# Kaixhin/imitation-learning

Measured on NVIDIA H100. Metric: env_steps_per_s, higher is better.
Workload: dtype f32

## Files before the change

### imitation-learning_b200/_lib.py

```python
from __future__ import annotations

import ctypes as C
import os
import threading
from typing import Dict, Optional

import torch

_HERE = os.path.dirname(os.path.abspath(__file__))
LIB_PATH = os.path.join(_HERE, 'csrc', 'libil_b200.so')
MAX_LAYERS = 6
MAX_WIDTH_CLASSES = 8
ACT = {'relu': 0, 'tanh': 1, 'sigmoid': 2}
REWARD = {'AIRL': 0, 'GAIL': 1, 'FAIRL': 2}
LOSS = {'BCE': 0, 'Mixup': 1, 'PUGAIL': 2}
GEMM_MODE = {'fp32': 0, 'tf32x3': 1, 'tf32': 2}

c_f32p, c_i32p, c_i64p, c_u64p, vp = C.c_void_p, C.c_void_p, C.c_void_p, C.c_void_p, C.c_void_p


class Mlp(C.Structure):
  _fields_ = [('params', vp), ('stride', C.c_int64), ('n_layers', C.c_int32), ('activation', C.c_int32), ('dims', C.c_int32 * (MAX_LAYERS + 1)), ('_pad', C.c_int32)]


class Adam(C.Structure):
  _fields_ = [('m', vp), ('v', vp), ('step', vp), ('lr', C.c_double), ('beta1', C.c_double), ('beta2', C.c_double), ('eps', C.c_double), ('weight_decay', C.c_double), ('lr_r', vp),
              ('weight_decay_r', vp), ('replica_floats', C.c_int64)]


class Batch(C.Structure):
  _fields_ = [('rows', vp), ('replica_stride', C.c_int64), ('B', C.c_int32), ('S', C.c_int32), ('A', C.c_int32), ('row', C.c_int32)]


class Replay(C.Structure):
  _fields_ = [('rows', vp), ('replica_stride', C.c_int64), ('idx', vp), ('full', vp), ('num_trajectories', vp), ('size', C.c_int32), ('S', C.c_int32), ('A', C.c_int32),
              ('row', C.c_int32), ('absorbing', C.c_int32), ('shared', C.c_int32)]


class SacArgs(C.Structure):
  _fields_ = [('actor', Mlp), ('critic', Mlp), ('target', Mlp), ('actor_opt', Adam), ('critic_opt', Adam), ('alpha_opt', Adam), ('log_alpha', vp), ('batch', Batch),
              ('absorbing', vp), ('absorbing_from_state', C.c_int32), ('R', C.c_int32), ('eps_next', vp), ('eps_new', vp), ('discount', C.c_float),
              ('entropy_target', C.c_float), ('polyak_factor', C.c_float), ('_pad0', C.c_float), ('out_log_probs', vp), ('out_q_values', vp), ('out_losses', vp),
              ('workspace', vp), ('workspace_bytes', C.c_int64), ('discount_r', vp), ('entropy_target_r', vp), ('polyak_r', vp)]


class BcArgs(C.Structure):
  _fields_ = [('actor', Mlp), ('opt', Adam), ('batch', Batch), ('R', C.c_int32), ('_pad', C.c_int32), ('out_loss', vp), ('workspace', vp), ('workspace_bytes', C.c_int64)]


class Gail(C.Structure):
  _fields_ = [('g', Mlp), ('u', vp), ('v', vp), ('u_stride', C.c_int32), ('v_stride', C.c_int32), ('state_only', C.c_int32), ('reward_function', C.c_int32),
              ('reward_function_r', vp), ('spectral_norm_r', vp), ('n_width_classes', C.c_int32), ('width_class_H', C.c_int32 * MAX_WIDTH_CLASSES),
              ('width_class_begin', C.c_int32 * MAX_WIDTH_CLASSES), ('_pad', C.c_int32), ('replica_order', vp)]


class GailUpdateArgs(C.Structure):
  _fields_ = [('disc', Gail), ('opt', Adam), ('policy', Batch), ('expert', Batch), ('eps_gp', vp), ('eps_mix', vp), ('R', C.c_int32), ('loss_function', C.c_int32),
              ('training', C.c_int32), ('_pad', C.c_int32), ('grad_penalty', C.c_float), ('entropy_bonus', C.c_float), ('pos_class_prior', C.c_float),
              ('nonnegative_margin', C.c_float), ('out_losses', vp), ('workspace', vp), ('workspace_bytes', C.c_int64), ('grad_penalty_r', vp), ('entropy_bonus_r', vp),
              ('loss_function_r', vp), ('pos_class_prior_r', vp), ('nonnegative_margin_r', vp)]


class Gailx(C.Structure):
  _fields_ = [('g', Mlp), ('h', Mlp), ('g_u', vp), ('g_v', vp), ('h_u', vp), ('h_v', vp), ('g_u_stride', C.c_int32), ('g_v_stride', C.c_int32), ('h_u_stride', C.c_int32),
              ('h_v_stride', C.c_int32), ('state_only', C.c_int32), ('reward_function', C.c_int32), ('subtract_log_policy', C.c_int32), ('discount', C.c_float), ('discount_r', vp)]


class GailxUpdateArgs(C.Structure):
  _fields_ = [('disc', Gailx), ('opt', Adam), ('params_floats', C.c_int64), ('policy', Batch), ('expert', Batch), ('eps_gp', vp), ('eps_mix', vp), ('logp_policy', vp),
              ('logp_expert', vp), ('logp_mix', vp), ('R', C.c_int32), ('loss_function', C.c_int32), ('training', C.c_int32), ('_pad', C.c_int32), ('grad_penalty', C.c_float),
              ('entropy_bonus', C.c_float), ('pos_class_prior', C.c_float), ('nonnegative_margin', C.c_float), ('out_losses', vp), ('workspace', vp), ('workspace_bytes', C.c_int64), ('grad_penalty_r', vp),
              ('entropy_bonus_r', vp)]


class Red(C.Structure):
  _fields_ = [('predictor', Mlp), ('target', Mlp), ('sigma', vp), ('state_only', C.c_int32), ('_pad', C.c_int32)]


class RedUpdateArgs(C.Structure):
  _fields_ = [('disc', Red), ('opt', Adam), ('batch', Batch), ('R', C.c_int32), ('_pad', C.c_int32), ('mask_in', vp), ('mask_hid', vp * MAX_LAYERS), ('out_loss', vp), ('workspace', vp),
              ('workspace_bytes', C.c_int64)]


class Pwil(C.Structure):
  _fields_ = [('atoms', vp), ('scale', vp), ('offset', vp), ('weights', vp), ('N', C.c_int32), ('d', C.c_int32), ('S', C.c_int32), ('A', C.c_int32), ('state_only', C.c_int32),
              ('time_horizon', C.c_int32), ('reward_scale', C.c_float), ('reward_bandwidth', C.c_float)]


class Env(C.Structure):
  _fields_ = [('M', vp), ('N', vp), ('c', vp), ('w_r', vp), ('x', vp), ('t', vp), ('obs', C.c_int32), ('act', C.c_int32), ('absorbing', C.c_int32),
              ('max_episode_steps', C.c_int32), ('early_termination', C.c_int32), ('term_threshold', C.c_float)]


class EvalArgs(C.Structure):
  _fields_ = [('actor', Mlp), ('env', Env), ('R', C.c_int32), ('episodes', C.c_int32), ('max_steps', C.c_int32), ('traj_T', C.c_int32), ('state', vp), ('returns', vp),
              ('traj_states', vp), ('traj_actions', vp), ('traj_rewards', vp), ('traj_len', vp), ('out_counters', vp), ('workspace', vp), ('workspace_bytes', C.c_int64)]


i32, i64, u64, f32 = C.c_int32, C.c_int64, C.c_uint64, C.c_float
P = C.POINTER

SIGNATURES = {
  'il_create': (C.c_int, [C.c_int, P(vp)]),
  'il_destroy': (C.c_int, [vp]),
  'il_last_error': (C.c_char_p, []),
  'il_version': (C.c_int, []),
  'il_set_gemm_mode': (C.c_int, [vp, C.c_int]),
  'il_launch_count': (i64, [vp]),
  'il_set_option': (C.c_int, [vp, C.c_char_p, C.c_int]),
  'il_struct_sizes': (C.c_int, [P(i32)]),
  'il_mlp_param_offsets': (C.c_int, [P(i32), C.c_int, P(i64), P(i64), P(i64)]),
  'il_row_layout': (C.c_int, [C.c_int, C.c_int, P(i32), P(i32)]),
  'il_profile_begin': (C.c_int, [vp]),
  'il_profile_end': (C.c_int, [vp, P(C.c_double), P(C.c_double), P(i64)]),
  'il_profile_bytes': (C.c_int, [vp, P(C.c_double)]),
  'il_debug_gemm': (C.c_int, [vp, C.c_int, C.c_int, C.c_int, C.c_int, vp, i64, C.c_int, C.c_int, vp, i64, C.c_int, C.c_int, vp, i64, C.c_int, vp, i64, C.c_int, vp, i64, C.c_int,
                              C.c_int, vp, i64, vp]),
  'il_fill_normal': (C.c_int, [vp, vp, i64, u64, u64, vp, vp]),
  'il_fill_uniform': (C.c_int, [vp, vp, i64, u64, u64, vp, vp]),
  'il_counter_add': (C.c_int, [vp, vp, u64, vp]),
  'il_fill_beta': (C.c_int, [vp, vp, C.c_int, i64, vp, u64, u64, vp, vp]),
  'il_actor_workspace_bytes': (i64, [P(Mlp), C.c_int, C.c_int]),
  'il_actor_forward': (C.c_int, [vp, P(Mlp), C.c_int, C.c_int, vp, i64, C.c_int, vp, vp, vp, vp, vp, vp, vp, i64, vp]),
  'il_critic_workspace_bytes': (i64, [P(Mlp), C.c_int, C.c_int]),
  'il_critic_forward': (C.c_int, [vp, P(Mlp), C.c_int, C.c_int, C.c_int, vp, i64, C.c_int, vp, i64, C.c_int, vp, vp, vp, i64, vp]),
  'il_polyak': (C.c_int, [vp, vp, vp, i64, f32, vp]),
  'il_sac_workspace_bytes': (i64, [P(SacArgs)]),
  'il_sac_update': (C.c_int, [vp, P(SacArgs), vp]),
  'il_bc_workspace_bytes': (i64, [P(BcArgs)]),
  'il_bc_update': (C.c_int, [vp, P(BcArgs), vp]),
  'il_adam_step': (C.c_int, [vp, vp, vp, P(Adam), i64, vp]),
  'il_adam_step_polyak': (C.c_int, [vp, vp, vp, P(Adam), i64, vp, C.c_float, vp]),
  'il_adam_step_polyak_r': (C.c_int, [vp, vp, vp, P(Adam), i64, vp, vp, vp]),
  'il_fill_dropout_mask': (C.c_int, [vp, vp, i64, f32, u64, u64, vp, vp]),
  'il_actor_dropout_workspace_bytes': (i64, [P(Mlp), C.c_int, C.c_int]),
  'il_actor_log_prob_dropout': (C.c_int, [vp, P(Mlp), C.c_int, C.c_int, C.c_int, vp, i64, C.c_int, vp, vp, P(vp), vp, vp, i64, vp]),
  'il_bc_update_dropout': (C.c_int, [vp, P(BcArgs), vp, P(vp), vp]),
  'il_dril_reward': (C.c_int, [vp, vp, C.c_int, C.c_int, C.c_int, vp, C.c_int, vp, i64, C.c_int, vp, vp]),
  'il_red_workspace_bytes': (i64, [P(Red), C.c_int, C.c_int]),
  'il_red_update': (C.c_int, [vp, P(RedUpdateArgs), vp]),
  'il_red_sigma': (C.c_int, [vp, P(Red), C.c_int, P(Batch), vp, P(vp), vp, i64, vp]),
  'il_red_reward': (C.c_int, [vp, P(Red), C.c_int, P(Batch), vp, i64, C.c_int, vp, i64, vp]),
  'il_replay_append': (C.c_int, [vp, P(Replay), C.c_int, vp, vp, vp, vp, vp, vp, vp, vp, C.c_int, vp]),
  'il_replay_wrap_absorbing': (C.c_int, [vp, P(Replay), C.c_int, vp, vp]),
  'il_replay_transfer': (C.c_int, [vp, P(Replay), C.c_int, P(Replay), vp]),
  'il_replay_sample_indices': (C.c_int, [vp, P(Replay), C.c_int, C.c_int, vp, vp, u64, u64, vp, vp]),
  'il_replay_gather': (C.c_int, [vp, P(Replay), C.c_int, vp, P(Batch), vp]),
  'il_mix_expert_rows': (C.c_int, [vp, P(Batch), P(Batch), C.c_int, vp]),
  'il_adril_relabel': (C.c_int, [vp, P(Batch), P(Batch), C.c_int, C.c_int, C.c_int, vp, vp, f32, vp, C.c_int, C.c_int, vp]),
  'il_gail_workspace_bytes': (i64, [P(GailUpdateArgs)]),
  'il_gail_update': (C.c_int, [vp, P(GailUpdateArgs), vp]),
  'il_gail_reward': (C.c_int, [vp, P(Gail), C.c_int, P(Batch), vp, i64, C.c_int, vp, vp]),
  'il_gailx_workspace_bytes': (i64, [P(GailxUpdateArgs)]),
  'il_gailx_update': (C.c_int, [vp, P(GailxUpdateArgs), vp]),
  'il_gailx_reward_workspace_bytes': (i64, [P(Gailx), C.c_int, C.c_int]),
  'il_gailx_reward': (C.c_int, [vp, P(Gailx), C.c_int, P(Batch), vp, vp, i64, C.c_int, vp, vp, i64, vp]),
  'il_gail_mix_batch': (C.c_int, [vp, P(Batch), P(Batch), vp, C.c_int, P(Batch), vp]),
  'il_gmmil_workspace_bytes': (i64, [C.c_int, C.c_int]),
  'il_gmmil_bandwidth': (C.c_int, [vp, C.c_int, P(Batch), P(Batch), C.c_int, vp, vp, i64, vp]),
  'il_gmmil_reward': (C.c_int, [vp, C.c_int, P(Batch), P(Batch), C.c_int, vp, vp, i64, C.c_int, vp]),
  'il_pwil_reset': (C.c_int, [vp, P(Pwil), C.c_int, vp, vp]),
  'il_pwil_reward': (C.c_int, [vp, P(Pwil), C.c_int, vp, vp, vp, vp, vp]),
  'il_env_reset': (C.c_int, [vp, P(Env), C.c_int, vp, vp, vp, vp, vp]),
  'il_env_step': (C.c_int, [vp, P(Env), C.c_int, vp, vp, vp, vp, vp, vp, vp, vp, vp]),
  'il_rollout_bookkeep': (C.c_int, [vp, C.c_int, vp, vp, vp, vp, vp, vp, vp, vp]),
  'il_eval_accumulate': (C.c_int, [vp, C.c_int, vp, vp, vp, vp, vp, vp]),
  'il_return_stats': (C.c_int, [vp, vp, i64, vp, vp]),
  'il_eval_workspace_bytes': (i64, [P(EvalArgs)]),
  'il_eval_rollout': (C.c_int, [vp, P(EvalArgs), vp]),
  'il_nccl_unique_id': (C.c_int, [vp]),
  'il_nccl_comm_create': (C.c_int, [vp, C.c_int, C.c_int, P(vp)]),
  'il_nccl_comm_destroy': (C.c_int, [vp]),
  'il_return_allreduce': (C.c_int, [vp, vp, vp, i64, vp, vp]),
}

_lock = threading.Lock()
_lib: Optional[C.CDLL] = None
_handles: Dict[int, int] = {}


def build(force: bool = False, verbose: bool = False) -> str:
  import importlib.util
  spec = importlib.util.spec_from_file_location('il_b200_csrc_build', os.path.join(_HERE, 'csrc', 'build.py'))
  mod = importlib.util.module_from_spec(spec)
  spec.loader.exec_module(mod)
  return mod.build(force=force, verbose=verbose)


def lib() -> C.CDLL:
  global _lib
  with _lock:
    if _lib is None:
      if not os.path.exists(LIB_PATH): build()
      l = C.CDLL(LIB_PATH)
      for name, (res, args) in SIGNATURES.items():
        fn = getattr(l, name)
        fn.restype, fn.argtypes = res, args
      _lib = l
  return _lib


def last_error() -> str:
  return lib().il_last_error().decode()


def check(rc: int):
  if rc != 0: raise RuntimeError(f'il_b200: {last_error()}')


def handle(device: Optional[int] = None) -> int:
  if not torch.cuda.is_available():
    raise RuntimeError('il_b200: no CUDA device available; the hot path only exists as sm_90a kernels (no CPU fallback)')
  device = torch.cuda.current_device() if device is None else device
  with _lock:
    h = _handles.get(device)
  if h is None:
    out = vp()
    check(lib().il_create(device, C.byref(out)))
    h = out.value
    with _lock: _handles[device] = h
    mode = os.environ.get('IL_GEMM_MODE')
    if mode: check(lib().il_set_gemm_mode(h, GEMM_MODE[mode]))
  return h


def set_option(name: str, value: int):
  check(lib().il_set_option(handle(), name.encode(), int(value)))


def stream() -> int:
  return torch.cuda.current_stream().cuda_stream


def launch_count() -> int:
  return int(lib().il_launch_count(handle()))


def mask_array(masks):
  arr = (vp * MAX_LAYERS)()
  for i, t in enumerate(masks or []): arr[i] = None if t is None else t.data_ptr()
  return arr


def ptr(t: Optional[torch.Tensor]) -> Optional[int]:
  if t is None: return None
  assert t.is_cuda, 'il_b200 expects CUDA tensors'
  return t.data_ptr()


def mlp_offsets(dims):
  n = len(dims) - 1
  d = (i32 * len(dims))(*dims)
  w, b, tot = (i64 * n)(), (i64 * n)(), i64()
  check(lib().il_mlp_param_offsets(d, n, w, b, C.byref(tot)))
  return list(w), list(b), tot.value


def row_layout(S: int, A: int):
  off, n = (i32 * 8)(), i32()
  check(lib().il_row_layout(S, A, off, C.byref(n)))
  names = ('states', 'actions', 'rewards', 'next_states', 'terminals', 'timeouts', 'weights', 'step')
  return dict(zip(names, list(off))), n.value


def py_mlp_offsets(dims):
  al = lambda x, a: (x + a - 1) // a * a
  off, w, b = 0, [], []
  for l in range(len(dims) - 1):
    w.append(off)
    off = al(off + dims[l + 1] * dims[l], 4)
    b.append(off)
    off = al(off + dims[l + 1], 4)
  return w, b, al(off, 32)


def py_row_layout(S: int, A: int):
  off = dict(states=0, actions=S, rewards=S + A, next_states=S + A + 1, terminals=2 * S + A + 1, timeouts=2 * S + A + 2, weights=2 * S + A + 3, step=2 * S + A + 4)
  return off, (2 * S + A + 5 + 3) // 4 * 4
```

### imitation-learning_b200/csrc/common.cuh

```cuda
#pragma once
#include <cuda_runtime.h>
#include <stdint.h>
#include <stdio.h>
#include <string.h>

#include <vector>

#include "../../include/il_b200.h"

struct ProfiledLaunch {
  cudaEvent_t start, stop;
  double flops;
  double bytes;
};
struct il_handle {
  int device;
  int sm_count;
  int gemm_mode;
  int thin_hoist;
  int wide_tn;
  int first_layer_fast;
  int mask_bits;
  int head_fused;
  int debug_sync;
  int adam_tma;
  int gail_tiled;
  int tc_fuse_l1;
  long long launches;
  int profiling;
  std::vector<ProfiledLaunch> profiled;
  double profiled_bytes;
  void* eval_graph;
  cudaStream_t build_stream;
};
void il_eval_release(il_handle* h);

extern thread_local char g_il_error[512];

#define IL_FAIL(...)                                     \
  do {                                                   \
    snprintf(g_il_error, sizeof(g_il_error), __VA_ARGS__); \
    return 1;                                            \
  } while (0)

#define IL_CHECK(cond, ...)        \
  do {                             \
    if (!(cond)) IL_FAIL(__VA_ARGS__); \
  } while (0)

#define IL_CUDA(expr)                                                                             \
  do {                                                                                            \
    cudaError_t _e = (expr);                                                                      \
    if (_e != cudaSuccess) IL_FAIL("%s failed: %s (%s:%d)", #expr, cudaGetErrorString(_e), __FILE__, __LINE__); \
  } while (0)

#define IL_LAUNCH(h, kernel, grid, block, smem, stream, ...)                                      \
  do {                                                                                            \
    kernel<<<(grid), (block), (smem), (cudaStream_t)(stream)>>>(__VA_ARGS__);                     \
    (h)->launches++;                                                                              \
    cudaError_t _e = cudaPeekAtLastError();                                                       \
    if (_e != cudaSuccess) IL_FAIL("launch of %s failed: %s (%s:%d)", #kernel, cudaGetErrorString(_e), __FILE__, __LINE__); \
  } while (0)

#define IL_TRY(expr)          \
  do {                        \
    int _r = (expr);          \
    if (_r != 0) return _r;   \
  } while (0)

__host__ __device__ static inline int64_t il_align_up(int64_t x, int64_t a) { return (x + a - 1) / a * a; }

struct RowLayout {
  int state, action, reward, next_state, terminal, timeout, weight, step, len;
};
__host__ __device__ inline RowLayout row_layout(int S, int A) {
  RowLayout L;
  L.state = 0;
  L.action = S;
  L.reward = S + A;
  L.next_state = S + A + 1;
  L.terminal = 2 * S + A + 1;
  L.timeout = L.terminal + 1;
  L.weight = L.terminal + 2;
  L.step = L.terminal + 3;
  L.len = (2 * S + A + 5 + 3) / 4 * 4;
  return L;
}

struct MlpOffsets {
  int64_t w[IL_MAX_LAYERS], b[IL_MAX_LAYERS], total;
};
__host__ __device__ static inline MlpOffsets mlp_offsets(const int32_t* dims, int n_layers) {
  MlpOffsets o;
  int64_t off = 0;
  for (int l = 0; l < n_layers; ++l) {
    o.w[l] = off;
    off = il_align_up(off + (int64_t)dims[l + 1] * dims[l], 4);
    o.b[l] = off;
    off = il_align_up(off + dims[l + 1], 4);
  }
  o.total = il_align_up(off, 32);
  return o;
}

__device__ __forceinline__ float act_apply(float x, int act) {
  if (act == IL_ACT_RELU) return fmaxf(x, 0.f);
  if (act == IL_ACT_TANH) return tanhf(x);
  return 1.f / (1.f + expf(-x));
}
__device__ __forceinline__ float act_grad_from_output(float y, int act) {
  if (act == IL_ACT_RELU) return y > 0.f ? 1.f : 0.f;
  if (act == IL_ACT_TANH) return 1.f - y * y;
  return y * (1.f - y);
}
__device__ __forceinline__ float softplusf(float x) {
  return x > 20.f ? x : log1pf(expf(x));
}
__device__ __forceinline__ float sigmoidf(float x) { return 1.f / (1.f + expf(-x)); }

__device__ __forceinline__ float warp_sum(float v) {
#pragma unroll
  for (int o = 16; o > 0; o >>= 1) v += __shfl_xor_sync(0xffffffffu, v, o);
  return v;
}
__device__ __forceinline__ float warp_max(float v) {
#pragma unroll
  for (int o = 16; o > 0; o >>= 1) v = fmaxf(v, __shfl_xor_sync(0xffffffffu, v, o));
  return v;
}
__device__ __forceinline__ float block_sum(float v, float* red) {
  const int lane = threadIdx.x & 31, warp = threadIdx.x >> 5, nw = (blockDim.x + 31) >> 5;
  v = warp_sum(v);
  __syncthreads();
  if (lane == 0) red[warp] = v;
  __syncthreads();
  float r = 0.f;
  if (warp == 0) {
    r = lane < nw ? red[lane] : 0.f;
    r = warp_sum(r);
    if (lane == 0) red[0] = r;
  }
  __syncthreads();
  return red[0];
}

__device__ __forceinline__ uint4 philox4x32_10(uint4 ctr, uint2 key) {
  const uint32_t M0 = 0xD2511F53u, M1 = 0xCD9E8D57u, W0 = 0x9E3779B9u, W1 = 0xBB67AE85u;
#pragma unroll
  for (int i = 0; i < 10; ++i) {
    const uint32_t hi0 = __umulhi(M0, ctr.x), lo0 = M0 * ctr.x;
    const uint32_t hi1 = __umulhi(M1, ctr.z), lo1 = M1 * ctr.z;
    ctr = make_uint4(hi1 ^ ctr.y ^ key.x, lo1, hi0 ^ ctr.w ^ key.y, lo0);
    key.x += W0;
    key.y += W1;
  }
  return ctr;
}
__device__ __forceinline__ float u32_to_unit(uint32_t x) { return (float)(x >> 8) * (1.0f / 16777216.0f); }

struct GemmArgs {
  const float* A;
  int64_t a_gs;
  int a_gdiv, lda, a_kmajor;
  const float* B;
  int64_t b_gs;
  int b_gdiv, ldb, b_kmajor;
  float* C;
  int64_t c_gs;
  int ldc;
  const float* bias;
  int64_t bias_gs;
  int act;
  const float* mask;
  int64_t mask_gs;
  int ldmask, mask_act;
  float* colsum;
  int64_t colsum_gs;
  int accumulate;
  int M, N, K, G;
  const uint32_t* mask_bits;
  int64_t mask_bits_gs;
  uint32_t* bits_out;
  int64_t bits_out_gs;
};
int launch_gemm(il_handle* h, const GemmArgs& a, cudaStream_t stream);
bool gemm_uses_tc(const il_handle* h, const GemmArgs& a);
bool gemm_first_layer_emits_bits(const il_handle* h, const GemmArgs& a);
double gemm_algorithmic_bytes(const GemmArgs& a, bool stores_c);
int profile_open(il_handle* h, ProfiledLaunch* pl, double flops, double bytes, cudaStream_t stream);
int profile_close(il_handle* h, ProfiledLaunch* pl, cudaStream_t stream);

bool tc_gemm_eligible(const GemmArgs& a);
int launch_tc_gemm(il_handle* h, const GemmArgs& a, cudaStream_t stream);
int tc_gemm_init();
struct TcFuseL1 {
  const float* x;
  int64_t x_gs;
  int x_gdiv, x_ld, x_k;
  const float* w1;
  const float* b1;
  int64_t gs;
  float* store;
  int64_t store_gs;
};
bool tc_head_fusable(const il_handle* h, const GemmArgs& a, int head_n);
bool tc_l1_fusable(const il_handle* h, const GemmArgs& a, int x_k);
bool tc_dx_head_fusable(const il_handle* h, const GemmArgs& a, int head_n);
int launch_tc_gemm_dx_head(il_handle* h, const GemmArgs& a, const float* w, int64_t w_gs, int w_ns, int head_n, float* out, int64_t out_gs, cudaStream_t stream);
int launch_tc_gemm_head(il_handle* h, const GemmArgs& a, const float* head_w, const float* head_b, int64_t head_gs, int head_n, float* head_out, int64_t head_out_gs, int store_c,
                        cudaStream_t stream, const TcFuseL1* l1 = nullptr);
```

### imitation-learning_b200/csrc/mlp.cu

```cuda
#include "mlp.cuh"

#include <math.h>

constexpr int HB_MAXN = 8;
struct HeadBwdArgs {
  const float* dout; int64_t dout_gs; int dout_gdiv, ld_dout;
  const float* w; int64_t w_gs;
  const float* y; int64_t y_gs;
  float* dz; int64_t dz_gs;
  float* dw; float* db; float* db_prev; int64_t g_gs;
  int n, H, Nh;
};
int launch_head_backward(il_handle* h, const HeadBwdArgs& a, int G, cudaStream_t stream);
int launch_head_dx_bits(il_handle* h, const HeadBwdArgs& a, const uint32_t* bits, int64_t bits_gs, int G, cudaStream_t stream);

int mlp_validate(const il_mlp* m, const char* what) {
  IL_CHECK(m != nullptr && m->params != nullptr, "%s: null mlp", what);
  IL_CHECK(m->n_layers >= 1 && m->n_layers <= IL_MAX_LAYERS, "%s: n_layers %d out of range", what, m->n_layers);
  IL_CHECK(m->activation >= 0 && m->activation <= 2, "%s: bad activation %d", what, m->activation);
  for (int l = 0; l <= m->n_layers; ++l) IL_CHECK(m->dims[l] > 0, "%s: dims[%d] = %d", what, l, m->dims[l]);
  const MlpOffsets o = mlp_offsets(m->dims, m->n_layers);
  IL_CHECK(m->stride >= o.total - 31 && m->stride % 4 == 0, "%s: stride %lld too small / unaligned for %lld parameters", what, (long long)m->stride, (long long)o.total);
  IL_CHECK((reinterpret_cast<uintptr_t>(m->params) & 15) == 0, "%s: params not 16-byte aligned", what);
  return 0;
}

int mlp_max_hidden(const il_mlp* m) {
  int mx = 1;
  for (int l = 1; l <= m->n_layers; ++l) mx = m->dims[l] > mx ? m->dims[l] : mx;
  return mx;
}

static int64_t mlp_bits_bytes(const il_mlp* m, int G, int n, int l) {
  return m->dims[l + 1] % 32 == 0 ? il_align_up((int64_t)G * n * (m->dims[l + 1] / 32) * 4, 256) : 0;
}

int64_t mlp_acts_bytes(const il_mlp* m, int G, int n) {
  int64_t b = 0;
  for (int l = 0; l + 1 < m->n_layers; ++l) b += il_align_up((int64_t)G * n * m->dims[l + 1] * 4, 256) + mlp_bits_bytes(m, G, n, l);
  return b;
}

char* mlp_acts_carve(const il_mlp* m, int G, int n, char* ws, MlpActs* acts) {
  for (int l = 0; l < IL_MAX_LAYERS; ++l) { acts->hid[l] = nullptr; acts->bits[l] = nullptr; acts->bits_valid[l] = false; }
  for (int l = 0; l + 1 < m->n_layers; ++l) {
    acts->hid[l] = reinterpret_cast<float*>(ws);
    ws += il_align_up((int64_t)G * n * m->dims[l + 1] * 4, 256);
    if (mlp_bits_bytes(m, G, n, l)) {
      acts->bits[l] = reinterpret_cast<uint32_t*>(ws);
      ws += mlp_bits_bytes(m, G, n, l);
    }
  }
  return ws;
}

int mlp_forward(il_handle* h, const il_mlp* m, int G, int n, MatView X, MlpActs& acts, float* out, int64_t out_gs, int ld_out, cudaStream_t stream, int keep) {
  const MlpOffsets o = mlp_offsets(m->dims, m->n_layers);
  const int L = m->n_layers;
  const bool keep_hidden = keep != MLP_KEEP_NONE;
  const bool want_bits = h->mask_bits && keep_hidden && m->activation == IL_ACT_RELU;
  for (int l = 0; l < IL_MAX_LAYERS; ++l) acts.bits_valid[l] = false;
  auto layer_args = [&](int l) {
    GemmArgs a{};
    if (l == 0) { a.A = X.ptr; a.a_gs = X.gs; a.a_gdiv = X.gdiv; a.lda = X.ld; }
    else { a.A = acts.hid[l - 1]; a.a_gs = (int64_t)n * m->dims[l]; a.a_gdiv = 1; a.lda = m->dims[l]; }
    a.a_kmajor = 1;
    a.B = m->params + o.w[l]; a.b_gs = m->stride; a.b_gdiv = 1; a.ldb = m->dims[l]; a.b_kmajor = 1;
    a.bias = m->params + o.b[l]; a.bias_gs = m->stride;
    if (l == L - 1) { a.C = out; a.c_gs = out_gs; a.ldc = ld_out; a.act = -1; }
    else { a.C = acts.hid[l]; a.c_gs = (int64_t)n * m->dims[l + 1]; a.ldc = m->dims[l + 1]; a.act = m->activation; }
    a.M = n; a.N = m->dims[l + 1]; a.K = m->dims[l]; a.G = G;
    return a;
  };
  const bool head_shape = L >= 2 && m->activation == IL_ACT_RELU && ld_out == m->dims[L] && out_gs == (int64_t)n * m->dims[L];
  for (int l = 0; l < L; ++l) {
    if (head_shape && l == L - 2) {
      GemmArgs a = layer_args(l);
      if (tc_head_fusable(h, a, m->dims[L])) {
        const bool bits = want_bits && keep == MLP_KEEP_MASKS && acts.bits[l] && m->dims[L] <= HB_MAXN;
        if (bits) { a.bits_out = acts.bits[l]; a.bits_out_gs = (int64_t)n * (m->dims[l + 1] / 32); acts.bits_valid[l] = true; }
        IL_TRY(launch_tc_gemm_head(h, a, m->params + o.w[L - 1], m->params + o.b[L - 1], m->stride, m->dims[L], out, out_gs, keep_hidden && !bits ? 1 : 0, stream));
        return 0;
      }
    }
    if (head_shape && l == 0 && L == 3) {
      GemmArgs a1 = layer_args(1);
      a1.A = nullptr; a1.a_gs = 0; a1.a_gdiv = 1; a1.lda = m->dims[1];
      if (tc_head_fusable(h, a1, m->dims[L]) && tc_l1_fusable(h, a1, m->dims[0])) {
        TcFuseL1 f{};
        f.x = X.ptr; f.x_gs = X.gs; f.x_gdiv = X.gdiv; f.x_ld = X.ld; f.x_k = m->dims[0];
        f.w1 = m->params + o.w[0]; f.b1 = m->params + o.b[0]; f.gs = m->stride;
        f.store = keep_hidden ? acts.hid[0] : nullptr; f.store_gs = (int64_t)n * m->dims[1];
        IL_TRY(launch_tc_gemm_head(h, a1, m->params + o.w[L - 1], m->params + o.b[L - 1], m->stride, m->dims[L], out, out_gs, keep_hidden ? 1 : 0, stream, &f));
        return 0;
      }
    }
    GemmArgs a = layer_args(l);
    if (want_bits && l + 1 < L && acts.bits[l] && gemm_first_layer_emits_bits(h, a)) {
      a.bits_out = acts.bits[l]; a.bits_out_gs = (int64_t)n * (m->dims[l + 1] / 32);
      acts.bits_valid[l] = true;
    }
    IL_TRY(launch_gemm(h, a, stream));
  }
  return 0;
}

static bool head_backward_eligible(const il_mlp* m, int n, int64_t grad_stride) {
  const int L = m->n_layers, H = m->dims[L - 1], Nh = m->dims[L];
  return m->activation == IL_ACT_RELU && Nh <= HB_MAXN && H % 4 == 0 && n <= 1024 && grad_stride % 4 == 0 && m->stride % 4 == 0;
}

int mlp_backward(il_handle* h, const il_mlp* m, int G, int n, MatView X, const MlpActs& acts, MatView dOut, float* grads, int64_t grad_stride,
                 float* dX, int64_t dx_gs, int ld_dx, int dx_col0, int dx_cols, float* tmpA, float* tmpB, cudaStream_t stream) {
  const MlpOffsets o = mlp_offsets(m->dims, m->n_layers);
  const int L = m->n_layers;
  MatView dZ = dOut;
  float* next_tmp = tmpA;
  bool bias_done = false;
  for (int l = L - 1; l >= 0; --l) {
    MatView Xin = l == 0 ? X : MatView{acts.hid[l - 1], (int64_t)n * m->dims[l], 1, m->dims[l]};
    if (l == L - 1 && l > 0 && grads && h->head_fused && head_backward_eligible(m, n, grad_stride)) {
      HeadBwdArgs a{};
      a.dout = dZ.ptr; a.dout_gs = dZ.gs; a.dout_gdiv = dZ.gdiv; a.ld_dout = dZ.ld;
      a.w = m->params + o.w[l]; a.w_gs = m->stride;
      a.y = acts.hid[l - 1]; a.y_gs = (int64_t)n * m->dims[l];
      a.dz = next_tmp; a.dz_gs = (int64_t)n * m->dims[l];
      a.dw = grads + o.w[l]; a.db = grads + o.b[l]; a.db_prev = grads + o.b[l - 1]; a.g_gs = grad_stride;
      a.n = n; a.H = m->dims[l]; a.Nh = m->dims[l + 1];
      IL_TRY(launch_head_backward(h, a, G, stream));
      dZ = MatView{next_tmp, (int64_t)n * m->dims[l], 1, m->dims[l]};
      next_tmp = next_tmp == tmpA ? tmpB : tmpA;
      bias_done = true;
      continue;
    }
    if (l == L - 1 && l > 0 && !grads && acts.bits_valid[l - 1] && m->dims[l + 1] <= HB_MAXN) {
      HeadBwdArgs a{};
      a.dout = dZ.ptr; a.dout_gs = dZ.gs; a.dout_gdiv = dZ.gdiv; a.ld_dout = dZ.ld;
      a.w = m->params + o.w[l]; a.w_gs = m->stride;
      a.dz = next_tmp; a.dz_gs = (int64_t)n * m->dims[l];
      a.n = n; a.H = m->dims[l]; a.Nh = m->dims[l + 1];
      IL_TRY(launch_head_dx_bits(h, a, acts.bits[l - 1], (int64_t)n * (m->dims[l] / 32), G, stream));
      dZ = MatView{next_tmp, (int64_t)n * m->dims[l], 1, m->dims[l]};
      next_tmp = next_tmp == tmpA ? tmpB : tmpA;
      continue;
    }
    if (grads) {
      GemmArgs a{};
      a.A = dZ.ptr; a.a_gs = dZ.gs; a.a_gdiv = dZ.gdiv; a.lda = dZ.ld; a.a_kmajor = 0;
      a.B = Xin.ptr; a.b_gs = Xin.gs; a.b_gdiv = Xin.gdiv; a.ldb = Xin.ld; a.b_kmajor = 0;
      a.C = grads + o.w[l]; a.c_gs = grad_stride; a.ldc = m->dims[l]; a.act = -1;
      if (!bias_done) { a.colsum = grads + o.b[l]; a.colsum_gs = grad_stride; }
      bias_done = false;
      a.M = m->dims[l + 1]; a.N = m->dims[l]; a.K = n; a.G = G;
      IL_TRY(launch_gemm(h, a, stream));
    }
    if (l > 0) {
      GemmArgs a{};
      a.A = dZ.ptr; a.a_gs = dZ.gs; a.a_gdiv = dZ.gdiv; a.lda = dZ.ld; a.a_kmajor = 1;
      a.B = m->params + o.w[l]; a.b_gs = m->stride; a.b_gdiv = 1; a.ldb = m->dims[l]; a.b_kmajor = 0;
      a.C = next_tmp; a.c_gs = (int64_t)n * m->dims[l]; a.ldc = m->dims[l]; a.act = -1;
      a.mask_act = m->activation;
      a.M = n; a.N = m->dims[l]; a.K = m->dims[l + 1]; a.G = G;
      if (acts.bits_valid[l - 1] && m->activation == IL_ACT_RELU && gemm_uses_tc(h, a)) {
        a.mask_bits = acts.bits[l - 1]; a.mask_bits_gs = (int64_t)n * (m->dims[l] / 32);
        if (h->mask_bits >= 2 && l == 1 && !grads && dX && ld_dx == dx_cols && dx_gs == (int64_t)n * dx_cols && tc_dx_head_fusable(h, a, dx_cols)) {
          a.C = nullptr;
          IL_TRY(launch_tc_gemm_dx_head(h, a, m->params + o.w[0] + dx_col0, m->stride, m->dims[0], dx_cols, dX, dx_gs, stream));
          return 0;
        }
      } else {
        a.mask = acts.hid[l - 1]; a.mask_gs = (int64_t)n * m->dims[l]; a.ldmask = m->dims[l];
      }
      IL_TRY(launch_gemm(h, a, stream));
      dZ = MatView{next_tmp, (int64_t)n * m->dims[l], 1, m->dims[l]};
      next_tmp = next_tmp == tmpA ? tmpB : tmpA;
    } else if (dX) {
      GemmArgs a{};
      a.A = dZ.ptr; a.a_gs = dZ.gs; a.a_gdiv = dZ.gdiv; a.lda = dZ.ld; a.a_kmajor = 1;
      a.B = m->params + o.w[0] + dx_col0; a.b_gs = m->stride; a.b_gdiv = 1; a.ldb = m->dims[0]; a.b_kmajor = 0;
      a.C = dX; a.c_gs = dx_gs; a.ldc = ld_dx; a.act = -1;
      a.M = n; a.N = dx_cols; a.K = m->dims[1]; a.G = G;
      IL_TRY(launch_gemm(h, a, stream));
    }
  }
  return 0;
}

namespace {

__global__ void actor_head_kernel(const HeadFwdArgs p) {
  const int64_t row = (int64_t)blockIdx.x * blockDim.x + threadIdx.x;
  if (row >= (int64_t)p.R * p.n) return;
  const int r = (int)(row / p.n), i = (int)(row % p.n);
  const int A = p.A;
  const float* hd = p.head + row * 2 * A;
  float* act_row = p.action ? p.action + (int64_t)r * p.action_rs + (int64_t)i * p.ld_action : nullptr;
  if (p.copy_src && act_row) {
    const float* src = p.copy_src + (int64_t)r * p.copy_rs + (int64_t)i * p.copy_ld;
    for (int j = 0; j < p.copy_cols; ++j) act_row[j - p.copy_cols] = __ldg(src + j);
  }
  const float keep = p.zero_mask ? 1.f - __ldg(p.zero_mask + (int64_t)r * p.zero_mask_rs + (int64_t)i * p.zero_mask_ld) : 1.f;
  const float LOG_SQRT_2PI = 0.91893853320467274178f, LOG2 = 0.69314718055994530942f;
  const float A_LO = (float)(-1.0 + 1e-6), A_HI = (float)(1.0 - 1e-6);
  float sum_ladj = 0.f, sum_nlp = 0.f;
  const bool want_lp = p.log_prob != nullptr && (p.eps != nullptr || p.given != nullptr);
  for (int j = 0; j < A; ++j) {
    const float mu = hd[j];
    const float ls = fminf(fmaxf(hd[A + j], -20.f), 2.f);
    if (p.mean) p.mean[row * A + j] = mu;
    if (p.log_std) p.log_std[row * A + j] = ls;
    float x, a;
    const float sd = expf(ls);
    if (p.given) {
      a = fminf(fmaxf(p.given[row * A + j], A_LO), A_HI);
      x = atanhf(a);
    } else if (p.eps) {
      x = __fadd_rn(mu, __fmul_rn(sd, p.eps[row * A + j]));
      a = tanhf(x);
    } else {
      x = mu;
      a = tanhf(mu);
    }
    if (act_row && !p.given) act_row[j] = keep * a;
    if (want_lp) {
      const float var = __fmul_rn(sd, sd);
      const float diff = __fsub_rn(x, mu);
      float nlp = __fdiv_rn(-__fmul_rn(diff, diff), __fmul_rn(2.f, var));
      nlp = __fsub_rn(__fsub_rn(nlp, logf(sd)), LOG_SQRT_2PI);
      const float ladj = __fmul_rn(2.f, __fsub_rn(__fsub_rn(LOG2, x), softplusf(__fmul_rn(-2.f, x))));
      sum_nlp += nlp;
      sum_ladj += ladj;
    }
  }
  if (want_lp) p.log_prob[row] = __fadd_rn(__fsub_rn(0.f, sum_ladj), sum_nlp);
}

struct SmallFwdArgs {
  il_mlp m;
  MlpOffsets o;
  const float* X;
  int64_t x_gs;
  int x_gdiv, ldx, n, maxd;
  float* out;
  int tanh_first;
};
template <int NR>
__global__ void __launch_bounds__(256) mlp_small_forward_kernel(const SmallFwdArgs p) {
  extern __shared__ __align__(16) float sm[];
  const int g = blockIdx.x, r0 = blockIdx.y * NR, tid = threadIdx.x, warp = tid >> 5, lane = tid & 31;
  const int nr = min(NR, p.n - r0), L = p.m.n_layers, maxd = p.maxd;
  float* bufs[2] = {sm, sm + NR * maxd};
  const float* X = p.X + (int64_t)(g / p.x_gdiv) * p.x_gs;
  for (int idx = tid; idx < NR * p.m.dims[0]; idx += 256) {
    const int r = idx / p.m.dims[0], k = idx % p.m.dims[0];
    bufs[0][r * maxd + k] = r < nr ? __ldg(X + (int64_t)(r0 + r) * p.ldx + k) : 0.f;
  }
  const float* prm = p.m.params + (int64_t)g * p.m.stride;
  __syncthreads();
  for (int l = 0; l < L; ++l) {
    const int in = p.m.dims[l], od = p.m.dims[l + 1];
    const float* W = prm + p.o.w[l];
    const float* bias = prm + p.o.b[l];
    const float* xin = bufs[l & 1];
    float* xout = bufs[(l + 1) & 1];
    const bool vec = (in % 4 == 0) && (p.m.stride % 4 == 0);
    if (NR == 1 && vec && in <= 16) {
      for (int o = tid; o < od; o += 256) {
        const float4* wr = reinterpret_cast<const float4*>(W + (int64_t)o * in);
        float4 w4[4];
#pragma unroll
        for (int q = 0; q < 4; ++q) w4[q] = 4 * q < in ? __ldg(wr + q) : make_float4(0.f, 0.f, 0.f, 0.f);
        float v = __ldg(bias + o);
#pragma unroll
        for (int q = 0; q < 4; ++q)
          if (4 * q < in) {
            const float4 x4 = *reinterpret_cast<const float4*>(xin + 4 * q);
            v = fmaf(w4[q].x, x4.x, fmaf(w4[q].y, x4.y, fmaf(w4[q].z, x4.z, fmaf(w4[q].w, x4.w, v))));
          }
        if (l < L - 1) v = act_apply(v, p.m.activation);
        xout[o] = v;
      }
      __syncthreads();
      continue;
    }
    if (NR == 1 && vec && in % 128 == 0 && in <= 256) {
      const int kv = in >> 7;
      float4 x4[2];
#pragma unroll
      for (int v = 0; v < 2; ++v) x4[v] = v < kv ? *reinterpret_cast<const float4*>(xin + v * 128 + lane * 4) : make_float4(0.f, 0.f, 0.f, 0.f);
      for (int o0 = warp * 8; o0 < od; o0 += 64) {
        float4 w4[8][2];
#pragma unroll
        for (int u = 0; u < 8; ++u)
#pragma unroll
          for (int v = 0; v < 2; ++v)
            w4[u][v] = (o0 + u < od && v < kv) ? __ldg(reinterpret_cast<const float4*>(W + (int64_t)(o0 + u) * in + v * 128 + lane * 4)) : make_float4(0.f, 0.f, 0.f, 0.f);
        float a8[8];
#pragma unroll
        for (int u = 0; u < 8; ++u) {
          float t = 0.f;
#pragma unroll
          for (int v = 0; v < 2; ++v) t = fmaf(w4[u][v].x, x4[v].x, fmaf(w4[u][v].y, x4[v].y, fmaf(w4[u][v].z, x4[v].z, fmaf(w4[u][v].w, x4[v].w, t))));
          a8[u] = warp_sum(t);
        }
        if (lane < 8 && o0 + lane < od) {
          float v = a8[0];
#pragma unroll
          for (int u = 1; u < 8; ++u) v = lane == u ? a8[u] : v;
          v += __ldg(bias + o0 + lane);
          if (l < L - 1) v = act_apply(v, p.m.activation);
          xout[o0 + lane] = v;
        }
      }
      __syncthreads();
      continue;
    }
    if (NR == 1 && vec) {
      for (int o0 = warp * 4; o0 < od; o0 += 32) {
        float a4[4] = {0.f, 0.f, 0.f, 0.f};
        for (int k = lane * 4; k < in; k += 128) {
          const float4 x4 = *reinterpret_cast<const float4*>(xin + k);
          float4 w4[4];
#pragma unroll
          for (int u = 0; u < 4; ++u) w4[u] = o0 + u < od ? __ldg(reinterpret_cast<const float4*>(W + (int64_t)(o0 + u) * in + k)) : make_float4(0.f, 0.f, 0.f, 0.f);
#pragma unroll
          for (int u = 0; u < 4; ++u) a4[u] = fmaf(w4[u].x, x4.x, fmaf(w4[u].y, x4.y, fmaf(w4[u].z, x4.z, fmaf(w4[u].w, x4.w, a4[u]))));
        }
#pragma unroll
        for (int u = 0; u < 4; ++u) a4[u] = warp_sum(a4[u]);
        if (lane < 4 && o0 + lane < od) {
          float v = (lane == 0 ? a4[0] : lane == 1 ? a4[1] : lane == 2 ? a4[2] : a4[3]) + __ldg(bias + o0 + lane);
          if (l < L - 1) v = act_apply(v, p.m.activation);
          xout[o0 + lane] = v;
        }
      }
      __syncthreads();
      continue;
    }
    for (int o = warp; o < od; o += 8) {
      float acc[NR];
#pragma unroll
      for (int r = 0; r < NR; ++r) acc[r] = 0.f;
      const float* wr = W + (int64_t)o * in;
      if (vec) {
        for (int k = lane * 4; k < in; k += 128) {
          const float4 w4 = __ldg(reinterpret_cast<const float4*>(wr + k));
#pragma unroll
          for (int r = 0; r < NR; ++r) {
            const float4 x4 = *reinterpret_cast<const float4*>(xin + r * maxd + k);
            acc[r] = fmaf(w4.x, x4.x, fmaf(w4.y, x4.y, fmaf(w4.z, x4.z, fmaf(w4.w, x4.w, acc[r]))));
          }
        }
      } else {
        for (int k = lane; k < in; k += 32) {
          const float w = __ldg(wr + k);
#pragma unroll
          for (int r = 0; r < NR; ++r) acc[r] = fmaf(w, xin[r * maxd + k], acc[r]);
        }
      }
#pragma unroll
      for (int r = 0; r < NR; ++r) acc[r] = warp_sum(acc[r]);
      if (lane == 0) {
        const float b = __ldg(bias + o);
#pragma unroll
        for (int r = 0; r < NR; ++r) {
          float v = acc[r] + b;
          if (l < L - 1) v = act_apply(v, p.m.activation);
          xout[r * maxd + o] = v;
        }
      }
    }
    __syncthreads();
  }
  const int od = p.m.dims[L];
  const float* fin = bufs[L & 1];
  if (p.tanh_first > 0) {
    const int A = p.tanh_first;
    for (int idx = tid; idx < nr * A; idx += 256) {
      const int r = idx / A, o = idx % A;
      p.out[((int64_t)g * p.n + r0 + r) * A + o] = tanhf(fin[r * maxd + o]);
    }
    return;
  }
  for (int idx = tid; idx < nr * od; idx += 256) {
    const int r = idx / od, o = idx % od;
    p.out[((int64_t)g * p.n + r0 + r) * od + o] = fin[r * maxd + o];
  }
}

struct AdamReplicas {
  const double* lr_r;
  const double* wd_r;
  const float* tau_r;
  int64_t rf;
  float inv_rf;
  int R;
};
struct AdamCoef { float step_size, decay, tau, one_minus_tau; };
constexpr int ADAM_MAX_REPLICAS = 2048;
__device__ __forceinline__ void adam_fill_table(AdamCoef* tab, const AdamReplicas& rp, double lr, double wd, double beta1_d, const int64_t* step, float tau) {
  if (!rp.R) return;
  const double bc1 = 1.0 - pow(beta1_d, (double)*step);
  for (int r = threadIdx.x; r < rp.R; r += blockDim.x) {
    const double l = rp.lr_r ? rp.lr_r[r] : lr, w = rp.wd_r ? rp.wd_r[r] : wd;
    const float t = rp.tau_r ? rp.tau_r[r] : tau;
    tab[r] = AdamCoef{(float)(l / bc1), w != 0.0 ? (float)(1.0 - l * w) : 1.f, t, (float)(1.0 - (double)t)};
  }
}
__device__ __forceinline__ int adam_replica(int64_t f, const AdamReplicas& rp) {
  int r = (int)((float)f * rp.inv_rf);
  if ((int64_t)r * rp.rf > f) --r;
  else if ((int64_t)(r + 1) * rp.rf <= f) ++r;
  return r;
}

__global__ void adam_kernel(float* __restrict__ p, const float* __restrict__ g, float* __restrict__ m, float* __restrict__ v, const int64_t* __restrict__ step,
                            double lr, double beta1_d, double beta2_d, double eps_d, double wd, int64_t n, float* __restrict__ target, float tau, float one_minus_tau,
                            const AdamReplicas rp) {
  extern __shared__ AdamCoef adam_tab[];
  __shared__ float s_step_size, s_bc2_sqrt;
  if (threadIdx.x == 0) {
    const double t = (double)*step;
    const double bc1 = 1.0 - pow(beta1_d, t), bc2 = 1.0 - pow(beta2_d, t);
    s_step_size = (float)(lr / bc1);
    s_bc2_sqrt = (float)sqrt(bc2);
  }
  adam_fill_table(adam_tab, rp, lr, wd, beta1_d, step, tau);
  __syncthreads();
  const float step_size = s_step_size, bc2_sqrt = s_bc2_sqrt;
  const float decay = (float)(1.0 - lr * wd), w1 = (float)(1.0 - beta1_d), w2 = (float)(1.0 - beta2_d);
  const float beta2 = (float)beta2_d, eps = (float)eps_d;
  const bool has_wd = wd != 0.0;
  auto upd = [&](float& pi, float& mi, float& vi, float gi, float ss, float dc, bool wdf) {
    if (wdf) pi = __fmul_rn(pi, dc);
    mi = __fadd_rn(mi, __fmul_rn(w1, __fsub_rn(gi, mi)));
    vi = __fadd_rn(__fmul_rn(vi, beta2), __fmul_rn(__fmul_rn(w2, gi), gi));
    const float denom = __fadd_rn(__fdiv_rn(sqrtf(vi), bc2_sqrt), eps);
    pi = __fadd_rn(pi, __fmul_rn(-ss, __fdiv_rn(mi, denom)));
  };
  const int64_t n4 = n >> 2;
  for (int64_t i = (int64_t)blockIdx.x * blockDim.x + threadIdx.x; i < n4; i += (int64_t)gridDim.x * blockDim.x) {
    float ss = step_size, dc = decay, ta = tau, omt = one_minus_tau;
    bool wdf = has_wd;
    if (rp.R) {
      const AdamCoef c = adam_tab[adam_replica(i << 2, rp)];
      ss = c.step_size; dc = c.decay; wdf = c.decay != 1.f; ta = c.tau; omt = c.one_minus_tau;
    }
    float4 pv = reinterpret_cast<float4*>(p)[i], mv = reinterpret_cast<float4*>(m)[i], vv = reinterpret_cast<float4*>(v)[i];
    const float4 gv = reinterpret_cast<const float4*>(g)[i];
    upd(pv.x, mv.x, vv.x, gv.x, ss, dc, wdf); upd(pv.y, mv.y, vv.y, gv.y, ss, dc, wdf); upd(pv.z, mv.z, vv.z, gv.z, ss, dc, wdf); upd(pv.w, mv.w, vv.w, gv.w, ss, dc, wdf);
    reinterpret_cast<float4*>(p)[i] = pv; reinterpret_cast<float4*>(m)[i] = mv; reinterpret_cast<float4*>(v)[i] = vv;
    if (target) {
      const float tau = ta, one_minus_tau = omt;
      float4 tv = reinterpret_cast<float4*>(target)[i];
      tv.x = __fadd_rn(__fmul_rn(tv.x, tau), __fmul_rn(one_minus_tau, pv.x)); tv.y = __fadd_rn(__fmul_rn(tv.y, tau), __fmul_rn(one_minus_tau, pv.y));
      tv.z = __fadd_rn(__fmul_rn(tv.z, tau), __fmul_rn(one_minus_tau, pv.z)); tv.w = __fadd_rn(__fmul_rn(tv.w, tau), __fmul_rn(one_minus_tau, pv.w));
      reinterpret_cast<float4*>(target)[i] = tv;
    }
  }
  for (int64_t i = (n4 << 2) + (int64_t)blockIdx.x * blockDim.x + threadIdx.x; i < n; i += (int64_t)gridDim.x * blockDim.x) {
    float pi = p[i], mi = m[i], vi = v[i];
    upd(pi, mi, vi, g[i], step_size, decay, has_wd);
    p[i] = pi; m[i] = mi; v[i] = vi;
    if (target) target[i] = __fadd_rn(__fmul_rn(target[i], tau), __fmul_rn(one_minus_tau, pi));
  }
}

constexpr int ADAM_STREAMS = 5;
constexpr int ADAM_CONSUMERS = 256;
template <int TILE, int STAGES> constexpr int adam_tma_smem() { return STAGES * ADAM_STREAMS * TILE * 4 + 2 * STAGES * 8 + 64; }
__device__ __forceinline__ void adam_mbar_wait(uint32_t bar, uint32_t parity) {
  asm volatile(
      "{\n\t.reg .pred q;\n\t"
      "ADAM_WAIT:\n\t"
      "mbarrier.try_wait.parity.shared::cta.b64 q, [%0], %1;\n\t"
      "@q bra ADAM_DONE;\n\t"
      "bra ADAM_WAIT;\n\t"
      "ADAM_DONE:\n\t}" ::"r"(bar), "r"(parity) : "memory");
}
template <int TILE, int STAGES>
__global__ void __launch_bounds__(ADAM_CONSUMERS + 32) adam_tma_kernel(float* __restrict__ p, const float* __restrict__ g, float* __restrict__ m, float* __restrict__ v,
                                                                      const int64_t* __restrict__ step, double lr, double beta1_d, double beta2_d, double eps_d, double wd, int64_t n,
                                                                      float* __restrict__ target, float tau, float one_minus_tau, const AdamReplicas rp) {
  extern __shared__ __align__(128) uint8_t adam_smem[];
  float* buf = reinterpret_cast<float*>(adam_smem);
  AdamCoef* tab = reinterpret_cast<AdamCoef*>(adam_smem + adam_tma_smem<TILE, STAGES>());
  const uint32_t smem0 = (uint32_t)__cvta_generic_to_shared(buf);
  const uint32_t full0 = smem0 + (uint32_t)(STAGES * ADAM_STREAMS * TILE * 4), done0 = full0 + 8u * STAGES;
  __shared__ float s_step_size, s_bc2_sqrt;
  const int tid = threadIdx.x;
  adam_fill_table(tab, rp, lr, wd, beta1_d, step, tau);
  if (tid == 0) {
    const double t = (double)*step;
    s_step_size = (float)(lr / (1.0 - pow(beta1_d, t)));
    s_bc2_sqrt = (float)sqrt(1.0 - pow(beta2_d, t));
    for (int s_ = 0; s_ < STAGES; ++s_) {
      asm volatile("mbarrier.init.shared::cta.b64 [%0], 1;" ::"r"(full0 + 8u * s_));
      asm volatile("mbarrier.init.shared::cta.b64 [%0], %1;" ::"r"(done0 + 8u * s_), "r"(ADAM_CONSUMERS));
    }
    asm volatile("fence.mbarrier_init.release.cluster;" ::: "memory");
  }
  __syncthreads();
  const int64_t n_tiles = (n + TILE - 1) / TILE;
  const int n_streams = target ? 5 : 4;
  auto tile_floats = [&](int64_t tile) { const int64_t left = n - tile * TILE; return (int)(left < TILE ? left : TILE); };
  const int64_t my_tiles = blockIdx.x < n_tiles ? (n_tiles - blockIdx.x + gridDim.x - 1) / gridDim.x : 0;
  if (tid >= ADAM_CONSUMERS) {
    if (tid != ADAM_CONSUMERS) return;
    auto issue_loads = [&](int64_t k) {
      const int64_t tile = blockIdx.x + k * gridDim.x;
      const int stage = (int)(k % STAGES);
      const uint32_t bytes = (uint32_t)tile_floats(tile) * 4u, bar = full0 + 8u * stage;
      asm volatile("mbarrier.arrive.expect_tx.shared::cta.b64 _, [%0], %1;" ::"r"(bar), "r"(bytes * (uint32_t)n_streams) : "memory");
      const float* src[5] = {p, g, m, v, target};
      for (int q = 0; q < n_streams; ++q)
        asm volatile("cp.async.bulk.shared::cluster.global.mbarrier::complete_tx::bytes [%0], [%1], %2, [%3];" ::"r"(smem0 + (uint32_t)((stage * ADAM_STREAMS + q) * TILE * 4)),
                     "l"(src[q] + tile * TILE), "r"(bytes), "r"(bar) : "memory");
    };
    for (int64_t k = 0; k < STAGES - 1 && k < my_tiles; ++k) issue_loads(k);
    for (int64_t k = 0; k < my_tiles; ++k) {
      const int stage = (int)(k % STAGES);
      const int64_t tile = blockIdx.x + k * gridDim.x;
      if (k + STAGES - 1 < my_tiles) {
        if (k > 0) asm volatile("cp.async.bulk.wait_group.read 0;" ::: "memory");
        issue_loads(k + STAGES - 1);
      }
      adam_mbar_wait(done0 + 8u * stage, (uint32_t)((k / STAGES) & 1));
      const uint32_t bytes = (uint32_t)tile_floats(tile) * 4u;
      float* dst[5] = {p, nullptr, m, v, target};
      for (int q = 0; q < n_streams; ++q) {
        if (!dst[q]) continue;
        asm volatile("cp.async.bulk.global.shared::cta.bulk_group [%0], [%1], %2;" ::"l"(dst[q] + tile * TILE), "r"(smem0 + (uint32_t)((stage * ADAM_STREAMS + q) * TILE * 4)), "r"(bytes)
                     : "memory");
      }
      asm volatile("cp.async.bulk.commit_group;" ::: "memory");
    }
    asm volatile("cp.async.bulk.wait_group 0;" ::: "memory");
    return;
  }
  const float step_size = s_step_size, bc2_sqrt = s_bc2_sqrt;
  const float decay = (float)(1.0 - lr * wd), w1 = (float)(1.0 - beta1_d), w2 = (float)(1.0 - beta2_d), beta2 = (float)beta2_d, eps = (float)eps_d;
  const bool has_wd = wd != 0.0;
  auto upd = [&](float& pi, float& mi, float& vi, float gi, float ss, float dc, bool wdf) {
    if (wdf) pi = __fmul_rn(pi, dc);
    mi = __fadd_rn(mi, __fmul_rn(w1, __fsub_rn(gi, mi)));
    vi = __fadd_rn(__fmul_rn(vi, beta2), __fmul_rn(__fmul_rn(w2, gi), gi));
    const float denom = __fadd_rn(__fdiv_rn(sqrtf(vi), bc2_sqrt), eps);
    pi = __fadd_rn(pi, __fmul_rn(-ss, __fdiv_rn(mi, denom)));
  };
  for (int64_t k = 0; k < my_tiles; ++k) {
    const int stage = (int)(k % STAGES);
    const int64_t tile = blockIdx.x + k * gridDim.x;
    adam_mbar_wait(full0 + 8u * stage, (uint32_t)((k / STAGES) & 1));
    const int nf4 = tile_floats(tile) >> 2;
    float4* sp = reinterpret_cast<float4*>(buf + (stage * ADAM_STREAMS + 0) * TILE);
    const float4* sg = reinterpret_cast<const float4*>(buf + (stage * ADAM_STREAMS + 1) * TILE);
    float4* smm = reinterpret_cast<float4*>(buf + (stage * ADAM_STREAMS + 2) * TILE);
    float4* sv = reinterpret_cast<float4*>(buf + (stage * ADAM_STREAMS + 3) * TILE);
    float4* stg = reinterpret_cast<float4*>(buf + (stage * ADAM_STREAMS + 4) * TILE);
    for (int i = tid; i < nf4; i += ADAM_CONSUMERS) {
      float ss = step_size, dc = decay, ta = tau, omt = one_minus_tau;
      bool wdf = has_wd;
      if (rp.R) {
        const AdamCoef c = tab[adam_replica(tile * TILE + 4 * i, rp)];
        ss = c.step_size; dc = c.decay; wdf = c.decay != 1.f; ta = c.tau; omt = c.one_minus_tau;
      }
      float4 pv = sp[i], mv = smm[i], vv = sv[i];
      const float4 gv = sg[i];
      upd(pv.x, mv.x, vv.x, gv.x, ss, dc, wdf); upd(pv.y, mv.y, vv.y, gv.y, ss, dc, wdf); upd(pv.z, mv.z, vv.z, gv.z, ss, dc, wdf); upd(pv.w, mv.w, vv.w, gv.w, ss, dc, wdf);
      sp[i] = pv; smm[i] = mv; sv[i] = vv;
      if (target) {
        const float tau = ta, one_minus_tau = omt;
        float4 tv = stg[i];
        tv.x = __fadd_rn(__fmul_rn(tv.x, tau), __fmul_rn(one_minus_tau, pv.x)); tv.y = __fadd_rn(__fmul_rn(tv.y, tau), __fmul_rn(one_minus_tau, pv.y));
        tv.z = __fadd_rn(__fmul_rn(tv.z, tau), __fmul_rn(one_minus_tau, pv.z)); tv.w = __fadd_rn(__fmul_rn(tv.w, tau), __fmul_rn(one_minus_tau, pv.w));
        stg[i] = tv;
      }
    }
    asm volatile("fence.proxy.async.shared::cta;" ::: "memory");
    asm volatile("mbarrier.arrive.shared::cta.b64 _, [%0];" ::"r"(done0 + 8u * stage) : "memory");
  }
}

template <int TILE, int STAGES>
static int launch_adam_tma(il_handle* h, int ctas_per_sm, float* params, const float* grads, const il_adam* opt, int64_t n, cudaStream_t stream, float* polyak_target, float polyak_factor,
                           const AdamReplicas& rp) {
  static bool attr_set = false;
  if (!attr_set) {
    IL_CUDA(cudaFuncSetAttribute(adam_tma_kernel<TILE, STAGES>, cudaFuncAttributeMaxDynamicSharedMemorySize, adam_tma_smem<TILE, STAGES>() + ADAM_MAX_REPLICAS * (int)sizeof(AdamCoef)));
    attr_set = true;
  }
  const size_t smem = (size_t)adam_tma_smem<TILE, STAGES>() + (size_t)rp.R * sizeof(AdamCoef);
  IL_LAUNCH(h, (adam_tma_kernel<TILE, STAGES>), h->sm_count * ctas_per_sm, ADAM_CONSUMERS + 32, smem, stream, params, grads, opt->m, opt->v, opt->step, opt->lr, opt->beta1,
            opt->beta2, opt->eps, opt->weight_decay, n, polyak_target, polyak_factor, (float)(1.0 - (double)polyak_factor), rp);
  return 0;
}
constexpr int ADAM_TMA_MIN_TILES = 4096;


template <int NH>
__global__ void __launch_bounds__(256, 2) head_backward_kernel(const HeadBwdArgs p) {
  extern __shared__ __align__(16) float hb_sm[];
  const int g = blockIdx.y, n0 = blockIdx.x * 256, tid = threadIdx.x, tc = tid & 63, tr = tid >> 6, col = n0 + tc * 4;
  float* dos = hb_sm;
  float* red = hb_sm + p.n * HB_MAXN;
  const float* dout = p.dout + (int64_t)(g / p.dout_gdiv) * p.dout_gs;
  const bool active = col < p.H;
  const float* Y = p.y + (int64_t)g * p.y_gs + col;
  float4 yv[4], yn[4];
  auto fetch = [&](float4 (&dst)[4], int b0) {
#pragma unroll
    for (int u = 0; u < 4; ++u) {
      const int b = b0 + 4 * u;
      dst[u] = (active && b < p.n) ? __ldg(reinterpret_cast<const float4*>(Y + (int64_t)b * p.H)) : make_float4(0.f, 0.f, 0.f, 0.f);
    }
  };
  fetch(yv, tr);
  for (int i = tid; i < p.n * HB_MAXN; i += 256) {
    const int b = i / HB_MAXN, j = i % HB_MAXN;
    dos[i] = j < p.Nh ? __ldg(dout + (int64_t)b * p.ld_dout + j) : 0.f;
  }
  float4 w[NH];
#pragma unroll
  for (int j = 0; j < NH; ++j) w[j] = (active && j < p.Nh) ? __ldg(reinterpret_cast<const float4*>(p.w + (int64_t)g * p.w_gs + (int64_t)j * p.H + col)) : make_float4(0.f, 0.f, 0.f, 0.f);
  __syncthreads();
  float4 dw[NH], cs = make_float4(0.f, 0.f, 0.f, 0.f);
#pragma unroll
  for (int j = 0; j < NH; ++j) dw[j] = make_float4(0.f, 0.f, 0.f, 0.f);
  if (active) {
    float* DZ = p.dz + (int64_t)g * p.dz_gs + col;
    for (int b0 = tr; b0 < p.n; b0 += 16) {
      fetch(yn, b0 + 16);
#pragma unroll
      for (int u = 0; u < 4; ++u) {
        const int b = b0 + 4 * u;
        if (b >= p.n) continue;
        float dj[NH];
        if (NH == 1) dj[0] = dos[b * HB_MAXN];
        else {
          const float4 d0 = *reinterpret_cast<const float4*>(dos + b * HB_MAXN), d1 = *reinterpret_cast<const float4*>(dos + b * HB_MAXN + 4);
          const float t[8] = {d0.x, d0.y, d0.z, d0.w, d1.x, d1.y, d1.z, d1.w};
#pragma unroll
          for (int j = 0; j < NH; ++j) dj[j] = t[j];
        }
        float4 z = make_float4(0.f, 0.f, 0.f, 0.f);
#pragma unroll
        for (int j = 0; j < NH; ++j) {
          z.x = fmaf(dj[j], w[j].x, z.x); z.y = fmaf(dj[j], w[j].y, z.y); z.z = fmaf(dj[j], w[j].z, z.z); z.w = fmaf(dj[j], w[j].w, z.w);
          dw[j].x = fmaf(dj[j], yv[u].x, dw[j].x); dw[j].y = fmaf(dj[j], yv[u].y, dw[j].y); dw[j].z = fmaf(dj[j], yv[u].z, dw[j].z); dw[j].w = fmaf(dj[j], yv[u].w, dw[j].w);
        }
        z.x = yv[u].x > 0.f ? z.x : 0.f; z.y = yv[u].y > 0.f ? z.y : 0.f; z.z = yv[u].z > 0.f ? z.z : 0.f; z.w = yv[u].w > 0.f ? z.w : 0.f;
        cs.x += z.x; cs.y += z.y; cs.z += z.z; cs.w += z.w;
        *reinterpret_cast<float4*>(DZ + (int64_t)b * p.H) = z;
      }
#pragma unroll
      for (int u = 0; u < 4; ++u) yv[u] = yn[u];
    }
  }
  float4* r4 = reinterpret_cast<float4*>(red);
#pragma unroll
  for (int j = 0; j < NH; ++j) r4[(tr * (HB_MAXN + 1) + j) * 64 + tc] = dw[j];
  r4[(tr * (HB_MAXN + 1) + HB_MAXN) * 64 + tc] = cs;
  __syncthreads();
  if (tr == 0 && active) {
#pragma unroll
    for (int j = 0; j <= HB_MAXN; ++j) {
      if ((j < NH && j < p.Nh) || j == HB_MAXN) {
        float4 a = r4[(0 * (HB_MAXN + 1) + j) * 64 + tc];
#pragma unroll
        for (int q = 1; q < 4; ++q) {
          const float4 t = r4[(q * (HB_MAXN + 1) + j) * 64 + tc];
          a.x += t.x; a.y += t.y; a.z += t.z; a.w += t.w;
        }
        float* dst = j == HB_MAXN ? p.db_prev + (int64_t)g * p.g_gs + col : p.dw + (int64_t)g * p.g_gs + (int64_t)j * p.H + col;
        *reinterpret_cast<float4*>(dst) = a;
      }
    }
  }
  if (blockIdx.x == 0 && tid < p.Nh) {
    float sacc = 0.f;
    for (int b = 0; b < p.n; ++b) sacc += dos[b * HB_MAXN + tid];
    p.db[(int64_t)g * p.g_gs + tid] = sacc;
  }
}

__global__ void tick_kernel(int64_t* s0, int64_t* s1, int64_t* s2) {
  if (s0) *s0 += 1;
  if (s1) *s1 += 1;
  if (s2) *s2 += 1;
}

__global__ void polyak_kernel(float* __restrict__ t, const float* __restrict__ o, int64_t n, float tau, float one_minus_tau) {
  for (int64_t i = (int64_t)blockIdx.x * blockDim.x + threadIdx.x; i < n; i += (int64_t)gridDim.x * blockDim.x)
    t[i] = __fadd_rn(__fmul_rn(t[i], tau), __fmul_rn(one_minus_tau, o[i]));
}

__global__ void split_twin_kernel(const float* __restrict__ q, float* __restrict__ q1, float* __restrict__ q2, int R, int n) {
  const int64_t i = (int64_t)blockIdx.x * blockDim.x + threadIdx.x;
  if (i >= (int64_t)R * n) return;
  const int r = (int)(i / n), b = (int)(i % n);
  if (q1) q1[i] = q[((int64_t)2 * r) * n + b];
  if (q2) q2[i] = q[((int64_t)2 * r + 1) * n + b];
}

__global__ void concat_kernel(const float* __restrict__ s, int64_t s_rs, int ld_s, int S, const float* __restrict__ a, int64_t a_rs, int ld_a, int A,
                              float* __restrict__ x, int R, int n) {
  const int64_t idx = (int64_t)blockIdx.x * blockDim.x + threadIdx.x;
  const int d = S + A;
  if (idx >= (int64_t)R * n * d) return;
  const int j = (int)(idx % d);
  const int64_t row = idx / d;
  const int r = (int)(row / n), i = (int)(row % n);
  x[idx] = j < S ? s[(int64_t)r * s_rs + (int64_t)i * ld_s + j] : a[(int64_t)r * a_rs + (int64_t)i * ld_a + (j - S)];
}

inline int ew_blocks(int64_t n, int threads, int sm_count) {
  int64_t b = (n + threads - 1) / threads;
  const int64_t cap = (int64_t)sm_count * 16;
  return (int)(b < 1 ? 1 : (b > cap ? cap : b));
}

}

int launch_actor_head(il_handle* h, const HeadFwdArgs& a, cudaStream_t stream) {
  const int64_t rows = (int64_t)a.R * a.n;
  IL_LAUNCH(h, actor_head_kernel, (unsigned)((rows + 127) / 128), 128, 0, stream, a);
  return 0;
}

int launch_adam(il_handle* h, float* params, const float* grads, const il_adam* opt, int64_t n, cudaStream_t stream, float* polyak_target, float polyak_factor,
                const float* polyak_r) {
  IL_CHECK(opt->m && opt->v && opt->step, "adam: null state");
  IL_CHECK(((reinterpret_cast<uintptr_t>(params) | reinterpret_cast<uintptr_t>(grads) | reinterpret_cast<uintptr_t>(opt->m) | reinterpret_cast<uintptr_t>(opt->v) |
             reinterpret_cast<uintptr_t>(polyak_target)) & 15) == 0, "adam: buffers must be 16-byte aligned");
  AdamReplicas rp{opt->lr_r, opt->weight_decay_r, polyak_target ? polyak_r : nullptr, 0, 0.f, 0};
  if (rp.lr_r || rp.wd_r || rp.tau_r) {
    const int64_t rf = opt->replica_floats;
    IL_CHECK(rf > 0 && rf % 4 == 0 && n % rf == 0, "adam: per-replica hyper-parameters need replica_floats (%lld) > 0, a multiple of 4 dividing n = %lld", (long long)rf, (long long)n);
    IL_CHECK(n / rf <= ADAM_MAX_REPLICAS, "adam: %lld replicas with per-replica hyper-parameters exceed the limit of %d per buffer", (long long)(n / rf), ADAM_MAX_REPLICAS);
    rp.rf = rf; rp.inv_rf = 1.f / (float)rf; rp.R = (int)(n / rf);
  }
  if (h->adam_tma && n % 4 == 0 && n >= (int64_t)ADAM_TMA_MIN_TILES * h->sm_count * 2) {
    const int variant = h->adam_tma;
    switch (variant) {
      case 2: return launch_adam_tma<4096, 2>(h, 1, params, grads, opt, n, stream, polyak_target, polyak_factor, rp);
      case 3: return launch_adam_tma<2048, 3>(h, 1, params, grads, opt, n, stream, polyak_target, polyak_factor, rp);
      case 4: return launch_adam_tma<1024, 4>(h, 2, params, grads, opt, n, stream, polyak_target, polyak_factor, rp);
      case 5: return launch_adam_tma<1024, 3>(h, 3, params, grads, opt, n, stream, polyak_target, polyak_factor, rp);
      case 6: return launch_adam_tma<512, 4>(h, 4, params, grads, opt, n, stream, polyak_target, polyak_factor, rp);
      case 7: return launch_adam_tma<2048, 4>(h, 1, params, grads, opt, n, stream, polyak_target, polyak_factor, rp);
      default: return launch_adam_tma<2048, 2>(h, 2, params, grads, opt, n, stream, polyak_target, polyak_factor, rp);
    }
  }
  IL_LAUNCH(h, adam_kernel, ew_blocks(n / 4 + 1, 256, h->sm_count), 256, (size_t)rp.R * sizeof(AdamCoef), stream, params, grads, opt->m, opt->v, opt->step, opt->lr, opt->beta1, opt->beta2,
            opt->eps, opt->weight_decay, n, polyak_target, polyak_factor, (float)(1.0 - (double)polyak_factor), rp);
  return 0;
}

namespace {
template <int NH, int U>
__global__ void __launch_bounds__(256) head_dx_bits_kernel(const HeadBwdArgs p, const uint32_t* __restrict__ bits, int64_t bits_gs) {
  const int g = blockIdx.y, tid = threadIdx.x, tc = tid & 63, tr = tid >> 6, col = blockIdx.x * 256 + tc * 4;
  if (col >= p.H) return;
  const float* __restrict__ dout = p.dout + (int64_t)(g / p.dout_gdiv) * p.dout_gs;
  const uint32_t* __restrict__ bw = bits + (int64_t)g * bits_gs + (col >> 5);
  const int sh = col & 31, wpr = p.H >> 5;
  float4 w[NH];
#pragma unroll
  for (int j = 0; j < NH; ++j) w[j] = j < p.Nh ? __ldg(reinterpret_cast<const float4*>(p.w + (int64_t)g * p.w_gs + (int64_t)j * p.H + col)) : make_float4(0.f, 0.f, 0.f, 0.f);
  float* __restrict__ dz = p.dz + (int64_t)g * p.dz_gs + col;
  for (int b0 = tr; b0 < p.n; b0 += 4 * U) {
    uint32_t m[U];
    float d[U][NH];
#pragma unroll
    for (int u = 0; u < U; ++u) {
      const int b = b0 + 4 * u;
      m[u] = b < p.n ? __ldg(bw + (int64_t)b * wpr) >> sh : 0u;
#pragma unroll
      for (int j = 0; j < NH; ++j) d[u][j] = (j < p.Nh && b < p.n) ? __ldg(dout + (int64_t)b * p.ld_dout + j) : 0.f;
    }
#pragma unroll
    for (int u = 0; u < U; ++u) {
      const int b = b0 + 4 * u;
      if (b >= p.n) break;
      float4 v = make_float4(0.f, 0.f, 0.f, 0.f);
#pragma unroll
      for (int j = 0; j < NH; ++j)
        if (j < p.Nh) { v.x = fmaf(d[u][j], w[j].x, v.x); v.y = fmaf(d[u][j], w[j].y, v.y); v.z = fmaf(d[u][j], w[j].z, v.z); v.w = fmaf(d[u][j], w[j].w, v.w); }
      v.x = m[u] & 1u ? v.x : 0.f; v.y = m[u] & 2u ? v.y : 0.f; v.z = m[u] & 4u ? v.z : 0.f; v.w = m[u] & 8u ? v.w : 0.f;
      *reinterpret_cast<float4*>(dz + (int64_t)b * p.H) = v;
    }
  }
}
}

int launch_head_dx_bits(il_handle* h, const HeadBwdArgs& a, const uint32_t* bits, int64_t bits_gs, int G, cudaStream_t stream) {
  IL_CHECK(a.H % 32 == 0 && a.Nh <= HB_MAXN && (reinterpret_cast<uintptr_t>(a.w) & 15) == 0 && a.w_gs % 4 == 0 && (reinterpret_cast<uintptr_t>(a.dz) & 15) == 0 && a.dz_gs % 4 == 0,
           "head_dx_bits: H=%d Nh=%d or unaligned buffers", a.H, a.Nh);
  if (a.Nh == 1) IL_LAUNCH(h, (head_dx_bits_kernel<1, 8>), dim3((a.H + 255) / 256, G), 256, 0, stream, a, bits, bits_gs);
  else IL_LAUNCH(h, (head_dx_bits_kernel<HB_MAXN, 4>), dim3((a.H + 255) / 256, G), 256, 0, stream, a, bits, bits_gs);
  return 0;
}

int launch_head_backward(il_handle* h, const HeadBwdArgs& a, int G, cudaStream_t stream) {
  const size_t smem = ((size_t)a.n * HB_MAXN + 4 * (HB_MAXN + 1) * 64 * 4) * sizeof(float);
  if (a.Nh == 1) IL_LAUNCH(h, head_backward_kernel<1>, dim3((a.H + 255) / 256, G), 256, smem, stream, a);
  else IL_LAUNCH(h, head_backward_kernel<HB_MAXN>, dim3((a.H + 255) / 256, G), 256, smem, stream, a);
  return 0;
}

int mlp_init() {
  IL_CUDA(cudaFuncSetAttribute(head_backward_kernel<1>, cudaFuncAttributeMaxDynamicSharedMemorySize, (1024 * HB_MAXN + 4 * (HB_MAXN + 1) * 64 * 4) * 4));
  IL_CUDA(cudaFuncSetAttribute(head_backward_kernel<HB_MAXN>, cudaFuncAttributeMaxDynamicSharedMemorySize, (1024 * HB_MAXN + 4 * (HB_MAXN + 1) * 64 * 4) * 4));
  return 0;
}

int launch_tick(il_handle* h, int64_t* s0, int64_t* s1, int64_t* s2, cudaStream_t stream) {
  IL_LAUNCH(h, tick_kernel, 1, 1, 0, stream, s0, s1, s2);
  return 0;
}

int mlp_small_forward(il_handle* h, const il_mlp* m, int G, int n, MatView X, float* out, cudaStream_t stream, int tanh_first) {
  SmallFwdArgs a;
  a.m = *m; a.o = mlp_offsets(m->dims, m->n_layers);
  a.X = X.ptr; a.x_gs = X.gs; a.x_gdiv = X.gdiv; a.ldx = X.ld; a.n = n; a.out = out; a.tanh_first = tanh_first;
  int maxd = 4;
  for (int l = 0; l <= m->n_layers; ++l) maxd = m->dims[l] > maxd ? m->dims[l] : maxd;
  a.maxd = (maxd + 3) / 4 * 4;
  if (n == 1) {
    IL_LAUNCH(h, mlp_small_forward_kernel<1>, dim3(G, 1), 256, (size_t)2 * 1 * a.maxd * 4, stream, a);
  } else {
    IL_CHECK((size_t)2 * 8 * a.maxd * 4 <= 48 * 1024, "mlp_small_forward: layer width %d too large", maxd);
    IL_LAUNCH(h, mlp_small_forward_kernel<8>, dim3(G, (n + 7) / 8), 256, (size_t)2 * 8 * a.maxd * 4, stream, a);
  }
  return 0;
}

extern "C" int il_adam_step(il_handle* h, float* params, const float* grads, const il_adam* opt, int64_t n, void* stream) {
  IL_CHECK(h && params && grads && opt, "il_adam_step: null argument");
  IL_TRY(launch_tick(h, opt->step, nullptr, nullptr, (cudaStream_t)stream));
  return launch_adam(h, params, grads, opt, n, (cudaStream_t)stream);
}

extern "C" int il_adam_step_polyak(il_handle* h, float* params, const float* grads, const il_adam* opt, int64_t n, float* target, float polyak_factor, void* stream) {
  IL_CHECK(h && params && grads && opt && target, "il_adam_step_polyak: null argument");
  IL_TRY(launch_tick(h, opt->step, nullptr, nullptr, (cudaStream_t)stream));
  return launch_adam(h, params, grads, opt, n, (cudaStream_t)stream, target, polyak_factor);
}

extern "C" int il_adam_step_polyak_r(il_handle* h, float* params, const float* grads, const il_adam* opt, int64_t n, float* target, const float* polyak_r, void* stream) {
  IL_CHECK(h && params && grads && opt && target && polyak_r, "il_adam_step_polyak_r: null argument");
  IL_TRY(launch_tick(h, opt->step, nullptr, nullptr, (cudaStream_t)stream));
  return launch_adam(h, params, grads, opt, n, (cudaStream_t)stream, target, 0.f, polyak_r);
}

extern "C" int il_polyak(il_handle* h, float* target, const float* online, int64_t n, float polyak_factor, void* stream) {
  IL_CHECK(h && target && online && n >= 0, "il_polyak: bad argument");
  if (n == 0) return 0;
  IL_LAUNCH(h, polyak_kernel, ew_blocks(n, 256, h->sm_count), 256, 0, (cudaStream_t)stream, target, online, n, polyak_factor, (float)(1.0 - (double)polyak_factor));
  return 0;
}

extern "C" int64_t il_actor_workspace_bytes(const il_mlp* actor, int R, int n) {
  return mlp_acts_bytes(actor, R, n) + il_align_up((int64_t)R * n * actor->dims[actor->n_layers] * 4, 256);
}

extern "C" int il_actor_forward(il_handle* h, const il_mlp* actor, int R, int n, const float* states, int64_t states_rs, int ld_states, const float* eps,
                                const float* given_action, float* action, float* log_prob, float* mean, float* log_std, void* workspace, int64_t workspace_bytes,
                                void* stream) {
  IL_CHECK(h && states && workspace, "il_actor_forward: null argument");
  IL_TRY(mlp_validate(actor, "il_actor_forward"));
  IL_CHECK(R > 0 && n > 0, "il_actor_forward: R=%d n=%d", R, n);
  const int out = actor->dims[actor->n_layers];
  IL_CHECK(out % 2 == 0, "il_actor_forward: head size %d is not 2*A", out);
  IL_CHECK(workspace_bytes >= il_actor_workspace_bytes(actor, R, n), "il_actor_forward: workspace too small");
  MlpActs acts;
  char* ws = mlp_acts_carve(actor, R, n, static_cast<char*>(workspace), &acts);
  float* head = reinterpret_cast<float*>(ws);
  if (n <= 32) IL_TRY(mlp_small_forward(h, actor, R, n, MatView{states, states_rs, 1, ld_states}, head, (cudaStream_t)stream));
  else IL_TRY(mlp_forward(h, actor, R, n, MatView{states, states_rs, 1, ld_states}, acts, head, (int64_t)n * out, out, (cudaStream_t)stream, MLP_KEEP_NONE));
  HeadFwdArgs a{};
  a.head = head; a.eps = eps; a.given = given_action;
  a.action = action; a.action_rs = (int64_t)n * (out / 2); a.ld_action = out / 2;
  a.log_prob = log_prob; a.mean = mean; a.log_std = log_std;
  a.R = R; a.n = n; a.A = out / 2;
  return launch_actor_head(h, a, (cudaStream_t)stream);
}

extern "C" int64_t il_critic_workspace_bytes(const il_mlp* critic, int R, int n) {
  return mlp_acts_bytes(critic, 2 * R, n) + il_align_up((int64_t)R * n * critic->dims[0] * 4, 256) + il_align_up((int64_t)2 * R * n * 4, 256);
}

extern "C" int il_critic_forward(il_handle* h, const il_mlp* twin, int R, int n, int S, const float* states, int64_t states_rs, int ld_states, const float* actions,
                                 int64_t actions_rs, int ld_actions, float* q1, float* q2, void* workspace, int64_t workspace_bytes, void* stream) {
  IL_CHECK(h && states && actions && workspace, "il_critic_forward: null argument");
  IL_TRY(mlp_validate(twin, "il_critic_forward"));
  IL_CHECK(twin->dims[twin->n_layers] == 1, "il_critic_forward: critic head must have one output");
  IL_CHECK(workspace_bytes >= il_critic_workspace_bytes(twin, R, n), "il_critic_forward: workspace too small");
  cudaStream_t st = (cudaStream_t)stream;
  const int d = twin->dims[0];
  MlpActs acts;
  char* ws = mlp_acts_carve(twin, 2 * R, n, static_cast<char*>(workspace), &acts);
  float* X = reinterpret_cast<float*>(ws);
  ws += il_align_up((int64_t)R * n * d * 4, 256);
  float* q = reinterpret_cast<float*>(ws);
  const int A = d - S;
  IL_CHECK(S > 0 && A > 0, "il_critic_forward: S=%d with input width %d", S, d);
  const int64_t total = (int64_t)R * n * d;
  IL_LAUNCH(h, concat_kernel, (unsigned)((total + 255) / 256), 256, 0, st, states, states_rs, ld_states, S, actions, actions_rs, ld_actions, A, X, R, n);
  IL_TRY(mlp_forward(h, twin, 2 * R, n, MatView{X, (int64_t)n * d, 2, d}, acts, q, (int64_t)n, 1, st, MLP_KEEP_NONE));
  IL_LAUNCH(h, split_twin_kernel, (unsigned)(((int64_t)R * n + 255) / 256), 256, 0, st, q, q1, q2, R, n);
  return 0;
}
```

### imitation-learning_b200/csrc/mlp.cuh

```cuda
#pragma once
#include "common.cuh"

struct MatView {
  const float* ptr;
  int64_t gs;
  int gdiv;
  int ld;
};

struct MlpActs {
  float* hid[IL_MAX_LAYERS];
  uint32_t* bits[IL_MAX_LAYERS];
  bool bits_valid[IL_MAX_LAYERS];
};
enum { MLP_KEEP_NONE = 0, MLP_KEEP_ALL = 1, MLP_KEEP_MASKS = 2 };

int64_t mlp_acts_bytes(const il_mlp* m, int G, int n);
char* mlp_acts_carve(const il_mlp* m, int G, int n, char* ws, MlpActs* acts);

int mlp_forward(il_handle* h, const il_mlp* m, int G, int n, MatView X, MlpActs& acts, float* out, int64_t out_gs, int ld_out,
                cudaStream_t stream, int keep = MLP_KEEP_ALL);

int mlp_backward(il_handle* h, const il_mlp* m, int G, int n, MatView X, const MlpActs& acts, MatView dOut, float* grads, int64_t grad_stride,
                 float* dX, int64_t dx_gs, int ld_dx, int dx_col0, int dx_cols, float* tmpA, float* tmpB, cudaStream_t stream);

int mlp_small_forward(il_handle* h, const il_mlp* m, int G, int n, MatView X, float* out, cudaStream_t stream, int tanh_first = 0);
int mlp_max_hidden(const il_mlp* m);
int mlp_validate(const il_mlp* m, const char* what);

struct HeadFwdArgs {
  const float* head;
  const float* eps;
  const float* given;
  float* action;
  int64_t action_rs;
  int ld_action;
  const float* zero_mask;
  int64_t zero_mask_rs;
  int zero_mask_ld;
  float* log_prob;
  float* mean;
  float* log_std;
  const float* copy_src;
  int64_t copy_rs;
  int copy_ld, copy_cols;
  int R, n, A;
};
int launch_actor_head(il_handle* h, const HeadFwdArgs& a, cudaStream_t stream);

int launch_adam(il_handle* h, float* params, const float* grads, const il_adam* opt, int64_t n, cudaStream_t stream, float* polyak_target = nullptr, float polyak_factor = 0.f,
                const float* polyak_r = nullptr);
int launch_tick(il_handle* h, int64_t* s0, int64_t* s1, int64_t* s2, cudaStream_t stream);
```

### imitation-learning_b200/csrc/sac.cu

```cuda
#include "mlp.cuh"

namespace {

struct AbsView {
  const float* ptr;
  int64_t rs;
  int ld;
};
__device__ __forceinline__ float abs_at(const AbsView& v, int r, int b) { return v.ptr ? __ldg(v.ptr + (int64_t)r * v.rs + (int64_t)b * v.ld) : 0.f; }

__global__ void sac_target_kernel(const float* __restrict__ qt, const float* __restrict__ lp_next, const float* __restrict__ log_alpha, const float* __restrict__ rows,
                                  int64_t rs, int row, int off_reward, int off_terminal, AbsView av, float discount, const float* __restrict__ discount_r, float* __restrict__ y,
                                  int R, int B) {
  const int64_t i = (int64_t)blockIdx.x * blockDim.x + threadIdx.x;
  if (i >= (int64_t)R * B) return;
  const int r = (int)(i / B), b = (int)(i % B);
  if (discount_r) discount = discount_r[r];
  const float alpha = expf(__ldg(log_alpha + r));
  const float* tr = rows + (int64_t)r * rs + (int64_t)b * row;
  const float q = fminf(qt[((int64_t)2 * r) * B + b], qt[((int64_t)2 * r + 1) * B + b]);
  const float ent = __fmul_rn(__fmul_rn(__fsub_rn(1.f, abs_at(av, r, b)), alpha), lp_next[i]);
  const float tv = __fsub_rn(q, ent);
  y[i] = __fadd_rn(tr[off_reward], __fmul_rn(__fmul_rn(__fsub_rn(1.f, tr[off_terminal]), discount), tv));
}

__global__ void sac_critic_lossgrad_kernel(const float* __restrict__ q, const float* __restrict__ y, const float* __restrict__ rows, int64_t rs, int row, int off_weight,
                                           float* __restrict__ dq, float* __restrict__ out_q, float* __restrict__ out_losses, int B) {
  __shared__ float red[32];
  const int r = blockIdx.x;
  const float invB = 1.f / (float)B;
  float l1 = 0.f, l2 = 0.f;
  for (int b = threadIdx.x; b < B; b += blockDim.x) {
    const float w = rows[(int64_t)r * rs + (int64_t)b * row + off_weight];
    const float yy = y[(int64_t)r * B + b];
    const float q1 = q[((int64_t)2 * r) * B + b], q2 = q[((int64_t)2 * r + 1) * B + b];
    const float d1 = __fsub_rn(q1, yy), d2 = __fsub_rn(q2, yy);
    l1 += w * d1 * d1;
    l2 += w * d2 * d2;
    const float c = __fmul_rn(invB, w);
    dq[((int64_t)2 * r) * B + b] = __fmul_rn(c, __fmul_rn(2.f, d1));
    dq[((int64_t)2 * r + 1) * B + b] = __fmul_rn(c, __fmul_rn(2.f, d2));
    if (out_q) out_q[(int64_t)r * B + b] = fminf(q1, q2);
  }
  l1 = block_sum(l1, red);
  l2 = block_sum(l2, red);
  if (threadIdx.x == 0 && out_losses) out_losses[r * 3 + 0] = l1 * invB + l2 * invB;
}

__global__ void sac_actor_loss_kernel(const float* __restrict__ q, const float* __restrict__ lp_new, const float* __restrict__ log_alpha, const float* __restrict__ rows,
                                      int64_t rs, int row, int off_weight, AbsView av, float* __restrict__ dq, float* __restrict__ out_losses, int B) {
  __shared__ float red[32];
  const int r = blockIdx.x;
  const float invB = 1.f / (float)B;
  const float alpha = expf(__ldg(log_alpha + r));
  float loss = 0.f;
  for (int b = threadIdx.x; b < B; b += blockDim.x) {
    const float w = rows[(int64_t)r * rs + (int64_t)b * row + off_weight];
    const float q1 = q[((int64_t)2 * r) * B + b], q2 = q[((int64_t)2 * r + 1) * B + b];
    const float g1 = q1 < q2 ? 1.f : (q1 == q2 ? 0.5f : 0.f);
    dq[((int64_t)2 * r) * B + b] = -invB * g1;
    dq[((int64_t)2 * r + 1) * B + b] = -invB * (1.f - g1);
    loss += w * (1.f - abs_at(av, r, b)) * alpha * lp_new[(int64_t)r * B + b] - fminf(q1, q2);
  }
  loss = block_sum(loss, red);
  if (threadIdx.x == 0 && out_losses) out_losses[r * 3 + 1] = loss * invB;
}

__global__ void sac_head_backward_kernel(const float* __restrict__ head, const float* __restrict__ eps, const float* __restrict__ xnew, int d, int S,
                                         const float* __restrict__ dxa, const float* __restrict__ log_alpha, const float* __restrict__ rows, int64_t rs, int row,
                                         int off_weight, AbsView av, float* __restrict__ dhead, int R, int B, int A) {
  const int64_t i = (int64_t)blockIdx.x * blockDim.x + threadIdx.x;
  if (i >= (int64_t)R * B) return;
  const int r = (int)(i / B), b = (int)(i % B);
  const float alpha = expf(__ldg(log_alpha + r));
  const float w = rows[(int64_t)r * rs + (int64_t)b * row + off_weight];
  const float c = w * (1.f - abs_at(av, r, b)) * alpha / (float)B;
  const float* hd = head + i * 2 * A;
  const float* a_row = xnew + i * d + S;
  const float* g1 = dxa + (((int64_t)2 * r) * B + b) * A;
  const float* g2 = dxa + (((int64_t)2 * r + 1) * B + b) * A;
  for (int j = 0; j < A; ++j) {
    const float raw = hd[A + j];
    const bool in_range = raw >= -20.f && raw <= 2.f;
    const float sd = expf(fminf(fmaxf(raw, -20.f), 2.f));
    const float a = a_row[j];
    const float dx = (g1[j] + g2[j]) * (1.f - a * a) + c * 2.f * a;
    dhead[i * 2 * A + j] = dx;
    dhead[i * 2 * A + A + j] = in_range ? dx * (sd * eps[i * A + j]) - c : 0.f;
  }
}

__global__ void sac_alpha_kernel(float* __restrict__ log_alpha, const float* __restrict__ lp_new, const float* __restrict__ rows, int64_t rs, int row, int off_weight,
                                 AbsView av, float entropy_target, const float* __restrict__ entropy_target_r, float* __restrict__ m, float* __restrict__ v,
                                 const int64_t* __restrict__ step, double lr, const double* __restrict__ lr_r, double beta1, double beta2, double eps, double wd,
                                 const double* __restrict__ wd_r, float* __restrict__ out_losses, int B) {
  __shared__ float red[32];
  const int r = blockIdx.x;
  if (entropy_target_r) entropy_target = entropy_target_r[r];
  if (lr_r) lr = lr_r[r];
  if (wd_r) wd = wd_r[r];
  float s = 0.f;
  for (int b = threadIdx.x; b < B; b += blockDim.x) {
    const float w = rows[(int64_t)r * rs + (int64_t)b * row + off_weight];
    s += w * (1.f - abs_at(av, r, b)) * (lp_new[(int64_t)r * B + b] + entropy_target);
  }
  s = block_sum(s, red);
  if (threadIdx.x == 0) {
    float p = log_alpha[r];
    const float alpha = expf(p);
    const float g = -alpha * s / (float)B;
    if (out_losses) out_losses[r * 3 + 2] = g;
    const double t = (double)*step;
    const float step_size = (float)(lr / (1.0 - pow(beta1, t))), bc2_sqrt = (float)sqrt(1.0 - pow(beta2, t));
    float mi = m[r], vi = v[r];
    if (wd != 0.0) p = __fmul_rn(p, (float)(1.0 - lr * wd));
    mi = __fadd_rn(mi, __fmul_rn((float)(1.0 - beta1), __fsub_rn(g, mi)));
    vi = __fadd_rn(__fmul_rn(vi, (float)beta2), __fmul_rn(__fmul_rn((float)(1.0 - beta2), g), g));
    const float denom = __fadd_rn(__fdiv_rn(sqrtf(vi), bc2_sqrt), (float)eps);
    p = __fadd_rn(p, __fmul_rn(-step_size, __fdiv_rn(mi, denom)));
    log_alpha[r] = p; m[r] = mi; v[r] = vi;
  }
}

__global__ void bc_head_backward_kernel(const float* __restrict__ head, const float* __restrict__ rows, int64_t rs, int row, int off_action, int off_weight,
                                        float* __restrict__ dhead, float* __restrict__ row_loss, int R, int B, int A) {
  const int64_t i = (int64_t)blockIdx.x * blockDim.x + threadIdx.x;
  if (i >= (int64_t)R * B) return;
  const int r = (int)(i / B), b = (int)(i % B);
  const float* tr = rows + (int64_t)r * rs + (int64_t)b * row;
  const float w = tr[off_weight], c = -w / (float)B;
  const float A_LO = (float)(-1.0 + 1e-6), A_HI = (float)(1.0 - 1e-6), LOG_SQRT_2PI = 0.91893853320467274178f, LOG2 = 0.69314718055994530942f;
  const float* hd = head + i * 2 * A;
  float lp = 0.f, ladj = 0.f;
  for (int j = 0; j < A; ++j) {
    const float raw = hd[A + j];
    const bool in_range = raw >= -20.f && raw <= 2.f;
    const float ls = fminf(fmaxf(raw, -20.f), 2.f), sd = expf(ls), var = sd * sd;
    const float x = atanhf(fminf(fmaxf(tr[off_action + j], A_LO), A_HI));
    const float diff = x - hd[j];
    lp += -(diff * diff) / (2.f * var) - logf(sd) - LOG_SQRT_2PI;
    ladj += 2.f * (LOG2 - x - softplusf(-2.f * x));
    dhead[i * 2 * A + j] = c * diff / var;
    dhead[i * 2 * A + A + j] = in_range ? c * (diff * diff / var - 1.f) : 0.f;
  }
  if (row_loss) row_loss[i] = -w * ((0.f - ladj) + lp);
}

__global__ void row_mean_kernel(const float* __restrict__ x, float* __restrict__ out, int B) {
  __shared__ float red[32];
  float s = 0.f;
  for (int b = threadIdx.x; b < B; b += blockDim.x) s += x[(int64_t)blockIdx.x * B + b];
  s = block_sum(s, red);
  if (threadIdx.x == 0) out[blockIdx.x] = s / (float)B;
}

struct SacWs {
  MlpActs actor_acts, critic_acts;
  float *head, *q, *xn, *y, *lp_next, *dq, *dxa, *dhead, *tmpA, *tmpB, *g_actor, *g_critic;
  int64_t bytes;
};

int64_t carve(char*& p, int64_t floats) {
  const int64_t b = il_align_up(floats * 4, 256);
  p += b;
  return b;
}

SacWs sac_layout(const il_sac_args* a, char* base) {
  SacWs w{};
  const int R = a->R, B = a->batch.B, A = a->batch.A, d = a->batch.S + a->batch.A;
  char* p = base;
  p = mlp_acts_carve(&a->actor, R, B, p, &w.actor_acts);
  p = mlp_acts_carve(&a->critic, 2 * R, B, p, &w.critic_acts);
  auto take = [&](int64_t floats) { float* r = reinterpret_cast<float*>(p); carve(p, floats); return r; };
  w.head = take((int64_t)R * B * 2 * A);
  w.q = take((int64_t)2 * R * B);
  w.xn = take((int64_t)R * B * d);
  w.y = take((int64_t)R * B);
  w.lp_next = take((int64_t)R * B);
  w.dq = take((int64_t)2 * R * B);
  w.dxa = take((int64_t)2 * R * B * A);
  w.dhead = take((int64_t)R * B * 2 * A);
  int hmax = mlp_max_hidden(&a->critic);
  if (mlp_max_hidden(&a->actor) > hmax) hmax = mlp_max_hidden(&a->actor);
  w.tmpA = take((int64_t)2 * R * B * hmax);
  w.tmpB = take((int64_t)2 * R * B * hmax);
  w.g_actor = take((int64_t)R * a->actor.stride);
  w.g_critic = take((int64_t)2 * R * a->critic.stride);
  w.bytes = p - base;
  return w;
}

}

extern "C" int64_t il_sac_workspace_bytes(const il_sac_args* a) {
  if (!a) return -1;
  return sac_layout(a, nullptr).bytes;
}

extern "C" int il_sac_update(il_handle* h, const il_sac_args* a, void* stream) {
  IL_CHECK(h && a, "il_sac_update: null argument");
  cudaStream_t st = (cudaStream_t)stream;
  const int R = a->R, B = a->batch.B, S = a->batch.S, A = a->batch.A, d = S + A;
  IL_CHECK(R > 0 && B > 0 && S > 0 && A > 0, "il_sac_update: R=%d B=%d S=%d A=%d", R, B, S, A);
  IL_TRY(mlp_validate(&a->actor, "il_sac_update(actor)"));
  IL_TRY(mlp_validate(&a->critic, "il_sac_update(critic)"));
  IL_TRY(mlp_validate(&a->target, "il_sac_update(target)"));
  IL_CHECK(a->actor.dims[0] == S && a->actor.dims[a->actor.n_layers] == 2 * A, "il_sac_update: actor dims do not match S=%d A=%d", S, A);
  IL_CHECK(a->critic.dims[0] == d && a->critic.dims[a->critic.n_layers] == 1, "il_sac_update: critic dims do not match S+A=%d", d);
  IL_CHECK(a->target.n_layers == a->critic.n_layers && a->target.stride == a->critic.stride, "il_sac_update: target/critic layout mismatch");
  const RowLayout L = row_layout(S, A);
  IL_CHECK(a->batch.row == L.len, "il_sac_update: batch row length %d != %d", a->batch.row, L.len);
  IL_CHECK(a->batch.rows && a->log_alpha && a->eps_next && a->eps_new && a->workspace, "il_sac_update: null buffer");
  IL_CHECK(a->workspace_bytes >= il_sac_workspace_bytes(a), "il_sac_update: workspace too small (%lld < %lld)", (long long)a->workspace_bytes,
           (long long)il_sac_workspace_bytes(a));
  IL_CHECK(!(a->actor_opt.lr_r || a->actor_opt.weight_decay_r) || a->actor_opt.replica_floats == a->actor.stride, "il_sac_update: actor_opt.replica_floats must be the actor stride");
  IL_CHECK(!(a->critic_opt.lr_r || a->critic_opt.weight_decay_r || a->polyak_r) || a->critic_opt.replica_floats == 2 * a->critic.stride,
           "il_sac_update: critic_opt.replica_floats must be 2 x the critic stride");
  SacWs w = sac_layout(a, static_cast<char*>(a->workspace));
  const float* rows = a->batch.rows;
  const int64_t rs = a->batch.replica_stride;
  const int row = L.len;
  AbsView av{nullptr, 0, 0};
  if (a->absorbing) av = AbsView{a->absorbing, (int64_t)B, 1};
  else if (a->absorbing_from_state) av = AbsView{rows + L.state + (S - 1), rs, row};
  const unsigned ew = (unsigned)(((int64_t)R * B + 127) / 128);

  IL_TRY(launch_tick(h, a->actor_opt.step, a->critic_opt.step, a->alpha_opt.step, st));

  IL_TRY(mlp_forward(h, &a->actor, R, B, MatView{rows + L.next_state, rs, 1, row}, w.actor_acts, w.head, (int64_t)B * 2 * A, 2 * A, st, false));
  {
    HeadFwdArgs ha{};
    ha.head = w.head; ha.eps = a->eps_next;
    ha.action = w.xn + S; ha.action_rs = (int64_t)B * d; ha.ld_action = d;
    ha.zero_mask = av.ptr; ha.zero_mask_rs = av.rs; ha.zero_mask_ld = av.ld;
    ha.log_prob = w.lp_next;
    ha.copy_src = rows + L.next_state; ha.copy_rs = rs; ha.copy_ld = row; ha.copy_cols = S;
    ha.R = R; ha.n = B; ha.A = A;
    IL_TRY(launch_actor_head(h, ha, st));
  }
  IL_TRY(mlp_forward(h, &a->target, 2 * R, B, MatView{w.xn, (int64_t)B * d, 2, d}, w.critic_acts, w.q, (int64_t)B, 1, st, false));
  IL_LAUNCH(h, sac_target_kernel, ew, 128, 0, st, w.q, w.lp_next, a->log_alpha, rows, rs, row, L.reward, L.terminal, av, a->discount, a->discount_r, w.y, R, B);
  IL_TRY(mlp_forward(h, &a->critic, 2 * R, B, MatView{rows + L.state, rs, 2, row}, w.critic_acts, w.q, (int64_t)B, 1, st));
  IL_LAUNCH(h, sac_critic_lossgrad_kernel, R, 256, 0, st, w.q, w.y, rows, rs, row, L.weight, w.dq, a->out_q_values, a->out_losses, B);
  IL_TRY(mlp_backward(h, &a->critic, 2 * R, B, MatView{rows + L.state, rs, 2, row}, w.critic_acts, MatView{w.dq, (int64_t)B, 1, 1}, w.g_critic, a->critic.stride, nullptr, 0,
                      0, 0, 0, w.tmpA, w.tmpB, st));
  IL_TRY(launch_adam(h, a->critic.params, w.g_critic, &a->critic_opt, (int64_t)2 * R * a->critic.stride, st, a->target.params, a->polyak_factor, a->polyak_r));
  IL_TRY(mlp_forward(h, &a->actor, R, B, MatView{rows + L.state, rs, 1, row}, w.actor_acts, w.head, (int64_t)B * 2 * A, 2 * A, st));
  {
    HeadFwdArgs ha{};
    ha.head = w.head; ha.eps = a->eps_new;
    ha.action = w.xn + S; ha.action_rs = (int64_t)B * d; ha.ld_action = d;
    ha.log_prob = a->out_log_probs ? a->out_log_probs : w.lp_next;
    ha.copy_src = rows + L.state; ha.copy_rs = rs; ha.copy_ld = row; ha.copy_cols = S;
    ha.R = R; ha.n = B; ha.A = A;
    IL_TRY(launch_actor_head(h, ha, st));
  }
  const float* lp_new = a->out_log_probs ? a->out_log_probs : w.lp_next;
  IL_TRY(mlp_forward(h, &a->critic, 2 * R, B, MatView{w.xn, (int64_t)B * d, 2, d}, w.critic_acts, w.q, (int64_t)B, 1, st, MLP_KEEP_MASKS));
  IL_LAUNCH(h, sac_actor_loss_kernel, R, 256, 0, st, w.q, lp_new, a->log_alpha, rows, rs, row, L.weight, av, w.dq, a->out_losses, B);
  IL_TRY(mlp_backward(h, &a->critic, 2 * R, B, MatView{w.xn, (int64_t)B * d, 2, d}, w.critic_acts, MatView{w.dq, (int64_t)B, 1, 1}, nullptr, 0, w.dxa, (int64_t)B * A, A, S,
                      A, w.tmpA, w.tmpB, st));
  IL_LAUNCH(h, sac_head_backward_kernel, ew, 128, 0, st, w.head, a->eps_new, w.xn, d, S, w.dxa, a->log_alpha, rows, rs, row, L.weight, av, w.dhead, R, B, A);
  IL_TRY(mlp_backward(h, &a->actor, R, B, MatView{rows + L.state, rs, 1, row}, w.actor_acts, MatView{w.dhead, (int64_t)B * 2 * A, 1, 2 * A}, w.g_actor, a->actor.stride,
                      nullptr, 0, 0, 0, 0, w.tmpA, w.tmpB, st));
  IL_TRY(launch_adam(h, a->actor.params, w.g_actor, &a->actor_opt, (int64_t)R * a->actor.stride, st));
  IL_LAUNCH(h, sac_alpha_kernel, R, 256, 0, st, a->log_alpha, lp_new, rows, rs, row, L.weight, av, a->entropy_target, a->entropy_target_r, a->alpha_opt.m, a->alpha_opt.v,
            a->alpha_opt.step, a->alpha_opt.lr, a->alpha_opt.lr_r, a->alpha_opt.beta1, a->alpha_opt.beta2, a->alpha_opt.eps, a->alpha_opt.weight_decay, a->alpha_opt.weight_decay_r,
            a->out_losses, B);
  return 0;
}

namespace {
struct BcWs {
  MlpActs acts;
  float *head, *dhead, *row_loss, *tmpA, *tmpB, *grads;
  int64_t bytes;
};
BcWs bc_layout(const il_bc_args* a, char* base) {
  BcWs w{};
  const int R = a->R, B = a->batch.B, A = a->batch.A;
  char* p = mlp_acts_carve(&a->actor, R, B, base, &w.acts);
  auto take = [&](int64_t floats) { float* r = reinterpret_cast<float*>(p); carve(p, floats); return r; };
  w.head = take((int64_t)R * B * 2 * A);
  w.dhead = take((int64_t)R * B * 2 * A);
  w.row_loss = take((int64_t)R * B);
  const int hmax = mlp_max_hidden(&a->actor);
  w.tmpA = take((int64_t)R * B * hmax);
  w.tmpB = take((int64_t)R * B * hmax);
  w.grads = take((int64_t)R * a->actor.stride);
  w.bytes = p - base;
  return w;
}
}

int bc_head_backward_launch(il_handle* h, const float* head, const il_batch* batch, float* dhead, float* row_loss, int R, cudaStream_t st) {
  const RowLayout L = row_layout(batch->S, batch->A);
  IL_LAUNCH(h, bc_head_backward_kernel, (unsigned)(((int64_t)R * batch->B + 127) / 128), 128, 0, st, head, batch->rows, batch->replica_stride, L.len, L.action, L.weight, dhead, row_loss, R,
            batch->B, batch->A);
  return 0;
}
int bc_row_mean_launch(il_handle* h, const float* row_loss, float* out_loss, int R, int B, cudaStream_t st) {
  IL_LAUNCH(h, row_mean_kernel, R, 256, 0, st, row_loss, out_loss, B);
  return 0;
}

extern "C" int64_t il_bc_workspace_bytes(const il_bc_args* a) { return a ? bc_layout(a, nullptr).bytes : -1; }

extern "C" int il_bc_update(il_handle* h, const il_bc_args* a, void* stream) {
  IL_CHECK(h && a, "il_bc_update: null argument");
  cudaStream_t st = (cudaStream_t)stream;
  const int R = a->R, B = a->batch.B, S = a->batch.S, A = a->batch.A;
  IL_TRY(mlp_validate(&a->actor, "il_bc_update(actor)"));
  IL_CHECK(R > 0 && B > 0 && a->actor.dims[0] == S && a->actor.dims[a->actor.n_layers] == 2 * A, "il_bc_update: actor dims do not match the batch");
  const RowLayout L = row_layout(S, A);
  IL_CHECK(a->batch.rows && a->batch.row == L.len && a->workspace && a->workspace_bytes >= il_bc_workspace_bytes(a), "il_bc_update: bad batch / workspace");
  BcWs w = bc_layout(a, static_cast<char*>(a->workspace));
  const MatView X{a->batch.rows + L.state, a->batch.replica_stride, 1, L.len};
  IL_TRY(launch_tick(h, a->opt.step, nullptr, nullptr, st));
  IL_TRY(mlp_forward(h, &a->actor, R, B, X, w.acts, w.head, (int64_t)B * 2 * A, 2 * A, st));
  IL_LAUNCH(h, bc_head_backward_kernel, (unsigned)(((int64_t)R * B + 127) / 128), 128, 0, st, w.head, a->batch.rows, a->batch.replica_stride, L.len, L.action, L.weight, w.dhead,
            a->out_loss ? w.row_loss : nullptr, R, B, A);
  if (a->out_loss) IL_LAUNCH(h, row_mean_kernel, R, 256, 0, st, w.row_loss, a->out_loss, B);
  IL_TRY(mlp_backward(h, &a->actor, R, B, X, w.acts, MatView{w.dhead, (int64_t)B * 2 * A, 1, 2 * A}, w.grads, a->actor.stride, nullptr, 0, 0, 0, 0, w.tmpA, w.tmpB, st));
  return launch_adam(h, a->actor.params, w.grads, &a->opt, (int64_t)R * a->actor.stride, st);
}
```

### imitation-learning_b200/csrc/tc_gemm.cu

```cuda
#include "common.cuh"
#include <cstdio>
#include <cstdlib>

namespace {

constexpr int BM = 128, BN = 256, BK = 16;
constexpr int THREADS = 256;
constexpr int A_BYTES = BM * BK * 4, B_BYTES = BN * BK * 4;
constexpr int A_HI = 0, A_LO = A_BYTES, B_HI = 2 * A_BYTES, B_LO = 2 * A_BYTES + B_BYTES;
constexpr int STAGE_BYTES = 2 * (A_BYTES + B_BYTES);
constexpr int N_STAGES = 3;
constexpr int RAW_STAGES = 3;
constexpr int HEAD_MAX = 8;
constexpr int HEAD_BYTES = (BN + HEAD_MAX * BN) * 4;
constexpr int L1_MAXK = 16, L1_ROWS = 256;
constexpr int L1_W_BYTES = L1_ROWS * L1_MAXK * 4, L1_B_BYTES = L1_ROWS * 4, L1_X_BYTES = BM * L1_MAXK * 4;
constexpr int raw_a_bytes(bool fuse) { return fuse ? 0 : A_BYTES; }
constexpr int raw_bytes(bool fuse) { return raw_a_bytes(fuse) + B_BYTES; }
constexpr int RAW_OFF = N_STAGES * STAGE_BYTES;
constexpr int head_off(bool fuse) { return RAW_OFF + RAW_STAGES * raw_bytes(fuse); }
constexpr int l1_off(bool fuse) { return head_off(fuse) + HEAD_BYTES; }
constexpr int smem_bytes(bool fuse) { return 1024 + l1_off(fuse) + (fuse ? L1_W_BYTES + L1_B_BYTES + L1_X_BYTES : 0); }
static_assert(smem_bytes(false) <= 227 * 1024 && smem_bytes(true) <= 227 * 1024, "tc_gemm: shared memory over the 227 KB per-CTA limit");

__device__ __forceinline__ uint32_t smem_u32(const void* p) { return (uint32_t)__cvta_generic_to_shared(p); }
__device__ __forceinline__ void fence_proxy_async() { asm volatile("fence.proxy.async.shared::cta;" ::: "memory"); }
__device__ __forceinline__ void wgmma_fence() { asm volatile("wgmma.fence.sync.aligned;" ::: "memory"); }
__device__ __forceinline__ void wgmma_commit() { asm volatile("wgmma.commit_group.sync.aligned;" ::: "memory"); }
template <int N>
__device__ __forceinline__ void wgmma_wait() { asm volatile("wgmma.wait_group.sync.aligned %0;" ::"n"(N) : "memory"); }
__device__ __forceinline__ void cp_async16(uint32_t dst, const float* src) { asm volatile("cp.async.cg.shared.global [%0], [%1], 16;" ::"r"(dst), "l"(src) : "memory"); }
__device__ __forceinline__ void cp_async_commit() { asm volatile("cp.async.commit_group;" ::: "memory"); }
template <int N>
__device__ __forceinline__ void cp_async_wait() { asm volatile("cp.async.wait_group %0;" ::"n"(N) : "memory"); }
__device__ __forceinline__ void wgmma_tf32(float (&d)[128], uint64_t a_desc, uint64_t b_desc) {
  asm volatile(
      "wgmma.mma_async.sync.aligned.m64n256k8.f32.tf32.tf32 {"
      "%0, %1, %2, %3, %4, %5, %6, %7, %8, %9, %10, %11, %12, %13, %14, %15, "
      "%16, %17, %18, %19, %20, %21, %22, %23, %24, %25, %26, %27, %28, %29, %30, %31, "
      "%32, %33, %34, %35, %36, %37, %38, %39, %40, %41, %42, %43, %44, %45, %46, %47, "
      "%48, %49, %50, %51, %52, %53, %54, %55, %56, %57, %58, %59, %60, %61, %62, %63, "
      "%64, %65, %66, %67, %68, %69, %70, %71, %72, %73, %74, %75, %76, %77, %78, %79, "
      "%80, %81, %82, %83, %84, %85, %86, %87, %88, %89, %90, %91, %92, %93, %94, %95, "
      "%96, %97, %98, %99, %100, %101, %102, %103, %104, %105, %106, %107, %108, %109, %110, %111, "
      "%112, %113, %114, %115, %116, %117, %118, %119, %120, %121, %122, %123, %124, %125, %126, %127 "
      "}, %128, %129, 1, 1, 1;"
      : "+f"(d[0]), "+f"(d[1]), "+f"(d[2]), "+f"(d[3]), "+f"(d[4]), "+f"(d[5]), "+f"(d[6]), "+f"(d[7]),
        "+f"(d[8]), "+f"(d[9]), "+f"(d[10]), "+f"(d[11]), "+f"(d[12]), "+f"(d[13]), "+f"(d[14]), "+f"(d[15]),
        "+f"(d[16]), "+f"(d[17]), "+f"(d[18]), "+f"(d[19]), "+f"(d[20]), "+f"(d[21]), "+f"(d[22]), "+f"(d[23]),
        "+f"(d[24]), "+f"(d[25]), "+f"(d[26]), "+f"(d[27]), "+f"(d[28]), "+f"(d[29]), "+f"(d[30]), "+f"(d[31]),
        "+f"(d[32]), "+f"(d[33]), "+f"(d[34]), "+f"(d[35]), "+f"(d[36]), "+f"(d[37]), "+f"(d[38]), "+f"(d[39]),
        "+f"(d[40]), "+f"(d[41]), "+f"(d[42]), "+f"(d[43]), "+f"(d[44]), "+f"(d[45]), "+f"(d[46]), "+f"(d[47]),
        "+f"(d[48]), "+f"(d[49]), "+f"(d[50]), "+f"(d[51]), "+f"(d[52]), "+f"(d[53]), "+f"(d[54]), "+f"(d[55]),
        "+f"(d[56]), "+f"(d[57]), "+f"(d[58]), "+f"(d[59]), "+f"(d[60]), "+f"(d[61]), "+f"(d[62]), "+f"(d[63]),
        "+f"(d[64]), "+f"(d[65]), "+f"(d[66]), "+f"(d[67]), "+f"(d[68]), "+f"(d[69]), "+f"(d[70]), "+f"(d[71]),
        "+f"(d[72]), "+f"(d[73]), "+f"(d[74]), "+f"(d[75]), "+f"(d[76]), "+f"(d[77]), "+f"(d[78]), "+f"(d[79]),
        "+f"(d[80]), "+f"(d[81]), "+f"(d[82]), "+f"(d[83]), "+f"(d[84]), "+f"(d[85]), "+f"(d[86]), "+f"(d[87]),
        "+f"(d[88]), "+f"(d[89]), "+f"(d[90]), "+f"(d[91]), "+f"(d[92]), "+f"(d[93]), "+f"(d[94]), "+f"(d[95]),
        "+f"(d[96]), "+f"(d[97]), "+f"(d[98]), "+f"(d[99]), "+f"(d[100]), "+f"(d[101]), "+f"(d[102]), "+f"(d[103]),
        "+f"(d[104]), "+f"(d[105]), "+f"(d[106]), "+f"(d[107]), "+f"(d[108]), "+f"(d[109]), "+f"(d[110]), "+f"(d[111]),
        "+f"(d[112]), "+f"(d[113]), "+f"(d[114]), "+f"(d[115]), "+f"(d[116]), "+f"(d[117]), "+f"(d[118]), "+f"(d[119]),
        "+f"(d[120]), "+f"(d[121]), "+f"(d[122]), "+f"(d[123]), "+f"(d[124]), "+f"(d[125]), "+f"(d[126]), "+f"(d[127])
      : "l"(a_desc), "l"(b_desc));
}
__device__ __forceinline__ uint64_t make_desc(uint32_t smem_addr) {
  return (uint64_t)((smem_addr >> 4) & 0x3FFF) | ((uint64_t)1 << 16) | ((uint64_t)(512 >> 4) << 32) | ((uint64_t)2 << 62);
}
__device__ __forceinline__ uint32_t sw64(int r, int c) { return (uint32_t)((r >> 3) * 512 + (r & 7) * 64 + ((c ^ ((r >> 1) & 3)) << 4)); }
__device__ __forceinline__ void sts128(uint32_t addr, uint32_t x, uint32_t y, uint32_t z, uint32_t w) {
  asm volatile("st.shared.v4.b32 [%0], {%1, %2, %3, %4};" ::"r"(addr), "r"(x), "r"(y), "r"(z), "r"(w) : "memory");
}
__device__ __forceinline__ uint4 lds128(uint32_t addr) {
  uint4 v;
  asm volatile("ld.shared.v4.b32 {%0, %1, %2, %3}, [%4];" : "=r"(v.x), "=r"(v.y), "=r"(v.z), "=r"(v.w) : "r"(addr));
  return v;
}
__device__ __forceinline__ uint32_t hi_of(uint32_t x) { return x & 0xFFFFE000u; }
__device__ __forceinline__ uint32_t lo_of(uint32_t x) { return __float_as_uint(__uint_as_float(x) - __uint_as_float(x & 0xFFFFE000u)); }
__device__ __forceinline__ void store_chunk(uint32_t hi_tile, uint32_t lo_tile, uint32_t off, uint4 v, bool split) {
  sts128(hi_tile + off, hi_of(v.x), hi_of(v.y), hi_of(v.z), hi_of(v.w));
  if (split) sts128(lo_tile + off, lo_of(v.x), lo_of(v.y), lo_of(v.z), lo_of(v.w));
}
__device__ __forceinline__ void store_block_t(uint32_t hi_tile, uint32_t lo_tile, int c4, int kg, const uint4 (&v)[4], bool split) {
  uint4 q0 = make_uint4(v[0].x, v[1].x, v[2].x, v[3].x), q1 = make_uint4(v[0].y, v[1].y, v[2].y, v[3].y);
  uint4 q2 = make_uint4(v[0].z, v[1].z, v[2].z, v[3].z), q3 = make_uint4(v[0].w, v[1].w, v[2].w, v[3].w);
  const int s = (c4 >> 1) & 3;
  if (s & 1) { const uint4 t = q0; q0 = q1; q1 = q2; q2 = q3; q3 = t; }
  if (s & 2) { uint4 t = q0; q0 = q2; q2 = t; t = q1; q1 = q3; q3 = t; }
  store_chunk(hi_tile, lo_tile, sw64(4 * c4 + (s & 3), kg), q0, split);
  store_chunk(hi_tile, lo_tile, sw64(4 * c4 + ((s + 1) & 3), kg), q1, split);
  store_chunk(hi_tile, lo_tile, sw64(4 * c4 + ((s + 2) & 3), kg), q2, split);
  store_chunk(hi_tile, lo_tile, sw64(4 * c4 + ((s + 3) & 3), kg), q3, split);
}

struct TcParams {
  GemmArgs g;
  int tiles_m;
  int split;
  const float* head_w;
  const float* head_b;
  float* head_out;
  int64_t head_gs, head_out_gs;
  int head_n, store_c;
  int head_js, head_ns;
  TcFuseL1 l1;
};

template <int EPI, bool FUSE = false>
__global__ void __launch_bounds__(THREADS, 1) tc_gemm_kernel(const TcParams p) {
  extern __shared__ uint8_t smem_raw[];
  uint8_t* smem = reinterpret_cast<uint8_t*>((reinterpret_cast<uintptr_t>(smem_raw) + 1023) & ~(uintptr_t)1023);
  float* head_s = reinterpret_cast<float*>(smem + head_off(FUSE));
  const uint32_t stage0 = smem_u32(smem), raw0 = stage0 + RAW_OFF;
  const uint32_t w1s = stage0 + l1_off(FUSE), b1s = w1s + L1_W_BYTES, xs = b1s + L1_B_BYTES;
  constexpr uint32_t RAW_A = 0, RAW_B = raw_a_bytes(FUSE), RAW_BYTES = raw_bytes(FUSE);

  const int tid = threadIdx.x, warp = tid >> 5, lane = tid & 31, wg = tid >> 7;
  const GemmArgs& g = p.g;
  const int nkb = g.K / BK, tiles_m = p.tiles_m;
  const int my_tiles = (g.G * tiles_m - (int)blockIdx.x + (int)gridDim.x - 1) / (int)gridDim.x;
  const int nq = my_tiles * nkb;
  const bool a_km = FUSE || g.a_kmajor != 0, b_km = g.b_kmajor != 0, split = p.split != 0;

  const int fr = tid >> 2, fc = tid & 3;
  const int a_c4 = tid & 31, a_kg = (tid >> 5) & 3, b_c4 = tid & 63, b_kg = tid >> 6;
  const uint32_t km_off = sw64(fr, fc);
  auto tile_of = [&](int i) { return (int)blockIdx.x + i * (int)gridDim.x; };

  auto copy_kb = [&](int q) {
    if (q < nq) {
      const int t = tile_of(q / nkb), kb = q % nkb, grp = t / tiles_m, m0 = (t % tiles_m) * BM;
      const uint32_t raw = raw0 + (uint32_t)(q % RAW_STAGES) * RAW_BYTES + (uint32_t)tid * 16u;
      if (!FUSE) {
        const float* A = g.A + (int64_t)(grp / g.a_gdiv) * g.a_gs;
        if (a_km) {
          const float* src = A + (int64_t)(m0 + fr) * g.lda + kb * BK + fc * 4;
          cp_async16(raw + RAW_A, src);
          cp_async16(raw + RAW_A + THREADS * 16, src + (int64_t)64 * g.lda);
        } else if (wg == 0) {
          const float* src = A + (int64_t)(kb * BK + a_kg * 4) * g.lda + m0 + a_c4 * 4;
#pragma unroll
          for (int k = 0; k < 4; ++k) cp_async16(raw + RAW_A + k * (THREADS / 2) * 16, src + (int64_t)k * g.lda);
        }
      }
      const float* Bg = g.B + (int64_t)(grp / g.b_gdiv) * g.b_gs;
      const float* src = b_km ? Bg + (int64_t)fr * g.ldb + kb * BK + fc * 4 : Bg + (int64_t)(kb * BK + b_kg * 4) * g.ldb + b_c4 * 4;
      const int64_t step = b_km ? (int64_t)64 * g.ldb : (int64_t)g.ldb;
#pragma unroll
      for (int j = 0; j < 4; ++j) cp_async16(raw + RAW_B + j * THREADS * 16, src + j * step);
    }
    cp_async_commit();
  };

  auto split_kb = [&](int q) {
    const uint32_t st = stage0 + (uint32_t)(q % N_STAGES) * STAGE_BYTES;
    const uint32_t raw = raw0 + (uint32_t)(q % RAW_STAGES) * RAW_BYTES + (uint32_t)tid * 16u;
    if (FUSE) {
      const int kb = q % nkb, k0 = kb * BK + fc * 4;
      const uint4 bq = lds128(b1s + (uint32_t)k0 * 4u);
      float c0[4] = {__uint_as_float(bq.x), __uint_as_float(bq.y), __uint_as_float(bq.z), __uint_as_float(bq.w)};
      float c1[4] = {c0[0], c0[1], c0[2], c0[3]};
      const int np = (p.l1.x_k + 3) >> 2;
#pragma unroll
      for (int c4 = 0; c4 < L1_MAXK / 4; ++c4) {
        if (c4 < np) {
          const uint4 x0 = lds128(xs + sw64(fr, c4)), x1 = lds128(xs + sw64(fr + 64, c4));
#pragma unroll
          for (int qq = 0; qq < 4; ++qq) {
            const uint4 w = lds128(w1s + (uint32_t)((k0 + qq) * 64 + ((c4 ^ fc) << 4)));
            c0[qq] = fmaf(__uint_as_float(x0.x), __uint_as_float(w.x), c0[qq]); c1[qq] = fmaf(__uint_as_float(x1.x), __uint_as_float(w.x), c1[qq]);
            c0[qq] = fmaf(__uint_as_float(x0.y), __uint_as_float(w.y), c0[qq]); c1[qq] = fmaf(__uint_as_float(x1.y), __uint_as_float(w.y), c1[qq]);
            c0[qq] = fmaf(__uint_as_float(x0.z), __uint_as_float(w.z), c0[qq]); c1[qq] = fmaf(__uint_as_float(x1.z), __uint_as_float(w.z), c1[qq]);
            c0[qq] = fmaf(__uint_as_float(x0.w), __uint_as_float(w.w), c0[qq]); c1[qq] = fmaf(__uint_as_float(x1.w), __uint_as_float(w.w), c1[qq]);
          }
        }
      }
      const uint4 a0 = make_uint4(__float_as_uint(fmaxf(c0[0], 0.f)), __float_as_uint(fmaxf(c0[1], 0.f)), __float_as_uint(fmaxf(c0[2], 0.f)), __float_as_uint(fmaxf(c0[3], 0.f)));
      const uint4 a1 = make_uint4(__float_as_uint(fmaxf(c1[0], 0.f)), __float_as_uint(fmaxf(c1[1], 0.f)), __float_as_uint(fmaxf(c1[2], 0.f)), __float_as_uint(fmaxf(c1[3], 0.f)));
      store_chunk(st + A_HI, st + A_LO, km_off, a0, split);
      store_chunk(st + A_HI, st + A_LO, km_off + 4096u, a1, split);
      if (p.l1.store) {
        const int t = tile_of(q / nkb);
        float* hs = p.l1.store + (int64_t)(t / tiles_m) * p.l1.store_gs + (int64_t)((t % tiles_m) * BM + fr) * g.K + k0;
        *reinterpret_cast<uint4*>(hs) = a0;
        *reinterpret_cast<uint4*>(hs + (int64_t)64 * g.K) = a1;
      }
    } else if (a_km) {
      store_chunk(st + A_HI, st + A_LO, km_off, lds128(raw + RAW_A), split);
      store_chunk(st + A_HI, st + A_LO, km_off + 4096u, lds128(raw + RAW_A + THREADS * 16), split);
    } else if (wg == 0) {
      uint4 v[4];
#pragma unroll
      for (int k = 0; k < 4; ++k) v[k] = lds128(raw + RAW_A + k * (THREADS / 2) * 16);
      store_block_t(st + A_HI, st + A_LO, a_c4, a_kg, v, split);
    }
    if (b_km) {
#pragma unroll
      for (int j = 0; j < 4; ++j) store_chunk(st + B_HI, st + B_LO, km_off + (uint32_t)j * 4096u, lds128(raw + RAW_B + j * THREADS * 16), split);
    } else {
      uint4 v[4];
#pragma unroll
      for (int k = 0; k < 4; ++k) v[k] = lds128(raw + RAW_B + k * THREADS * 16);
      store_block_t(st + B_HI, st + B_LO, b_c4, b_kg, v, split);
    }
  };

  auto stage_l1 = [&](int t) {
    const int grp = t / tiles_m, m0 = (t % tiles_m) * BM, xk = p.l1.x_k;
    const float* w1 = p.l1.w1 + (int64_t)grp * p.l1.gs;
    const float* b1 = p.l1.b1 + (int64_t)grp * p.l1.gs;
    const float* x = p.l1.x + (int64_t)(grp / p.l1.x_gdiv) * p.l1.x_gs + (int64_t)m0 * p.l1.x_ld;
    float* w1f = reinterpret_cast<float*>(smem + l1_off(FUSE));
    float* b1f = reinterpret_cast<float*>(smem + l1_off(FUSE) + L1_W_BYTES);
    float* xf = reinterpret_cast<float*>(smem + l1_off(FUSE) + L1_W_BYTES + L1_B_BYTES);
    for (int i = tid; i < L1_ROWS * L1_MAXK; i += THREADS) {
      const int k = i / L1_MAXK, j = i % L1_MAXK;
      w1f[k * L1_MAXK + ((((j >> 2) ^ ((k >> 2) & 3)) << 2) | (j & 3))] = (k < g.K && j < xk) ? __ldg(w1 + (int64_t)k * xk + j) : 0.f;
    }
    for (int i = tid; i < L1_ROWS; i += THREADS) b1f[i] = i < g.K ? __ldg(b1 + i) : 0.f;
    for (int i = tid; i < BM * L1_MAXK; i += THREADS) {
      const int r = i / L1_MAXK, j = i % L1_MAXK;
      xf[(sw64(r, j >> 2) >> 2) + (j & 3)] = j < xk ? __ldg(x + (int64_t)r * p.l1.x_ld + j) : 0.f;
    }
  };

#pragma unroll 1
  for (int q = 0; q < RAW_STAGES; ++q) copy_kb(q);
  if (FUSE) {
    stage_l1(tile_of(0));
    __syncthreads();
  }
  cp_async_wait<RAW_STAGES - 1>();
  split_kb(0);
  copy_kb(RAW_STAGES);
  fence_proxy_async();
  __syncthreads();
  const uint64_t a_desc0 = make_desc(stage0 + (uint32_t)wg * 4096u), b_desc0 = make_desc(stage0);

  float acc[128];
#pragma unroll 1
  for (int i = 0, q = 0; i < my_tiles; ++i) {
#pragma unroll
    for (int j = 0; j < 128; ++j) acc[j] = 0.f;
#pragma unroll 1
    for (int kb = 0; kb < nkb; ++kb, ++q) {
      const uint32_t cur = (uint32_t)(q % N_STAGES) * STAGE_BYTES;
      wgmma_fence();
#pragma unroll
      for (int kk = 0; kk < BK / 8; ++kk) {
        const uint32_t o = cur + kk * 32;
        const uint64_t ah = a_desc0 + ((o + A_HI) >> 4), al = a_desc0 + ((o + A_LO) >> 4), bh = b_desc0 + ((o + B_HI) >> 4), bl = b_desc0 + ((o + B_LO) >> 4);
        if (split) {
          wgmma_tf32(acc, al, bh);
          wgmma_tf32(acc, ah, bl);
        }
        wgmma_tf32(acc, ah, bh);
      }
      wgmma_commit();
      if (q + 1 < nq) {
        if (FUSE && kb == nkb - 1) {
          stage_l1(tile_of(i + 1));
          __syncthreads();
        }
        cp_async_wait<RAW_STAGES - 1>();
        split_kb(q + 1);
      }
      copy_kb(q + 1 + RAW_STAGES);
      wgmma_wait<1>();
      fence_proxy_async();
      __syncthreads();
    }

    const int t = tile_of(i), grp = t / tiles_m, m0 = (t % tiles_m) * BM;
    if (EPI == 4 || EPI == 6) {
      const float* wsrc = p.head_w + (int64_t)grp * p.head_gs;
      if (EPI == 4) head_s[tid] = __ldg(g.bias + (int64_t)grp * g.bias_gs + tid);
#pragma unroll
      for (int j = 0; j < HEAD_MAX; ++j)
        if (j < p.head_n) head_s[BN + j * BN + tid] = __ldg(wsrc + (int64_t)j * p.head_js + (int64_t)tid * p.head_ns);
    }
    wgmma_wait<0>();
    if (EPI == 4 || EPI == 6) __syncthreads();
    const int r0 = m0 + wg * 64 + (warp & 3) * 16 + (lane >> 2), cl = (lane & 3) * 2;
    float* C = g.C + (int64_t)grp * g.c_gs + (int64_t)r0 * g.ldc + cl;
    const int64_t c8 = (int64_t)8 * g.ldc;
    const float* bias = (EPI == 1 || (EPI == 3 && g.bias)) ? g.bias + (int64_t)grp * g.bias_gs + cl : nullptr;
    const float* mask = (EPI == 2 || (EPI == 3 && g.mask)) ? g.mask + (int64_t)grp * g.mask_gs + (int64_t)r0 * g.ldmask + cl : nullptr;
    const int64_t m8 = (int64_t)8 * g.ldmask;
    const uint32_t* mbits = (EPI == 5 || EPI == 6) ? g.mask_bits + (int64_t)grp * g.mask_bits_gs + (int64_t)r0 * (BN / 32) : nullptr;
    uint32_t word0 = 0, word1 = 0;
#pragma unroll
    for (int c = 0; c < BN / 8; ++c) {
      float v00 = acc[4 * c], v01 = acc[4 * c + 1], v10 = acc[4 * c + 2], v11 = acc[4 * c + 3];
      const int col = 8 * c, bit = (c & 3) * 8 + cl;
      if (EPI == 5 || EPI == 6) {
        if ((c & 3) == 0) { word0 = __ldg(mbits + (c >> 2)); word1 = __ldg(mbits + 8 * (BN / 32) + (c >> 2)); }
        v00 = (word0 >> bit) & 1u ? v00 : 0.f; v01 = (word0 >> (bit + 1)) & 1u ? v01 : 0.f;
        v10 = (word1 >> bit) & 1u ? v10 : 0.f; v11 = (word1 >> (bit + 1)) & 1u ? v11 : 0.f;
      }
      if (EPI == 4) {
        const float2 b = *reinterpret_cast<const float2*>(head_s + col + cl);
        v00 = fmaxf(v00 + b.x, 0.f); v01 = fmaxf(v01 + b.y, 0.f); v10 = fmaxf(v10 + b.x, 0.f); v11 = fmaxf(v11 + b.y, 0.f);
        if (g.bits_out) {
          if ((c & 3) == 0) word0 = word1 = 0;
          word0 |= (v00 > 0.f ? 1u : 0u) << bit | (v01 > 0.f ? 1u : 0u) << (bit + 1);
          word1 |= (v10 > 0.f ? 1u : 0u) << bit | (v11 > 0.f ? 1u : 0u) << (bit + 1);
          if ((c & 3) == 3) {
            word0 |= __shfl_xor_sync(0xffffffffu, word0, 1); word0 |= __shfl_xor_sync(0xffffffffu, word0, 2);
            word1 |= __shfl_xor_sync(0xffffffffu, word1, 1); word1 |= __shfl_xor_sync(0xffffffffu, word1, 2);
            if ((lane & 3) == 0) {
              uint32_t* bo = g.bits_out + (int64_t)grp * g.bits_out_gs + (int64_t)r0 * (BN / 32) + (c >> 2);
              bo[0] = word0;
              bo[8 * (BN / 32)] = word1;
            }
          }
        }
      }
      if (EPI == 4 || EPI == 6) {
        acc[4 * c] = v00; acc[4 * c + 1] = v01; acc[4 * c + 2] = v10; acc[4 * c + 3] = v11;
        if (!p.store_c) continue;
      }
      if (EPI == 1) {
        const float2 b = __ldg(reinterpret_cast<const float2*>(bias + col));
        v00 = fmaxf(v00 + b.x, 0.f); v01 = fmaxf(v01 + b.y, 0.f); v10 = fmaxf(v10 + b.x, 0.f); v11 = fmaxf(v11 + b.y, 0.f);
      } else if (EPI == 2) {
        const float2 ma = __ldg(reinterpret_cast<const float2*>(mask + col)), mb = __ldg(reinterpret_cast<const float2*>(mask + m8 + col));
        v00 = ma.x > 0.f ? v00 : 0.f; v01 = ma.y > 0.f ? v01 : 0.f; v10 = mb.x > 0.f ? v10 : 0.f; v11 = mb.y > 0.f ? v11 : 0.f;
      } else if (EPI == 3) {
        if (bias) {
          const float2 b = __ldg(reinterpret_cast<const float2*>(bias + col));
          v00 += b.x; v01 += b.y; v10 += b.x; v11 += b.y;
        }
        if (g.act >= 0) { v00 = act_apply(v00, g.act); v01 = act_apply(v01, g.act); v10 = act_apply(v10, g.act); v11 = act_apply(v11, g.act); }
        if (mask) {
          const float2 ma = __ldg(reinterpret_cast<const float2*>(mask + col)), mb = __ldg(reinterpret_cast<const float2*>(mask + m8 + col));
          v00 *= act_grad_from_output(ma.x, g.mask_act); v01 *= act_grad_from_output(ma.y, g.mask_act);
          v10 *= act_grad_from_output(mb.x, g.mask_act); v11 *= act_grad_from_output(mb.y, g.mask_act);
        }
      }
      *reinterpret_cast<float2*>(C + col) = make_float2(v00, v01);
      *reinterpret_cast<float2*>(C + c8 + col) = make_float2(v10, v11);
    }
    if (EPI == 4 || EPI == 6) {
      float* ho = p.head_out + (int64_t)grp * p.head_out_gs + (int64_t)r0 * p.head_n;
      const float* hb = p.head_b ? p.head_b + (int64_t)grp * p.head_gs : nullptr;
#pragma unroll 1
      for (int j = 0; j < HEAD_MAX; ++j) {
        if (j < p.head_n) {
          float s0 = 0.f, s1 = 0.f;
#pragma unroll
          for (int c = 0; c < BN / 8; ++c) {
            const float2 w = *reinterpret_cast<const float2*>(head_s + BN + j * BN + 8 * c + cl);
            s0 = fmaf(acc[4 * c], w.x, s0); s0 = fmaf(acc[4 * c + 1], w.y, s0);
            s1 = fmaf(acc[4 * c + 2], w.x, s1); s1 = fmaf(acc[4 * c + 3], w.y, s1);
          }
          s0 += __shfl_xor_sync(0xffffffffu, s0, 1); s0 += __shfl_xor_sync(0xffffffffu, s0, 2);
          s1 += __shfl_xor_sync(0xffffffffu, s1, 1); s1 += __shfl_xor_sync(0xffffffffu, s1, 2);
          if ((lane & 3) == 0) {
            const float b = hb ? __ldg(hb + j) : 0.f;
            ho[j] = s0 + b;
            ho[(int64_t)8 * p.head_n + j] = s1 + b;
          }
        }
      }
    }
  }
  cp_async_wait<0>();
}

__global__ void colsum_kernel(const float* __restrict__ A, int64_t a_gs, int a_gdiv, int lda, int K, int M, float* __restrict__ out, int64_t out_gs) {
  const int g = blockIdx.y, m = blockIdx.x * blockDim.x + threadIdx.x;
  if (m >= M) return;
  const float* a = A + (int64_t)(g / a_gdiv) * a_gs + m;
  float s = 0.f;
  for (int k = 0; k < K; ++k) s += a[(int64_t)k * lda];
  out[(int64_t)g * out_gs + m] = s;
}

}

bool tc_gemm_eligible(const GemmArgs& a) {
  auto al16 = [](const void* p) { return (reinterpret_cast<uintptr_t>(p) & 15) == 0; };
  if (a.M % BM != 0 || a.N != BN || a.K % BK != 0 || a.accumulate) return false;
  if (a.a_kmajor == 0 && a.b_kmajor != 0) return false;
  if (!al16(a.A) || !al16(a.B) || !al16(a.C) || a.lda % 4 || a.ldb % 4 || a.ldc % 4 || a.a_gs % 4 || a.b_gs % 4 || a.c_gs % 4) return false;
  if (a.bias && (!al16(a.bias) || a.bias_gs % 4)) return false;
  if (a.mask && (!al16(a.mask) || a.ldmask % 4 || a.mask_gs % 4)) return false;
  return true;
}

template <int EPI, bool FUSE = false>
int tc_set_attr() {
  IL_CUDA(cudaFuncSetAttribute(tc_gemm_kernel<EPI, FUSE>, cudaFuncAttributeMaxDynamicSharedMemorySize, smem_bytes(FUSE)));
  return 0;
}

int tc_gemm_init() {
  IL_TRY((tc_set_attr<0>())); IL_TRY((tc_set_attr<1>())); IL_TRY((tc_set_attr<2>())); IL_TRY((tc_set_attr<3>())); IL_TRY((tc_set_attr<4>()));
  IL_TRY((tc_set_attr<4, true>())); IL_TRY((tc_set_attr<5>())); IL_TRY((tc_set_attr<6>()));
  return 0;
}

template <int EPI, bool FUSE = false>
static int tc_launch(il_handle* h, TcParams& p, cudaStream_t stream) {
  const GemmArgs& a = p.g;
  p.tiles_m = a.M / BM;
  const int tiles = a.G * p.tiles_m, wave = h->sm_count >= p.tiles_m ? h->sm_count / p.tiles_m * p.tiles_m : h->sm_count;
  IL_LAUNCH(h, (tc_gemm_kernel<EPI, FUSE>), tiles < wave ? tiles : wave, THREADS, smem_bytes(FUSE), stream, p);
  return 0;
}

bool tc_head_fusable(const il_handle* h, const GemmArgs& a, int head_n) {
  return h->gemm_mode != IL_GEMM_FP32 && tc_gemm_eligible(a) && a.bias && a.act == IL_ACT_RELU && !a.mask && !a.colsum && head_n >= 1 && head_n <= HEAD_MAX;
}

bool tc_l1_fusable(const il_handle* h, const GemmArgs& a, int x_k) {
  return h->tc_fuse_l1 && tc_gemm_eligible(a) && x_k >= 1 && x_k <= L1_MAXK && a.K <= L1_ROWS && a.a_kmajor;
}

int launch_tc_gemm_head(il_handle* h, const GemmArgs& a, const float* head_w, const float* head_b, int64_t head_gs, int head_n, float* head_out, int64_t head_out_gs, int store_c,
                        cudaStream_t stream, const TcFuseL1* l1) {
  IL_CHECK(tc_head_fusable(h, a, head_n), "tc_gemm_head: not fusable");
  TcParams p{};
  p.g = a;
  p.split = h->gemm_mode == IL_GEMM_TF32X3 ? 1 : 0;
  p.head_w = head_w; p.head_b = head_b; p.head_out = head_out; p.head_gs = head_gs; p.head_out_gs = head_out_gs; p.head_n = head_n; p.store_c = store_c;
  p.head_js = BN; p.head_ns = 1;
  double bytes = gemm_algorithmic_bytes(a, store_c != 0) + 4.0 * a.G * (double)a.M * head_n, flops = 2.0 * a.M * a.N * a.K * a.G;
  if (l1) {
    IL_CHECK(tc_l1_fusable(h, a, l1->x_k), "tc_gemm_head: first layer not fusable (K0=%d)", l1->x_k);
    IL_CHECK(l1->x && l1->w1 && l1->b1 && (reinterpret_cast<uintptr_t>(l1->b1) & 15) == 0 && l1->gs % 4 == 0, "tc_gemm_head: bad first-layer buffers");
    IL_CHECK(!l1->store || ((reinterpret_cast<uintptr_t>(l1->store) & 15) == 0 && l1->store_gs % 4 == 0), "tc_gemm_head: unaligned hidden store");
    p.l1 = *l1;
    const double gx = (a.G + l1->x_gdiv - 1) / l1->x_gdiv;
    bytes += -4.0 * a.G * (double)a.M * a.K + 4.0 * (gx * a.M * l1->x_k + (double)a.G * a.K * (l1->x_k + 1)) + (l1->store ? 4.0 * a.G * (double)a.M * a.K : 0.0);
    flops += 2.0 * a.G * (double)a.M * a.K * l1->x_k;
  }
  auto run = [&]() { return l1 ? tc_launch<4, true>(h, p, stream) : tc_launch<4>(h, p, stream); };
  if (h->profiling) {
    ProfiledLaunch pl;
    IL_TRY(profile_open(h, &pl, flops, bytes, stream));
    const int rc = run();
    IL_TRY(profile_close(h, &pl, stream));
    return rc;
  }
  return run();
}

bool tc_dx_head_fusable(const il_handle* h, const GemmArgs& a, int head_n) {
  return h->gemm_mode != IL_GEMM_FP32 && a.M >= 128 && a.K >= 128 && tc_gemm_eligible(a) && a.mask_bits && !a.mask && !a.bias && a.act < 0 && !a.colsum && a.mask_act == IL_ACT_RELU &&
         head_n >= 1 && head_n <= HEAD_MAX;
}
int launch_tc_gemm_dx_head(il_handle* h, const GemmArgs& a, const float* w, int64_t w_gs, int w_ns, int head_n, float* out, int64_t out_gs, cudaStream_t stream) {
  IL_CHECK(tc_dx_head_fusable(h, a, head_n), "tc_gemm_dx_head: not fusable");
  TcParams p{};
  p.g = a;
  p.split = h->gemm_mode == IL_GEMM_TF32X3 ? 1 : 0;
  p.head_w = w; p.head_b = nullptr; p.head_out = out; p.head_gs = w_gs; p.head_out_gs = out_gs; p.head_n = head_n; p.store_c = 0;
  p.head_js = 1; p.head_ns = w_ns;
  const double bytes = gemm_algorithmic_bytes(a, false) + 4.0 * a.G * (double)a.M * head_n, flops = 2.0 * a.M * a.N * a.K * a.G;
  if (h->profiling) {
    ProfiledLaunch pl;
    IL_TRY(profile_open(h, &pl, flops, bytes, stream));
    const int rc = tc_launch<6>(h, p, stream);
    IL_TRY(profile_close(h, &pl, stream));
    return rc;
  }
  return tc_launch<6>(h, p, stream);
}

int launch_tc_gemm(il_handle* h, const GemmArgs& a, cudaStream_t stream) {
  IL_CHECK(tc_gemm_eligible(a), "tc_gemm: shape/layout not eligible (M=%d N=%d K=%d)", a.M, a.N, a.K);
  TcParams p{};
  p.g = a;
  p.split = h->gemm_mode == IL_GEMM_TF32X3 ? 1 : 0;
  const bool bits = a.mask_bits != nullptr;
  IL_CHECK(!bits || (!a.bias && a.act < 0 && a.mask_act == IL_ACT_RELU), "tc_gemm: sign-bit masks are the ReLU derivative of a plain product");
  if (bits) p.g.mask = nullptr;
  const bool plain = !a.bias && a.act < 0 && !a.mask && !bits;
  const bool bias_relu = a.bias && a.act == IL_ACT_RELU && !a.mask;
  const bool mask_relu = !a.bias && a.act < 0 && a.mask && a.mask_act == IL_ACT_RELU && !bits;
  if (bits) IL_TRY(tc_launch<5>(h, p, stream));
  else if (plain) IL_TRY(tc_launch<0>(h, p, stream));
  else if (bias_relu) IL_TRY(tc_launch<1>(h, p, stream));
  else if (mask_relu) IL_TRY(tc_launch<2>(h, p, stream));
  else IL_TRY(tc_launch<3>(h, p, stream));
  if (a.colsum) {
    dim3 cg((a.M + 127) / 128, a.G);
    IL_LAUNCH(h, colsum_kernel, cg, 128, 0, stream, a.A, a.a_gs, a.a_gdiv, a.lda, a.K, a.M, a.colsum, a.colsum_gs);
  }
  return 0;
}
```

### include/il_b200.h

```cpp
#ifndef IL_B200_H
#define IL_B200_H

#include <stdint.h>

#ifdef __cplusplus
extern "C" {
#endif

#define IL_MAX_LAYERS 6
#define IL_MAX_WIDTH_CLASSES 8

enum { IL_ACT_RELU = 0, IL_ACT_TANH = 1, IL_ACT_SIGMOID = 2 };
enum { IL_REWARD_AIRL = 0, IL_REWARD_GAIL = 1, IL_REWARD_FAIRL = 2 };
enum { IL_LOSS_BCE = 0, IL_LOSS_MIXUP = 1, IL_LOSS_PUGAIL = 2 };
enum { IL_GEMM_FP32 = 0, IL_GEMM_TF32X3 = 1, IL_GEMM_TF32 = 2 };

typedef struct il_handle il_handle;

typedef struct il_mlp {
  float*  params;
  int64_t stride;
  int32_t n_layers;
  int32_t activation;
  int32_t dims[IL_MAX_LAYERS + 1];
  int32_t _pad;
} il_mlp;

typedef struct il_adam {
  float*   m;
  float*   v;
  int64_t* step;
  double lr, beta1, beta2, eps, weight_decay;
  const double* lr_r;
  const double* weight_decay_r;
  int64_t replica_floats;
} il_adam;

typedef struct il_batch {
  float*  rows;
  int64_t replica_stride;
  int32_t B, S, A, row;
} il_batch;

typedef struct il_replay {
  float*   rows;
  int64_t  replica_stride;
  int32_t* idx;
  int32_t* full;
  int32_t* num_trajectories;
  int32_t  size, S, A, row;
  int32_t  absorbing;
  int32_t  shared;
} il_replay;

int         il_create(int device, il_handle** out);
int         il_destroy(il_handle* h);
const char* il_last_error(void);
int         il_version(void);
int         il_set_gemm_mode(il_handle* h, int mode);
int64_t     il_launch_count(il_handle* h);
int         il_set_option(il_handle* h, const char* name, int value);
int         il_struct_sizes(int32_t* out15);
int         il_mlp_param_offsets(const int32_t* dims, int n_layers, int64_t* w_off, int64_t* b_off, int64_t* total);
int         il_row_layout(int S, int A, int32_t* offsets8, int32_t* row_len);

int il_profile_begin(il_handle* h);
int il_profile_end(il_handle* h, double* total_ms, double* total_flops, int64_t* launches);
int il_profile_bytes(il_handle* h, double* total_bytes);

int il_debug_gemm(il_handle* h, int M, int N, int K, int G, const float* A, int64_t a_gs, int lda, int a_kmajor,
                  const float* B, int64_t b_gs, int ldb, int b_kmajor, float* C, int64_t c_gs, int ldc,
                  const float* bias, int64_t bias_gs, int act, const float* mask, int64_t mask_gs, int ldmask, int mask_act,
                  float* colsum, int64_t colsum_gs, void* stream);

int il_fill_normal(il_handle* h, float* out, int64_t n, uint64_t seed, uint64_t stream_id, const uint64_t* counter, void* stream);
int il_fill_uniform(il_handle* h, float* out, int64_t n, uint64_t seed, uint64_t stream_id, const uint64_t* counter, void* stream);
int il_counter_add(il_handle* h, uint64_t* counter, uint64_t inc, void* stream);
int il_fill_beta(il_handle* h, float* out, int R, int64_t n_per_replica, const float* alpha_r, uint64_t seed, uint64_t stream_id, const uint64_t* counter,
                 void* stream);

int64_t il_actor_workspace_bytes(const il_mlp* actor, int R, int n);
int il_actor_forward(il_handle* h, const il_mlp* actor, int R, int n,
                     const float* states, int64_t states_rs, int ld_states,
                     const float* eps, const float* given_action,
                     float* action, float* log_prob, float* mean, float* log_std,
                     void* workspace, int64_t workspace_bytes, void* stream);

int64_t il_critic_workspace_bytes(const il_mlp* critic, int R, int n);
int il_critic_forward(il_handle* h, const il_mlp* twin, int R, int n, int S,
                      const float* states, int64_t states_rs, int ld_states,
                      const float* actions, int64_t actions_rs, int ld_actions,
                      float* q1, float* q2, void* workspace, int64_t workspace_bytes, void* stream);

int il_polyak(il_handle* h, float* target, const float* online, int64_t n, float polyak_factor, void* stream);

typedef struct il_sac_args {
  il_mlp  actor, critic, target;
  il_adam actor_opt, critic_opt, alpha_opt;
  float*  log_alpha;
  il_batch batch;
  const float* absorbing;
  int32_t absorbing_from_state;
  int32_t R;
  const float* eps_next;
  const float* eps_new;
  float discount, entropy_target, polyak_factor;
  float _pad0;
  float* out_log_probs;
  float* out_q_values;
  float* out_losses;
  void*   workspace;
  int64_t workspace_bytes;
  const float* discount_r;
  const float* entropy_target_r;
  const float* polyak_r;
} il_sac_args;
int64_t il_sac_workspace_bytes(const il_sac_args* a);
int il_sac_update(il_handle* h, const il_sac_args* a, void* stream);

typedef struct il_bc_args {
  il_mlp   actor;
  il_adam  opt;
  il_batch batch;
  int32_t  R;
  int32_t  _pad;
  float*   out_loss;
  void*    workspace;
  int64_t  workspace_bytes;
} il_bc_args;
int64_t il_bc_workspace_bytes(const il_bc_args* a);
int il_bc_update(il_handle* h, const il_bc_args* a, void* stream);

int il_fill_dropout_mask(il_handle* h, float* out, int64_t n, float p, uint64_t seed, uint64_t stream_id, const uint64_t* counter, void* stream);
int64_t il_actor_dropout_workspace_bytes(const il_mlp* actor, int R, int n);
int il_actor_log_prob_dropout(il_handle* h, const il_mlp* actor, int R, int n, int repeat, const float* states, int64_t states_rs, int ld_states, const float* given_action,
                              const float* mask_in, const float* const* mask_hid, float* log_prob, void* workspace, int64_t workspace_bytes, void* stream);
int il_bc_update_dropout(il_handle* h, const il_bc_args* a, const float* mask_in, const float* const* mask_hid, void* stream);
int il_dril_reward(il_handle* h, const float* log_prob, int R, int B, int ensemble, const float* q, int q_shared, float* reward, int64_t reward_rs, int reward_ld, float* variance,
                   void* stream);

typedef struct il_red {
  il_mlp  predictor;
  il_mlp  target;
  float*  sigma;
  int32_t state_only, _pad;
} il_red;
typedef struct il_red_update_args {
  il_red   disc;
  il_adam  opt;
  il_batch batch;
  int32_t  R, _pad;
  const float* mask_in;
  const float* mask_hid[IL_MAX_LAYERS];
  float*   out_loss;
  void*    workspace;
  int64_t  workspace_bytes;
} il_red_update_args;
int64_t il_red_workspace_bytes(const il_red* disc, int R, int B);
int il_red_update(il_handle* h, const il_red_update_args* a, void* stream);
int il_red_sigma(il_handle* h, const il_red* disc, int R, const il_batch* batch, const float* mask_in, const float* const* mask_hid, void* workspace, int64_t workspace_bytes, void* stream);
int il_red_reward(il_handle* h, const il_red* disc, int R, const il_batch* batch, float* reward, int64_t reward_rs, int reward_ld, void* workspace, int64_t workspace_bytes, void* stream);

int il_adam_step(il_handle* h, float* params, const float* grads, const il_adam* opt, int64_t n, void* stream);
int il_adam_step_polyak(il_handle* h, float* params, const float* grads, const il_adam* opt, int64_t n, float* target, float polyak_factor, void* stream);
int il_adam_step_polyak_r(il_handle* h, float* params, const float* grads, const il_adam* opt, int64_t n, float* target, const float* polyak_r, void* stream);

int il_replay_append(il_handle* h, const il_replay* mem, int R, const float* step, const float* state, const float* action,
                     const float* reward, const float* next_state, const float* terminal, const float* timeout,
                     const int32_t* active, int wrap, void* stream);
int il_replay_transfer(il_handle* h, const il_replay* dst, int R, const il_replay* src, void* stream);
int il_replay_wrap_absorbing(il_handle* h, const il_replay* mem, int R, const int32_t* mask, void* stream);
int il_replay_sample_indices(il_handle* h, const il_replay* mem, int R, int n, int32_t* idx_out, const float* uniform,
                             uint64_t seed, uint64_t stream_id, const uint64_t* counter, void* stream);
int il_replay_gather(il_handle* h, const il_replay* mem, int R, const int32_t* idx, const il_batch* out, void* stream);
int il_mix_expert_rows(il_handle* h, const il_batch* batch, const il_batch* expert, int R, void* stream);

int il_adril_relabel(il_handle* h, const il_batch* batch, const il_batch* expert, int R, int balanced, int update_freq, int32_t* sample_expert_flag,
                     const float* step_f, float step_offset, const int32_t* num_trajectories, int trajectories_shared, int num_expert_trajectories, void* stream);

typedef struct il_gail {
  il_mlp  g;
  float*  u;
  float*  v;
  int32_t u_stride, v_stride;
  int32_t state_only;
  int32_t reward_function;
  const int32_t* reward_function_r;
  const int32_t* spectral_norm_r;
  int32_t n_width_classes;
  int32_t width_class_H[IL_MAX_WIDTH_CLASSES];
  int32_t width_class_begin[IL_MAX_WIDTH_CLASSES];
  int32_t _pad;
  const int32_t* replica_order;
} il_gail;
typedef struct il_gail_update_args {
  il_gail  disc;
  il_adam  opt;
  il_batch policy, expert;
  const float* eps_gp;
  const float* eps_mix;
  int32_t R;
  int32_t loss_function;
  int32_t training;
  int32_t _pad;
  float grad_penalty, entropy_bonus, pos_class_prior, nonnegative_margin;
  float* out_losses;
  void*   workspace;
  int64_t workspace_bytes;
  const float* grad_penalty_r;
  const float* entropy_bonus_r;
  const int32_t* loss_function_r;
  const float* pos_class_prior_r;
  const float* nonnegative_margin_r;
} il_gail_update_args;
int64_t il_gail_workspace_bytes(const il_gail_update_args* a);
int il_gail_update(il_handle* h, const il_gail_update_args* a, void* stream);
int il_gail_reward(il_handle* h, const il_gail* disc, int R, const il_batch* batch, float* reward, int64_t reward_rs, int reward_ld,
                   float* logits, void* stream);

typedef struct il_gailx {
  il_mlp  g;
  il_mlp  h;
  float*  g_u; float* g_v;
  float*  h_u; float* h_v;
  int32_t g_u_stride, g_v_stride, h_u_stride, h_v_stride;
  int32_t state_only;
  int32_t reward_function;
  int32_t subtract_log_policy;
  float   discount;
  const float* discount_r;
} il_gailx;
typedef struct il_gailx_update_args {
  il_gailx disc;
  il_adam  opt;
  int64_t  params_floats;
  il_batch policy, expert;
  const float* eps_gp;
  const float* eps_mix;
  const float* logp_policy;
  const float* logp_expert;
  const float* logp_mix;
  int32_t R, loss_function, training, _pad;
  float grad_penalty, entropy_bonus, pos_class_prior, nonnegative_margin;
  float* out_losses;
  void*   workspace;
  int64_t workspace_bytes;
  const float* grad_penalty_r;
  const float* entropy_bonus_r;
} il_gailx_update_args;
int64_t il_gailx_workspace_bytes(const il_gailx_update_args* a);
int il_gailx_update(il_handle* h, const il_gailx_update_args* a, void* stream);
int64_t il_gailx_reward_workspace_bytes(const il_gailx* disc, int R, int B);
int il_gailx_reward(il_handle* h, const il_gailx* disc, int R, const il_batch* batch, const float* log_policy, float* reward, int64_t reward_rs, int reward_ld,
                    float* logits, void* workspace, int64_t workspace_bytes, void* stream);
int il_gail_mix_batch(il_handle* h, const il_batch* expert, const il_batch* policy, const float* eps, int R, const il_batch* out, void* stream);

int64_t il_gmmil_workspace_bytes(int R, int B);
int il_gmmil_bandwidth(il_handle* h, int R, const il_batch* policy, const il_batch* expert, int state_only, float* gamma,
                       void* workspace, int64_t workspace_bytes, void* stream);
int il_gmmil_reward(il_handle* h, int R, const il_batch* policy, const il_batch* expert, int state_only, const float* gamma,
                    float* reward, int64_t reward_rs, int reward_ld, void* stream);

typedef struct il_pwil {
  const float* atoms;
  const float* scale;
  const float* offset;
  float*   weights;
  int32_t  N, d, S, A;
  int32_t  state_only, time_horizon;
  float    reward_scale, reward_bandwidth;
} il_pwil;
int il_pwil_reset(il_handle* h, const il_pwil* p, int R, const int32_t* mask, void* stream);
int il_pwil_reward(il_handle* h, const il_pwil* p, int R, const float* state, const float* action, float* reward,
                   const int32_t* active, void* stream);

typedef struct il_env {
  const float* M;
  const float* N;
  const float* c;
  const float* w_r;
  float*   x;
  int32_t* t;
  int32_t  obs, act, absorbing, max_episode_steps, early_termination;
  float    term_threshold;
} il_env;
int il_env_reset(il_handle* h, const il_env* env, int n_envs, const float* u, const int32_t* mask, float* state, const float* else_state, void* stream);
int il_env_step(il_handle* h, const il_env* env, int n_envs, const float* action, float* next_state, float* reward,
                int32_t* done, int32_t* timeout, float* terminal_f, float* timeout_f, const int32_t* frozen, void* stream);

int il_rollout_bookkeep(il_handle* h, int n_envs, const float* reward, const int32_t* done, float* running, float* last_return,
                        float* return_sum, int32_t* episodes, float* step_f, void* stream);

int il_eval_accumulate(il_handle* h, int n_envs, const float* reward, const int32_t* done, float* returns, int32_t* finished,
                       int32_t* n_unfinished, void* stream);
int il_return_stats(il_handle* h, const float* returns, int64_t n, float* out3, void* stream);

typedef struct il_eval_args {
  il_mlp   actor;
  il_env   env;
  int32_t  R, episodes;
  int32_t  max_steps;
  int32_t  traj_T;
  float*   state;
  float*   returns;
  float*   traj_states;
  float*   traj_actions;
  float*   traj_rewards;
  int32_t* traj_len;
  int64_t* out_counters;
  void*    workspace;
  int64_t  workspace_bytes;
} il_eval_args;
int64_t il_eval_workspace_bytes(const il_eval_args* a);
int il_eval_rollout(il_handle* h, const il_eval_args* a, void* stream);

int il_nccl_unique_id(uint8_t* out128);
int il_nccl_comm_create(const uint8_t* id128, int rank, int world, void** comm);
int il_nccl_comm_destroy(void* comm);
int il_return_allreduce(il_handle* h, void* nccl_comm, const float* returns, int64_t n, float* out3, void* stream);

#ifdef __cplusplus
}
#endif
#endif
```

Baseline: 79830.

## Fuse AdamW update into weight-gradient GEMM epilogue for hidden layers

For hidden layers whose weight-gradient GEMM runs on the wgmma tensor-core path, the gradient tile is staged in free shared-memory pipeline stages and the AdamW step (plus optional Polyak target update) is applied directly in the epilogue, so the gradient is never written out. The separate Adam kernel then updates only the remaining segments (first/last layers, biases) through a segment-index mapping. The aim is to remove the gradient store/reload and part of the standalone optimiser pass. In exchange the GEMM epilogue gets heavier, it loses the TMA Adam path for the remainder, and the bias colsum needs an extra kernel launch.

```diff
diff --git a/imitation-learning_b200/_lib.py b/imitation-learning_b200/_lib.py
--- a/imitation-learning_b200/_lib.py
+++ b/imitation-learning_b200/_lib.py
@@ -132,6 +132,7 @@
   'il_adam_step': (C.c_int, [vp, vp, vp, P(Adam), i64, vp]),
   'il_adam_step_polyak': (C.c_int, [vp, vp, vp, P(Adam), i64, vp, C.c_float, vp]),
   'il_adam_step_polyak_r': (C.c_int, [vp, vp, vp, P(Adam), i64, vp, vp, vp]),
+  'il_debug_gemm_adam': (C.c_int, [vp, C.c_int, C.c_int, C.c_int, C.c_int, vp, i64, C.c_int, C.c_int, vp, i64, C.c_int, C.c_int, vp, vp, i64, i64, P(Adam), vp, C.c_float, vp, vp]),
   'il_fill_dropout_mask': (C.c_int, [vp, vp, i64, f32, u64, u64, vp, vp]),
   'il_actor_dropout_workspace_bytes': (i64, [P(Mlp), C.c_int, C.c_int]),
   'il_actor_log_prob_dropout': (C.c_int, [vp, P(Mlp), C.c_int, C.c_int, C.c_int, vp, i64, C.c_int, vp, vp, P(vp), vp, vp, i64, vp]),
diff --git a/imitation-learning_b200/csrc/common.cuh b/imitation-learning_b200/csrc/common.cuh
--- a/imitation-learning_b200/csrc/common.cuh
+++ b/imitation-learning_b200/csrc/common.cuh
@@ -117,6 +117,22 @@
   return x > 20.f ? x : log1pf(expf(x));
 }
 __device__ __forceinline__ float sigmoidf(float x) { return 1.f / (1.f + expf(-x)); }
+
+struct AdamConst {
+  float w1, w2, beta2, eps;
+  float bc2_sqrt;
+};
+__device__ __forceinline__ AdamConst adam_const(double beta1_d, double beta2_d, double eps_d, double bc2_sqrt) {
+  return AdamConst{(float)(1.0 - beta1_d), (float)(1.0 - beta2_d), (float)beta2_d, (float)eps_d, (float)bc2_sqrt};
+}
+__device__ __forceinline__ void adamw_update(float& pi, float& mi, float& vi, float gi, float ss, float dc, bool wdf, const AdamConst& k) {
+  if (wdf) pi = __fmul_rn(pi, dc);
+  mi = __fadd_rn(mi, __fmul_rn(k.w1, __fsub_rn(gi, mi)));
+  vi = __fadd_rn(__fmul_rn(vi, k.beta2), __fmul_rn(__fmul_rn(k.w2, gi), gi));
+  const float denom = __fadd_rn(__fdiv_rn(sqrtf(vi), k.bc2_sqrt), k.eps);
+  pi = __fadd_rn(pi, __fmul_rn(-ss, __fdiv_rn(mi, denom)));
+}
+__device__ __forceinline__ float polyak_update(float ti, float pi, float tau, float one_minus_tau) { return __fadd_rn(__fmul_rn(ti, tau), __fmul_rn(one_minus_tau, pi)); }
 
 __device__ __forceinline__ float warp_sum(float v) {
 #pragma unroll
@@ -203,9 +219,24 @@
   float* store;
   int64_t store_gs;
 };
+struct TcAdam {
+  float* p;
+  float* m;
+  float* v;
+  float* target;
+  int64_t gs;
+  const int64_t* step;
+  double lr, beta1, beta2, eps, wd;
+  const double* lr_r;
+  const double* wd_r;
+  float tau;
+  const float* tau_r;
+  int nets_per_replica;
+};
 bool tc_head_fusable(const il_handle* h, const GemmArgs& a, int head_n);
 bool tc_l1_fusable(const il_handle* h, const GemmArgs& a, int x_k);
 bool tc_dx_head_fusable(const il_handle* h, const GemmArgs& a, int head_n);
 int launch_tc_gemm_dx_head(il_handle* h, const GemmArgs& a, const float* w, int64_t w_gs, int w_ns, int head_n, float* out, int64_t out_gs, cudaStream_t stream);
 int launch_tc_gemm_head(il_handle* h, const GemmArgs& a, const float* head_w, const float* head_b, int64_t head_gs, int head_n, float* head_out, int64_t head_out_gs, int store_c,
                         cudaStream_t stream, const TcFuseL1* l1 = nullptr);
+int launch_tc_gemm_adam(il_handle* h, const GemmArgs& a, const TcAdam& opt, cudaStream_t stream);
diff --git a/imitation-learning_b200/csrc/mlp.cu b/imitation-learning_b200/csrc/mlp.cu
--- a/imitation-learning_b200/csrc/mlp.cu
+++ b/imitation-learning_b200/csrc/mlp.cu
@@ -110,10 +110,24 @@
   return m->activation == IL_ACT_RELU && Nh <= HB_MAXN && H % 4 == 0 && n <= 1024 && grad_stride % 4 == 0 && m->stride % 4 == 0;
 }
 
+static TcAdam tc_adam_of(const il_adam* adam, float* params, int64_t gs, int64_t w_off, float* target, float tau, const float* tau_r) {
+  TcAdam t{};
+  t.p = params + w_off; t.m = adam->m + w_off; t.v = adam->v + w_off; t.target = target ? target + w_off : nullptr; t.gs = gs;
+  t.step = adam->step; t.lr = adam->lr; t.beta1 = adam->beta1; t.beta2 = adam->beta2; t.eps = adam->eps; t.wd = adam->weight_decay;
+  t.lr_r = adam->lr_r; t.wd_r = adam->weight_decay_r; t.tau = tau; t.tau_r = target ? tau_r : nullptr;
+  t.nets_per_replica = (t.lr_r || t.wd_r || t.tau_r) && adam->replica_floats >= gs ? (int)(adam->replica_floats / gs) : 1;
+  return t;
+}
+
 int mlp_backward(il_handle* h, const il_mlp* m, int G, int n, MatView X, const MlpActs& acts, MatView dOut, float* grads, int64_t grad_stride,
-                 float* dX, int64_t dx_gs, int ld_dx, int dx_col0, int dx_cols, float* tmpA, float* tmpB, cudaStream_t stream) {
+                 float* dX, int64_t dx_gs, int ld_dx, int dx_col0, int dx_cols, float* tmpA, float* tmpB, cudaStream_t stream, const MlpOptim* opt) {
   const MlpOffsets o = mlp_offsets(m->dims, m->n_layers);
   const int L = m->n_layers;
+  IL_CHECK(!opt || (grads && grad_stride == m->stride && opt->adam), "mlp_backward: the optimiser step needs the gradients in the parameter layout");
+  if (opt && (opt->adam->lr_r || opt->adam->weight_decay_r || (opt->target && opt->tau_r)))
+    IL_CHECK(opt->adam->replica_floats % m->stride == 0, "mlp_backward: replica_floats %lld is not a whole number of nets", (long long)opt->adam->replica_floats);
+  int64_t fused_off[IL_MAX_LAYERS], fused_len[IL_MAX_LAYERS];
+  int n_fused = 0;
   MatView dZ = dOut;
   float* next_tmp = tmpA;
   bool bias_done = false;
@@ -144,15 +158,17 @@
       next_tmp = next_tmp == tmpA ? tmpB : tmpA;
       continue;
     }
+    GemmArgs dw{};
+    bool fuse = false;
     if (grads) {
-      GemmArgs a{};
-      a.A = dZ.ptr; a.a_gs = dZ.gs; a.a_gdiv = dZ.gdiv; a.lda = dZ.ld; a.a_kmajor = 0;
-      a.B = Xin.ptr; a.b_gs = Xin.gs; a.b_gdiv = Xin.gdiv; a.ldb = Xin.ld; a.b_kmajor = 0;
-      a.C = grads + o.w[l]; a.c_gs = grad_stride; a.ldc = m->dims[l]; a.act = -1;
-      if (!bias_done) { a.colsum = grads + o.b[l]; a.colsum_gs = grad_stride; }
+      dw.A = dZ.ptr; dw.a_gs = dZ.gs; dw.a_gdiv = dZ.gdiv; dw.lda = dZ.ld; dw.a_kmajor = 0;
+      dw.B = Xin.ptr; dw.b_gs = Xin.gs; dw.b_gdiv = Xin.gdiv; dw.ldb = Xin.ld; dw.b_kmajor = 0;
+      dw.C = grads + o.w[l]; dw.c_gs = grad_stride; dw.ldc = m->dims[l]; dw.act = -1;
+      if (!bias_done) { dw.colsum = grads + o.b[l]; dw.colsum_gs = grad_stride; }
       bias_done = false;
-      a.M = m->dims[l + 1]; a.N = m->dims[l]; a.K = n; a.G = G;
-      IL_TRY(launch_gemm(h, a, stream));
+      dw.M = m->dims[l + 1]; dw.N = m->dims[l]; dw.K = n; dw.G = G;
+      fuse = opt && l > 0 && l < L - 1 && gemm_uses_tc(h, dw);
+      if (!fuse) IL_TRY(launch_gemm(h, dw, stream));
     }
     if (l > 0) {
       GemmArgs a{};
@@ -174,6 +190,10 @@
       IL_TRY(launch_gemm(h, a, stream));
       dZ = MatView{next_tmp, (int64_t)n * m->dims[l], 1, m->dims[l]};
       next_tmp = next_tmp == tmpA ? tmpB : tmpA;
+      if (fuse) {
+        IL_TRY(launch_tc_gemm_adam(h, dw, tc_adam_of(opt->adam, m->params, m->stride, o.w[l], opt->target, opt->tau, opt->tau_r), stream));
+        fused_off[n_fused] = o.w[l]; fused_len[n_fused++] = (int64_t)dw.M * dw.N;
+      }
     } else if (dX) {
       GemmArgs a{};
       a.A = dZ.ptr; a.a_gs = dZ.gs; a.a_gdiv = dZ.gdiv; a.lda = dZ.ld; a.a_kmajor = 1;
@@ -183,6 +203,8 @@
       IL_TRY(launch_gemm(h, a, stream));
     }
   }
+  if (opt)
+    IL_TRY(launch_adam_outside(h, m->params, grads, opt->adam, G, m->stride, fused_off, fused_len, n_fused, stream, opt->target, opt->tau, opt->target ? opt->tau_r : nullptr));
   return 0;
 }
 
@@ -414,9 +436,16 @@
   return r;
 }
 
+__device__ __forceinline__ int64_t adam_seg_index(int64_t f, const AdamSegs& s) {
+  const int64_t net = f / s.kept, local = f - net * s.kept;
+  int j = 0;
+  while (j + 1 < s.n_segs && local >= s.start[j + 1]) ++j;
+  return net * s.net_floats + s.off[j] + (local - s.start[j]);
+}
+
 __global__ void adam_kernel(float* __restrict__ p, const float* __restrict__ g, float* __restrict__ m, float* __restrict__ v, const int64_t* __restrict__ step,
                             double lr, double beta1_d, double beta2_d, double eps_d, double wd, int64_t n, float* __restrict__ target, float tau, float one_minus_tau,
-                            const AdamReplicas rp) {
+                            const AdamReplicas rp, const AdamSegs segs) {
   extern __shared__ AdamCoef adam_tab[];
   __shared__ float s_step_size, s_bc2_sqrt;
   if (threadIdx.x == 0) {
@@ -427,42 +456,36 @@
   }
   adam_fill_table(adam_tab, rp, lr, wd, beta1_d, step, tau);
   __syncthreads();
-  const float step_size = s_step_size, bc2_sqrt = s_bc2_sqrt;
-  const float decay = (float)(1.0 - lr * wd), w1 = (float)(1.0 - beta1_d), w2 = (float)(1.0 - beta2_d);
-  const float beta2 = (float)beta2_d, eps = (float)eps_d;
+  const float step_size = s_step_size;
+  const float decay = (float)(1.0 - lr * wd);
+  const AdamConst k = adam_const(beta1_d, beta2_d, eps_d, s_bc2_sqrt);
   const bool has_wd = wd != 0.0;
-  auto upd = [&](float& pi, float& mi, float& vi, float gi, float ss, float dc, bool wdf) {
-    if (wdf) pi = __fmul_rn(pi, dc);
-    mi = __fadd_rn(mi, __fmul_rn(w1, __fsub_rn(gi, mi)));
-    vi = __fadd_rn(__fmul_rn(vi, beta2), __fmul_rn(__fmul_rn(w2, gi), gi));
-    const float denom = __fadd_rn(__fdiv_rn(sqrtf(vi), bc2_sqrt), eps);
-    pi = __fadd_rn(pi, __fmul_rn(-ss, __fdiv_rn(mi, denom)));
-  };
-  const int64_t n4 = n >> 2;
-  for (int64_t i = (int64_t)blockIdx.x * blockDim.x + threadIdx.x; i < n4; i += (int64_t)gridDim.x * blockDim.x) {
+  const int64_t n4 = (segs.n_segs ? n / segs.net_floats * segs.kept : n) >> 2;
+  for (int64_t j = (int64_t)blockIdx.x * blockDim.x + threadIdx.x; j < n4; j += (int64_t)gridDim.x * blockDim.x) {
+    const int64_t f = segs.n_segs ? adam_seg_index(j << 2, segs) : j << 2, i = f >> 2;
     float ss = step_size, dc = decay, ta = tau, omt = one_minus_tau;
     bool wdf = has_wd;
     if (rp.R) {
-      const AdamCoef c = adam_tab[adam_replica(i << 2, rp)];
+      const AdamCoef c = adam_tab[adam_replica(f, rp)];
       ss = c.step_size; dc = c.decay; wdf = c.decay != 1.f; ta = c.tau; omt = c.one_minus_tau;
     }
     float4 pv = reinterpret_cast<float4*>(p)[i], mv = reinterpret_cast<float4*>(m)[i], vv = reinterpret_cast<float4*>(v)[i];
     const float4 gv = reinterpret_cast<const float4*>(g)[i];
-    upd(pv.x, mv.x, vv.x, gv.x, ss, dc, wdf); upd(pv.y, mv.y, vv.y, gv.y, ss, dc, wdf); upd(pv.z, mv.z, vv.z, gv.z, ss, dc, wdf); upd(pv.w, mv.w, vv.w, gv.w, ss, dc, wdf);
+    adamw_update(pv.x, mv.x, vv.x, gv.x, ss, dc, wdf, k); adamw_update(pv.y, mv.y, vv.y, gv.y, ss, dc, wdf, k);
+    adamw_update(pv.z, mv.z, vv.z, gv.z, ss, dc, wdf, k); adamw_update(pv.w, mv.w, vv.w, gv.w, ss, dc, wdf, k);
     reinterpret_cast<float4*>(p)[i] = pv; reinterpret_cast<float4*>(m)[i] = mv; reinterpret_cast<float4*>(v)[i] = vv;
     if (target) {
-      const float tau = ta, one_minus_tau = omt;
       float4 tv = reinterpret_cast<float4*>(target)[i];
-      tv.x = __fadd_rn(__fmul_rn(tv.x, tau), __fmul_rn(one_minus_tau, pv.x)); tv.y = __fadd_rn(__fmul_rn(tv.y, tau), __fmul_rn(one_minus_tau, pv.y));
-      tv.z = __fadd_rn(__fmul_rn(tv.z, tau), __fmul_rn(one_minus_tau, pv.z)); tv.w = __fadd_rn(__fmul_rn(tv.w, tau), __fmul_rn(one_minus_tau, pv.w));
+      tv.x = polyak_update(tv.x, pv.x, ta, omt); tv.y = polyak_update(tv.y, pv.y, ta, omt); tv.z = polyak_update(tv.z, pv.z, ta, omt); tv.w = polyak_update(tv.w, pv.w, ta, omt);
       reinterpret_cast<float4*>(target)[i] = tv;
     }
   }
+  if (segs.n_segs) return;
   for (int64_t i = (n4 << 2) + (int64_t)blockIdx.x * blockDim.x + threadIdx.x; i < n; i += (int64_t)gridDim.x * blockDim.x) {
     float pi = p[i], mi = m[i], vi = v[i];
-    upd(pi, mi, vi, g[i], step_size, decay, has_wd);
+    adamw_update(pi, mi, vi, g[i], step_size, decay, has_wd, k);
     p[i] = pi; m[i] = mi; v[i] = vi;
-    if (target) target[i] = __fadd_rn(__fmul_rn(target[i], tau), __fmul_rn(one_minus_tau, pi));
+    if (target) target[i] = polyak_update(target[i], pi, tau, one_minus_tau);
   }
 }
 
@@ -538,16 +561,10 @@
     asm volatile("cp.async.bulk.wait_group 0;" ::: "memory");
     return;
   }
-  const float step_size = s_step_size, bc2_sqrt = s_bc2_sqrt;
-  const float decay = (float)(1.0 - lr * wd), w1 = (float)(1.0 - beta1_d), w2 = (float)(1.0 - beta2_d), beta2 = (float)beta2_d, eps = (float)eps_d;
+  const float step_size = s_step_size;
+  const float decay = (float)(1.0 - lr * wd);
+  const AdamConst kc = adam_const(beta1_d, beta2_d, eps_d, s_bc2_sqrt);
   const bool has_wd = wd != 0.0;
-  auto upd = [&](float& pi, float& mi, float& vi, float gi, float ss, float dc, bool wdf) {
-    if (wdf) pi = __fmul_rn(pi, dc);
-    mi = __fadd_rn(mi, __fmul_rn(w1, __fsub_rn(gi, mi)));
-    vi = __fadd_rn(__fmul_rn(vi, beta2), __fmul_rn(__fmul_rn(w2, gi), gi));
-    const float denom = __fadd_rn(__fdiv_rn(sqrtf(vi), bc2_sqrt), eps);
-    pi = __fadd_rn(pi, __fmul_rn(-ss, __fdiv_rn(mi, denom)));
-  };
   for (int64_t k = 0; k < my_tiles; ++k) {
     const int stage = (int)(k % STAGES);
     const int64_t tile = blockIdx.x + k * gridDim.x;
@@ -567,13 +584,12 @@
       }
       float4 pv = sp[i], mv = smm[i], vv = sv[i];
       const float4 gv = sg[i];
-      upd(pv.x, mv.x, vv.x, gv.x, ss, dc, wdf); upd(pv.y, mv.y, vv.y, gv.y, ss, dc, wdf); upd(pv.z, mv.z, vv.z, gv.z, ss, dc, wdf); upd(pv.w, mv.w, vv.w, gv.w, ss, dc, wdf);
+      adamw_update(pv.x, mv.x, vv.x, gv.x, ss, dc, wdf, kc); adamw_update(pv.y, mv.y, vv.y, gv.y, ss, dc, wdf, kc);
+      adamw_update(pv.z, mv.z, vv.z, gv.z, ss, dc, wdf, kc); adamw_update(pv.w, mv.w, vv.w, gv.w, ss, dc, wdf, kc);
       sp[i] = pv; smm[i] = mv; sv[i] = vv;
       if (target) {
-        const float tau = ta, one_minus_tau = omt;
         float4 tv = stg[i];
-        tv.x = __fadd_rn(__fmul_rn(tv.x, tau), __fmul_rn(one_minus_tau, pv.x)); tv.y = __fadd_rn(__fmul_rn(tv.y, tau), __fmul_rn(one_minus_tau, pv.y));
-        tv.z = __fadd_rn(__fmul_rn(tv.z, tau), __fmul_rn(one_minus_tau, pv.z)); tv.w = __fadd_rn(__fmul_rn(tv.w, tau), __fmul_rn(one_minus_tau, pv.w));
+        tv.x = polyak_update(tv.x, pv.x, ta, omt); tv.y = polyak_update(tv.y, pv.y, ta, omt); tv.z = polyak_update(tv.z, pv.z, ta, omt); tv.w = polyak_update(tv.w, pv.w, ta, omt);
         stg[i] = tv;
       }
     }
@@ -729,7 +745,7 @@
 }
 
 int launch_adam(il_handle* h, float* params, const float* grads, const il_adam* opt, int64_t n, cudaStream_t stream, float* polyak_target, float polyak_factor,
-                const float* polyak_r) {
+                const float* polyak_r, const AdamSegs* segs) {
   IL_CHECK(opt->m && opt->v && opt->step, "adam: null state");
   IL_CHECK(((reinterpret_cast<uintptr_t>(params) | reinterpret_cast<uintptr_t>(grads) | reinterpret_cast<uintptr_t>(opt->m) | reinterpret_cast<uintptr_t>(opt->v) |
              reinterpret_cast<uintptr_t>(polyak_target)) & 15) == 0, "adam: buffers must be 16-byte aligned");
@@ -739,6 +755,16 @@
     IL_CHECK(rf > 0 && rf % 4 == 0 && n % rf == 0, "adam: per-replica hyper-parameters need replica_floats (%lld) > 0, a multiple of 4 dividing n = %lld", (long long)rf, (long long)n);
     IL_CHECK(n / rf <= ADAM_MAX_REPLICAS, "adam: %lld replicas with per-replica hyper-parameters exceed the limit of %d per buffer", (long long)(n / rf), ADAM_MAX_REPLICAS);
     rp.rf = rf; rp.inv_rf = 1.f / (float)rf; rp.R = (int)(n / rf);
+  }
+  AdamSegs sg{};
+  if (segs && segs->n_segs) {
+    sg = *segs;
+    IL_CHECK(sg.n_segs <= IL_MAX_LAYERS + 1 && sg.net_floats > 0 && sg.net_floats % 4 == 0 && n % sg.net_floats == 0 && sg.kept > 0 && sg.kept % 4 == 0,
+             "adam: bad segment list");
+    const int64_t n_up = n / sg.net_floats * sg.kept;
+    IL_LAUNCH(h, adam_kernel, ew_blocks(n_up / 4 + 1, 256, h->sm_count), 256, (size_t)rp.R * sizeof(AdamCoef), stream, params, grads, opt->m, opt->v, opt->step, opt->lr, opt->beta1,
+              opt->beta2, opt->eps, opt->weight_decay, n, polyak_target, polyak_factor, (float)(1.0 - (double)polyak_factor), rp, sg);
+    return 0;
   }
   if (h->adam_tma && n % 4 == 0 && n >= (int64_t)ADAM_TMA_MIN_TILES * h->sm_count * 2) {
     const int variant = h->adam_tma;
@@ -753,8 +779,33 @@
     }
   }
   IL_LAUNCH(h, adam_kernel, ew_blocks(n / 4 + 1, 256, h->sm_count), 256, (size_t)rp.R * sizeof(AdamCoef), stream, params, grads, opt->m, opt->v, opt->step, opt->lr, opt->beta1, opt->beta2,
-            opt->eps, opt->weight_decay, n, polyak_target, polyak_factor, (float)(1.0 - (double)polyak_factor), rp);
-  return 0;
+            opt->eps, opt->weight_decay, n, polyak_target, polyak_factor, (float)(1.0 - (double)polyak_factor), rp, sg);
+  return 0;
+}
+
+int launch_adam_outside(il_handle* h, float* params, const float* grads, const il_adam* opt, int G, int64_t net_floats, const int64_t* w_off, const int64_t* w_len, int n_fused,
+                        cudaStream_t stream, float* polyak_target, float polyak_factor, const float* polyak_r) {
+  const int64_t n = (int64_t)G * net_floats;
+  if (!n_fused) return launch_adam(h, params, grads, opt, n, stream, polyak_target, polyak_factor, polyak_r);
+  IL_CHECK(n_fused <= IL_MAX_LAYERS, "adam: %d fused windows", n_fused);
+  int64_t lo[IL_MAX_LAYERS], len[IL_MAX_LAYERS];
+  for (int i = 0; i < n_fused; ++i) {
+    int j = i;
+    for (; j > 0 && lo[j - 1] > w_off[i]; --j) { lo[j] = lo[j - 1]; len[j] = len[j - 1]; }
+    lo[j] = w_off[i]; len[j] = w_len[i];
+  }
+  AdamSegs s{};
+  s.net_floats = net_floats;
+  int64_t at = 0;
+  for (int i = 0; i <= n_fused; ++i) {
+    const int64_t end = i < n_fused ? lo[i] : net_floats;
+    IL_CHECK(end >= at && at % 4 == 0 && end % 4 == 0, "adam: fused windows overlap or are not 4-float aligned");
+    if (end > at) { s.off[s.n_segs] = at; s.start[s.n_segs] = s.kept; s.kept += end - at; ++s.n_segs; }
+    if (i < n_fused) at = lo[i] + len[i];
+  }
+  s.start[s.n_segs] = s.kept;
+  if (!s.n_segs) return 0;
+  return launch_adam(h, params, grads, opt, n, stream, polyak_target, polyak_factor, polyak_r, &s);
 }
 
 namespace {
@@ -852,6 +903,26 @@
   IL_CHECK(h && params && grads && opt && target && polyak_r, "il_adam_step_polyak_r: null argument");
   IL_TRY(launch_tick(h, opt->step, nullptr, nullptr, (cudaStream_t)stream));
   return launch_adam(h, params, grads, opt, n, (cudaStream_t)stream, target, 0.f, polyak_r);
+}
+
+extern "C" int il_debug_gemm_adam(il_handle* h, int M, int N, int K, int G, const float* A, int64_t a_gs, int lda, int a_kmajor, const float* B, int64_t b_gs, int ldb, int b_kmajor,
+                                  float* params, const float* grads, int64_t net_floats, int64_t w_off, const il_adam* opt, float* target, float polyak_factor, const float* polyak_r,
+                                  void* stream) {
+  IL_CHECK(h && A && B && params && grads && opt && opt->m && opt->v && opt->step, "il_debug_gemm_adam: null argument");
+  IL_CHECK(net_floats > 0 && w_off >= 0 && w_off + (int64_t)M * N <= net_floats, "il_debug_gemm_adam: window [%lld, %lld) outside a net of %lld floats", (long long)w_off,
+           (long long)(w_off + (int64_t)M * N), (long long)net_floats);
+  if (opt->lr_r || opt->weight_decay_r || (target && polyak_r))
+    IL_CHECK(opt->replica_floats % net_floats == 0, "il_debug_gemm_adam: replica_floats is not a whole number of nets");
+  GemmArgs a{};
+  a.A = A; a.a_gs = a_gs; a.a_gdiv = 1; a.lda = lda; a.a_kmajor = a_kmajor;
+  a.B = B; a.b_gs = b_gs; a.b_gdiv = 1; a.ldb = ldb; a.b_kmajor = b_kmajor;
+  a.ldc = N; a.act = -1; a.M = M; a.N = N; a.K = K; a.G = G;
+  IL_CHECK(gemm_uses_tc(h, a), "il_debug_gemm_adam: the product does not run on the wgmma engine (M=%d N=%d K=%d, gemm mode %d)", M, N, K, h->gemm_mode);
+  cudaStream_t st = (cudaStream_t)stream;
+  IL_TRY(launch_tick(h, opt->step, nullptr, nullptr, st));
+  IL_TRY(launch_tc_gemm_adam(h, a, tc_adam_of(opt, params, net_floats, w_off, target, polyak_factor, polyak_r), st));
+  const int64_t len = (int64_t)M * N;
+  return launch_adam_outside(h, params, grads, opt, G, net_floats, &w_off, &len, 1, st, target, polyak_factor, target ? polyak_r : nullptr);
 }
 
 extern "C" int il_polyak(il_handle* h, float* target, const float* online, int64_t n, float polyak_factor, void* stream) {
diff --git a/imitation-learning_b200/csrc/mlp.cuh b/imitation-learning_b200/csrc/mlp.cuh
--- a/imitation-learning_b200/csrc/mlp.cuh
+++ b/imitation-learning_b200/csrc/mlp.cuh
@@ -21,8 +21,15 @@
 int mlp_forward(il_handle* h, const il_mlp* m, int G, int n, MatView X, MlpActs& acts, float* out, int64_t out_gs, int ld_out,
                 cudaStream_t stream, int keep = MLP_KEEP_ALL);
 
+struct MlpOptim {
+  const il_adam* adam;
+  float* target;
+  float tau;
+  const float* tau_r;
+};
+
 int mlp_backward(il_handle* h, const il_mlp* m, int G, int n, MatView X, const MlpActs& acts, MatView dOut, float* grads, int64_t grad_stride,
-                 float* dX, int64_t dx_gs, int ld_dx, int dx_col0, int dx_cols, float* tmpA, float* tmpB, cudaStream_t stream);
+                 float* dX, int64_t dx_gs, int ld_dx, int dx_col0, int dx_cols, float* tmpA, float* tmpB, cudaStream_t stream, const MlpOptim* opt = nullptr);
 
 int mlp_small_forward(il_handle* h, const il_mlp* m, int G, int n, MatView X, float* out, cudaStream_t stream, int tanh_first = 0);
 int mlp_max_hidden(const il_mlp* m);
@@ -48,6 +55,13 @@
 };
 int launch_actor_head(il_handle* h, const HeadFwdArgs& a, cudaStream_t stream);
 
+struct AdamSegs {
+  int64_t net_floats, kept;
+  int n_segs;
+  int64_t off[IL_MAX_LAYERS + 1], start[IL_MAX_LAYERS + 2];
+};
 int launch_adam(il_handle* h, float* params, const float* grads, const il_adam* opt, int64_t n, cudaStream_t stream, float* polyak_target = nullptr, float polyak_factor = 0.f,
-                const float* polyak_r = nullptr);
+                const float* polyak_r = nullptr, const AdamSegs* segs = nullptr);
+int launch_adam_outside(il_handle* h, float* params, const float* grads, const il_adam* opt, int G, int64_t net_floats, const int64_t* w_off, const int64_t* w_len, int n_fused,
+                        cudaStream_t stream, float* polyak_target, float polyak_factor, const float* polyak_r);
 int launch_tick(il_handle* h, int64_t* s0, int64_t* s1, int64_t* s2, cudaStream_t stream);
diff --git a/imitation-learning_b200/csrc/sac.cu b/imitation-learning_b200/csrc/sac.cu
--- a/imitation-learning_b200/csrc/sac.cu
+++ b/imitation-learning_b200/csrc/sac.cu
@@ -243,9 +243,9 @@
   IL_LAUNCH(h, sac_target_kernel, ew, 128, 0, st, w.q, w.lp_next, a->log_alpha, rows, rs, row, L.reward, L.terminal, av, a->discount, a->discount_r, w.y, R, B);
   IL_TRY(mlp_forward(h, &a->critic, 2 * R, B, MatView{rows + L.state, rs, 2, row}, w.critic_acts, w.q, (int64_t)B, 1, st));
   IL_LAUNCH(h, sac_critic_lossgrad_kernel, R, 256, 0, st, w.q, w.y, rows, rs, row, L.weight, w.dq, a->out_q_values, a->out_losses, B);
+  const MlpOptim critic_opt{&a->critic_opt, a->target.params, a->polyak_factor, a->polyak_r};
   IL_TRY(mlp_backward(h, &a->critic, 2 * R, B, MatView{rows + L.state, rs, 2, row}, w.critic_acts, MatView{w.dq, (int64_t)B, 1, 1}, w.g_critic, a->critic.stride, nullptr, 0,
-                      0, 0, 0, w.tmpA, w.tmpB, st));
-  IL_TRY(launch_adam(h, a->critic.params, w.g_critic, &a->critic_opt, (int64_t)2 * R * a->critic.stride, st, a->target.params, a->polyak_factor, a->polyak_r));
+                      0, 0, 0, w.tmpA, w.tmpB, st, &critic_opt));
   IL_TRY(mlp_forward(h, &a->actor, R, B, MatView{rows + L.state, rs, 1, row}, w.actor_acts, w.head, (int64_t)B * 2 * A, 2 * A, st));
   {
     HeadFwdArgs ha{};
@@ -262,9 +262,9 @@
   IL_TRY(mlp_backward(h, &a->critic, 2 * R, B, MatView{w.xn, (int64_t)B * d, 2, d}, w.critic_acts, MatView{w.dq, (int64_t)B, 1, 1}, nullptr, 0, w.dxa, (int64_t)B * A, A, S,
                       A, w.tmpA, w.tmpB, st));
   IL_LAUNCH(h, sac_head_backward_kernel, ew, 128, 0, st, w.head, a->eps_new, w.xn, d, S, w.dxa, a->log_alpha, rows, rs, row, L.weight, av, w.dhead, R, B, A);
+  const MlpOptim actor_opt{&a->actor_opt, nullptr, 0.f, nullptr};
   IL_TRY(mlp_backward(h, &a->actor, R, B, MatView{rows + L.state, rs, 1, row}, w.actor_acts, MatView{w.dhead, (int64_t)B * 2 * A, 1, 2 * A}, w.g_actor, a->actor.stride,
-                      nullptr, 0, 0, 0, 0, w.tmpA, w.tmpB, st));
-  IL_TRY(launch_adam(h, a->actor.params, w.g_actor, &a->actor_opt, (int64_t)R * a->actor.stride, st));
+                      nullptr, 0, 0, 0, 0, w.tmpA, w.tmpB, st, &actor_opt));
   IL_LAUNCH(h, sac_alpha_kernel, R, 256, 0, st, a->log_alpha, lp_new, rows, rs, row, L.weight, av, a->entropy_target, a->entropy_target_r, a->alpha_opt.m, a->alpha_opt.v,
             a->alpha_opt.step, a->alpha_opt.lr, a->alpha_opt.lr_r, a->alpha_opt.beta1, a->alpha_opt.beta2, a->alpha_opt.eps, a->alpha_opt.weight_decay, a->alpha_opt.weight_decay_r,
             a->out_losses, B);
diff --git a/imitation-learning_b200/csrc/tc_gemm.cu b/imitation-learning_b200/csrc/tc_gemm.cu
--- a/imitation-learning_b200/csrc/tc_gemm.cu
+++ b/imitation-learning_b200/csrc/tc_gemm.cu
@@ -13,6 +13,8 @@
 constexpr int RAW_STAGES = 3;
 constexpr int HEAD_MAX = 8;
 constexpr int HEAD_BYTES = (BN + HEAD_MAX * BN) * 4;
+constexpr int ADAM_U = 4;
+static_assert(2 * STAGE_BYTES == 96 * BN * 4, "tc_gemm: the two free hi/lo stages hold 96 rows of the gradient tile");
 constexpr int L1_MAXK = 16, L1_ROWS = 256;
 constexpr int L1_W_BYTES = L1_ROWS * L1_MAXK * 4, L1_B_BYTES = L1_ROWS * 4, L1_X_BYTES = BM * L1_MAXK * 4;
 constexpr int raw_a_bytes(bool fuse) { return fuse ? 0 : A_BYTES; }
@@ -104,6 +106,7 @@
   int head_n, store_c;
   int head_js, head_ns;
   TcFuseL1 l1;
+  TcAdam opt;
 };
 
 template <int EPI, bool FUSE = false>
@@ -282,6 +285,75 @@
     wgmma_wait<0>();
     if (EPI == 4 || EPI == 6) __syncthreads();
     const int r0 = m0 + wg * 64 + (warp & 3) * 16 + (lane >> 2), cl = (lane & 3) * 2;
+    if (EPI == 7) {
+      const TcAdam& o = p.opt;
+      const int rep = grp / o.nets_per_replica;
+      const bool table = o.lr_r || o.wd_r || o.tau_r;
+      const double st = (double)*o.step, l = o.lr_r ? o.lr_r[rep] : o.lr, w = o.wd_r ? o.wd_r[rep] : o.wd;
+      const float ss = (float)(l / (1.0 - pow(o.beta1, st))), dc = w != 0.0 ? (float)(1.0 - l * w) : 1.f;
+      const bool wdf = table ? dc != 1.f : w != 0.0;
+      const float tau = o.tau_r ? o.tau_r[rep] : o.tau, omt = (float)(1.0 - (double)tau);
+      const AdamConst k = adam_const(o.beta1, o.beta2, o.eps, sqrt(1.0 - pow(o.beta2, st)));
+      const uint32_t sa = stage0 + (uint32_t)((q + 1) % N_STAGES) * STAGE_BYTES, sb = stage0 + (uint32_t)((q + 2) % N_STAGES) * STAGE_BYTES;
+      auto slot_of = [](int h, int row) { return h == 0 ? row : (row & 8) ? (row >> 4) * 8 + (row & 7) : 64 + (row >> 4) * 8 + (row & 7); };
+      auto saddr = [&](int h, int row, int byte) {
+        const int sl = slot_of(h, row);
+        return (sl < 48 ? sa + (uint32_t)sl * 1024u : sb + (uint32_t)(sl - 48) * 1024u) + (uint32_t)(byte ^ ((row & 7) << 5));
+      };
+      auto put = [&](int h, int row, int half) {
+#pragma unroll
+        for (int c = 0; c < BN / 8; ++c)
+          asm volatile("st.shared.v2.f32 [%0], {%1, %2};" ::"r"(saddr(h, row, (8 * c + cl) * 4)), "f"(acc[4 * c + 2 * half]), "f"(acc[4 * c + 2 * half + 1]) : "memory");
+      };
+      float* const tile_p[4] = {o.p, o.m, o.v, o.target};
+      const int64_t base = (int64_t)grp * o.gs + (int64_t)m0 * g.ldc;
+      auto stream = [&](int h) {
+        const int64_t blk = base + (int64_t)h * 64 * g.ldc;
+#pragma unroll 1
+        for (int i0 = tid; i0 < 64 * BN / 4; i0 += ADAM_U * THREADS) {
+          float4 v[ADAM_U][4];
+#pragma unroll
+          for (int u = 0; u < ADAM_U; ++u) {
+            const int i = i0 + u * THREADS;
+            const int64_t e = blk + (int64_t)(i >> 6) * g.ldc + 4 * (i & 63);
+#pragma unroll
+            for (int j = 0; j < 4; ++j)
+              if (j < 3 || tile_p[3]) v[u][j] = __ldcs(reinterpret_cast<const float4*>(tile_p[j] + e));
+          }
+#pragma unroll
+          for (int u = 0; u < ADAM_U; ++u) {
+            const int i = i0 + u * THREADS;
+            const int64_t e = blk + (int64_t)(i >> 6) * g.ldc + 4 * (i & 63);
+            const uint4 gq = lds128(saddr(h, i >> 6, 16 * (i & 63)));
+            float4 &pv = v[u][0], &mv = v[u][1], &vv = v[u][2], &tv = v[u][3];
+            adamw_update(pv.x, mv.x, vv.x, __uint_as_float(gq.x), ss, dc, wdf, k);
+            adamw_update(pv.y, mv.y, vv.y, __uint_as_float(gq.y), ss, dc, wdf, k);
+            adamw_update(pv.z, mv.z, vv.z, __uint_as_float(gq.z), ss, dc, wdf, k);
+            adamw_update(pv.w, mv.w, vv.w, __uint_as_float(gq.w), ss, dc, wdf, k);
+            __stcs(reinterpret_cast<float4*>(tile_p[0] + e), pv);
+            __stcs(reinterpret_cast<float4*>(tile_p[1] + e), mv);
+            __stcs(reinterpret_cast<float4*>(tile_p[2] + e), vv);
+            if (tile_p[3]) {
+              tv.x = polyak_update(tv.x, pv.x, tau, omt); tv.y = polyak_update(tv.y, pv.y, tau, omt);
+              tv.z = polyak_update(tv.z, pv.z, tau, omt); tv.w = polyak_update(tv.w, pv.w, tau, omt);
+              __stcs(reinterpret_cast<float4*>(tile_p[3] + e), tv);
+            }
+          }
+        }
+      };
+      const int lr = (warp & 3) * 16 + (lane >> 2);
+      __syncthreads();
+      if (wg == 0) { put(0, lr, 0); put(0, lr + 8, 1); }
+      else put(1, lr, 0);
+      __syncthreads();
+      stream(0);
+      __syncthreads();
+      if (wg == 1) put(1, lr + 8, 1);
+      __syncthreads();
+      stream(1);
+      __syncthreads();
+      continue;
+    }
     float* C = g.C + (int64_t)grp * g.c_gs + (int64_t)r0 * g.ldc + cl;
     const int64_t c8 = (int64_t)8 * g.ldc;
     const float* bias = (EPI == 1 || (EPI == 3 && g.bias)) ? g.bias + (int64_t)grp * g.bias_gs + cl : nullptr;
@@ -397,7 +469,7 @@
 
 int tc_gemm_init() {
   IL_TRY((tc_set_attr<0>())); IL_TRY((tc_set_attr<1>())); IL_TRY((tc_set_attr<2>())); IL_TRY((tc_set_attr<3>())); IL_TRY((tc_set_attr<4>()));
-  IL_TRY((tc_set_attr<4, true>())); IL_TRY((tc_set_attr<5>())); IL_TRY((tc_set_attr<6>()));
+  IL_TRY((tc_set_attr<4, true>())); IL_TRY((tc_set_attr<5>())); IL_TRY((tc_set_attr<6>())); IL_TRY((tc_set_attr<7>()));
   return 0;
 }
 
@@ -467,6 +539,35 @@
     return rc;
   }
   return tc_launch<6>(h, p, stream);
+}
+
+int launch_tc_gemm_adam(il_handle* h, const GemmArgs& a, const TcAdam& opt, cudaStream_t stream) {
+  auto al16 = [](const void* q) { return (reinterpret_cast<uintptr_t>(q) & 15) == 0; };
+  IL_CHECK(gemm_uses_tc(h, a) && !a.bias && a.act < 0 && !a.mask && !a.mask_bits, "tc_gemm_adam: not a plain product on the wgmma engine (M=%d N=%d K=%d)", a.M, a.N, a.K);
+  IL_CHECK(opt.p && opt.m && opt.v && opt.step && al16(opt.p) && al16(opt.m) && al16(opt.v) && al16(opt.target) && opt.gs % 4 == 0 && opt.nets_per_replica >= 1,
+           "tc_gemm_adam: bad optimiser buffers");
+  TcParams p{};
+  p.g = a;
+  p.g.C = nullptr;
+  p.split = h->gemm_mode == IL_GEMM_TF32X3 ? 1 : 0;
+  p.opt = opt;
+  auto run = [&]() {
+    IL_TRY(tc_launch<7>(h, p, stream));
+    if (a.colsum) {
+      dim3 cg((a.M + 127) / 128, a.G);
+      IL_LAUNCH(h, colsum_kernel, cg, 128, 0, stream, a.A, a.a_gs, a.a_gdiv, a.lda, a.K, a.M, a.colsum, a.colsum_gs);
+    }
+    return 0;
+  };
+  if (h->profiling) {
+    const double bytes = gemm_algorithmic_bytes(a, false) + 2.0 * 4.0 * (opt.target ? 4 : 3) * a.G * (double)a.M * a.N;
+    ProfiledLaunch pl;
+    IL_TRY(profile_open(h, &pl, 2.0 * a.M * a.N * a.K * a.G, bytes, stream));
+    const int rc = run();
+    IL_TRY(profile_close(h, &pl, stream));
+    return rc;
+  }
+  return run();
 }
 
 int launch_tc_gemm(il_handle* h, const GemmArgs& a, cudaStream_t stream) {
diff --git a/include/il_b200.h b/include/il_b200.h
--- a/include/il_b200.h
+++ b/include/il_b200.h
@@ -72,6 +72,9 @@
                   const float* B, int64_t b_gs, int ldb, int b_kmajor, float* C, int64_t c_gs, int ldc,
                   const float* bias, int64_t bias_gs, int act, const float* mask, int64_t mask_gs, int ldmask, int mask_act,
                   float* colsum, int64_t colsum_gs, void* stream);
+int il_debug_gemm_adam(il_handle* h, int M, int N, int K, int G, const float* A, int64_t a_gs, int lda, int a_kmajor,
+                       const float* B, int64_t b_gs, int ldb, int b_kmajor, float* params, const float* grads, int64_t net_floats, int64_t w_off,
+                       const il_adam* opt, float* target, float polyak_factor, const float* polyak_r, void* stream);
 
 int il_fill_normal(il_handle* h, float* out, int64_t n, uint64_t seed, uint64_t stream_id, const uint64_t* counter, void* stream);
 int il_fill_uniform(il_handle* h, float* out, int64_t n, uint64_t seed, uint64_t stream_id, const uint64_t* counter, void* stream);
```

Result: faster. 81130, median of 6 (+1.6%).
